# intellerce/controlanimate

Hardware: AMD Instinct MI355X
Metric: frames_per_sec (higher is better)
Workload: dtype fp16

## Files before the change

### controlanimate_amd/_capi.py

```python
from __future__ import annotations

import ctypes as C
import os

_HERE = os.path.dirname(os.path.abspath(__file__))
LIB_PATH = os.environ.get("CA_HIP_LIB") or os.path.join(_HERE, "csrc", "libcontrolanimate_hip.so")

CA_BF16, CA_F16 = 0, 1
CA_F32 = 2
CA_ACT_NONE, CA_ACT_SILU = 0, 1
CA_ACT_RELU = 4
CA_ACT_RELU6 = 5
CA_ACT_LEAKY02 = 6
CA_MLSD_TOPK = 200
CA_POSE_MAX_PEAKS, CA_POSE_MAX_PEOPLE, CA_POSE_AREA_TAPS = 64, 64, 8
CA_POSE_OVERFLOW_PEAKS, CA_POSE_OVERFLOW_PEOPLE = 1, 2
CA_POSE_OVERFLOW_FACES, CA_POSE_OVERFLOW_FACE_RESIZE = 4, 8
CA_FACE_SIZE, CA_FACE_HEAT, CA_FACE_PARTS, CA_FACE_MIN_SIDE, CA_FACE_SLOT_INTS = 384, 48, 71, 11, 8
CA_FACE_MODE_NONE, CA_FACE_MODE_LANCZOS4, CA_FACE_MODE_AREA = 0, 1, 2
CA_POSE_OVERFLOW_HANDS, CA_POSE_OVERFLOW_HAND_RESIZE = 16, 32
CA_HAND_PARTS, CA_HAND_HEAT_COLS, CA_HAND_MAP, CA_HAND_SCALES, CA_HAND_SLOT_INTS = 21, 24, 128, 4, 8
CA_HAND_MODE_NONE, CA_HAND_MODE_RESIZE, CA_HAND_MIN_BOX, CA_HAND_AREA_TAPS = 0, 1, 20, 16
ABI_VERSION = 16


class CAHipUnavailable(RuntimeError):
    pass


class CAHipError(RuntimeError):
    pass


class GemmArgs(C.Structure):
    _fields_ = [
        ("a", C.c_void_p), ("a2", C.c_void_p), ("w", C.c_void_p), ("c", C.c_void_p),
        ("bias", C.c_void_p), ("rowbias", C.c_void_p), ("residual", C.c_void_p),
        ("lda", C.c_int64), ("lda2", C.c_int64), ("ldc", C.c_int64), ("ld_res", C.c_int64),
        ("ld_rowbias", C.c_int64),
        ("m", C.c_int32), ("n", C.c_int32), ("k1", C.c_int32), ("k2", C.c_int32),
        ("rows_per_group", C.c_int32),
        ("alpha", C.c_float), ("post_scale", C.c_float),
        ("act", C.c_int32), ("geglu", C.c_int32), ("out_f32", C.c_int32), ("dtype", C.c_int32),
        ("ln_stats", C.c_void_p), ("ln_colsum", C.c_void_p), ("ln_eps", C.c_float),
        ("workspace", C.c_void_p), ("workspace_bytes", C.c_int64),
        ("row_sums_out", C.c_void_p), ("ln_parts", C.c_int32),
        ("w_frag", C.c_void_p),
    ]


class FfArgs(C.Structure):
    _fields_ = [
        ("x", C.c_void_p), ("w1_frag", C.c_void_p), ("bias1", C.c_void_p), ("colsum1", C.c_void_p), ("ln_stats", C.c_void_p),
        ("w2_frag", C.c_void_p), ("bias2", C.c_void_p), ("residual", C.c_void_p), ("y", C.c_void_p),
        ("lda", C.c_int64), ("ldc", C.c_int64), ("ld_res", C.c_int64),
        ("m", C.c_int32), ("c", C.c_int32), ("inner", C.c_int32), ("ln_eps", C.c_float), ("dtype", C.c_int32),
        ("w_out_frag", C.c_void_p), ("bias_out", C.c_void_p), ("residual_out", C.c_void_p), ("ld_res_out", C.c_int64),
    ]


class TattnArgs(C.Structure):
    _fields_ = [
        ("x", C.c_void_p), ("w_frag", C.c_void_p), ("gamma", C.c_void_p), ("bias_pe", C.c_void_p), ("o", C.c_void_p),
        ("lda", C.c_int64), ("ldo", C.c_int64), ("ld_bias_pe", C.c_int64),
        ("batch", C.c_int32), ("frames", C.c_int32), ("tokens", C.c_int32), ("heads", C.c_int32), ("c", C.c_int32),
        ("ln_eps", C.c_float), ("scale", C.c_float), ("dtype", C.c_int32),
        ("w_out_frag", C.c_void_p), ("bias_out", C.c_void_p), ("residual", C.c_void_p), ("ld_res", C.c_int64),
    ]


ATTN_WOUT_FRAG_ELEMS = 102400
TATTN_W_FRAG_ELEMS = 368640


class XattnArgs(C.Structure):
    _fields_ = [
        ("x", C.c_void_p), ("wq_frag", C.c_void_p), ("bias", C.c_void_p), ("kv_frag", C.c_void_p), ("o", C.c_void_p),
        ("lda", C.c_int64), ("ldo", C.c_int64),
        ("m", C.c_int32), ("tokens", C.c_int32), ("frames_per_kv", C.c_int32), ("kv_mod", C.c_int32), ("kv_batches", C.c_int32),
        ("nk", C.c_int32), ("heads", C.c_int32), ("c", C.c_int32),
        ("ln_eps", C.c_float), ("dtype", C.c_int32),
        ("w_out_frag", C.c_void_p), ("bias_out", C.c_void_p), ("residual", C.c_void_p), ("ld_res", C.c_int64),
        ("kv_frag_ip", C.c_void_p), ("nk_ip", C.c_int32), ("ip_scale", C.c_float),
    ]


XATTN_W_FRAG_ELEMS = 122880
XATTN_KV_FRAG_ELEMS = 7680


class ConvArgs(C.Structure):
    _fields_ = [
        ("x", C.c_void_p), ("x2", C.c_void_p), ("w", C.c_void_p), ("y", C.c_void_p),
        ("bias", C.c_void_p), ("rowbias", C.c_void_p), ("residual", C.c_void_p),
        ("ld_res", C.c_int64), ("ld_rowbias", C.c_int64),
        ("images", C.c_int32), ("hin", C.c_int32), ("win", C.c_int32),
        ("cin1", C.c_int32), ("cin2", C.c_int32), ("cout", C.c_int32),
        ("stride", C.c_int32), ("upsample", C.c_int32), ("rows_per_group", C.c_int32),
        ("alpha", C.c_float), ("post_scale", C.c_float),
        ("act", C.c_int32), ("out_f32", C.c_int32), ("dtype", C.c_int32),
        ("workspace", C.c_void_p), ("workspace_bytes", C.c_int64), ("pad_asym", C.c_int32),
        ("w_wino", C.c_void_p), ("x_is_wino_v", C.c_int32),
    ]


class GroupNormArgs(C.Structure):
    _fields_ = [
        ("x", C.c_void_p), ("x2", C.c_void_p), ("y", C.c_void_p),
        ("gamma", C.c_void_p), ("beta", C.c_void_p), ("partials", C.c_void_p),
        ("images", C.c_int32), ("hw", C.c_int32), ("c1", C.c_int32), ("c2", C.c_int32),
        ("groups", C.c_int32), ("frames_per_stat", C.c_int32),
        ("eps", C.c_float), ("act", C.c_int32), ("dtype", C.c_int32),
        ("wino_v", C.c_void_p), ("wino_h", C.c_int32), ("wino_w", C.c_int32),
    ]


class LayerNormArgs(C.Structure):
    _fields_ = [
        ("x", C.c_void_p), ("y", C.c_void_p), ("gamma", C.c_void_p), ("beta", C.c_void_p),
        ("pos", C.c_void_p),
        ("rows", C.c_int64),
        ("c", C.c_int32), ("rows_per_frame", C.c_int32), ("frames", C.c_int32),
        ("eps", C.c_float), ("dtype", C.c_int32), ("stats", C.c_void_p),
    ]


class AttnArgs(C.Structure):
    _fields_ = [
        ("q", C.c_void_p), ("k", C.c_void_p), ("v", C.c_void_p), ("o", C.c_void_p),
        ("q_outer", C.c_int64), ("q_inner", C.c_int64), ("q_row", C.c_int64),
        ("o_outer", C.c_int64), ("o_inner", C.c_int64), ("o_row", C.c_int64),
        ("k_outer", C.c_int64), ("k_inner", C.c_int64), ("k_row", C.c_int64),
        ("inner_count", C.c_int32), ("kv_inner_count", C.c_int32), ("kv_div", C.c_int32), ("kv_mod", C.c_int32),
        ("batches", C.c_int32), ("heads", C.c_int32), ("head_dim", C.c_int32),
        ("nq", C.c_int32), ("nk", C.c_int32),
        ("scale", C.c_float), ("out_scale", C.c_float),
        ("accumulate", C.c_int32), ("dtype", C.c_int32), ("causal", C.c_int32),
        ("key_mask", C.c_void_p), ("key_mask_stride", C.c_int64),
    ]


class ConvNarrowArgs(C.Structure):
    _fields_ = [
        ("x", C.c_void_p), ("w", C.c_void_p), ("y", C.c_void_p), ("bias", C.c_void_p), ("r1", C.c_void_p), ("r2", C.c_void_p),
        ("ldx", C.c_int64), ("ldy", C.c_int64), ("ld_r1", C.c_int64), ("ld_r2", C.c_int64),
        ("images", C.c_int32), ("hin", C.c_int32), ("win", C.c_int32), ("cin", C.c_int32), ("cout", C.c_int32),
        ("channel_offset", C.c_int32), ("upsample", C.c_int32), ("leaky_relu", C.c_int32),
        ("s0", C.c_float), ("s1", C.c_float), ("s2", C.c_float),
        ("out_u8", C.c_int32), ("dtype", C.c_int32),
    ]


class PerceiverAttnArgs(C.Structure):
    _fields_ = [
        ("q", C.c_void_p), ("x", C.c_void_p), ("l", C.c_void_p), ("o", C.c_void_p),
        ("q_row", C.c_int64), ("q_batch", C.c_int64),
        ("x_row", C.c_int64), ("x_batch", C.c_int64), ("x_v_off", C.c_int64),
        ("l_row", C.c_int64), ("l_batch", C.c_int64), ("l_v_off", C.c_int64),
        ("o_row", C.c_int64), ("o_batch", C.c_int64),
        ("batches", C.c_int32), ("heads", C.c_int32), ("head_dim", C.c_int32),
        ("nq", C.c_int32), ("n_x", C.c_int32), ("n_l", C.c_int32),
        ("scale", C.c_float), ("dtype", C.c_int32),
    ]


class ModconvArgs(C.Structure):
    _fields_ = [
        ("x", C.c_void_p), ("wt", C.c_void_p), ("s", C.c_void_p), ("demod", C.c_void_p), ("noise", C.c_void_p), ("bias", C.c_void_p),
        ("sft_scale", C.c_void_p), ("sft_shift", C.c_void_p), ("y", C.c_void_p),
        ("s_stride", C.c_int64), ("demod_stride", C.c_int64),
        ("images", C.c_int32), ("h", C.c_int32), ("w", C.c_int32), ("cin", C.c_int32), ("cout", C.c_int32),
        ("upsample", C.c_int32), ("x_shared", C.c_int32),
        ("noise_weight", C.c_float), ("dtype", C.c_int32),
    ]


class Conv7x7Args(C.Structure):
    _fields_ = [
        ("x", C.c_void_p * 2), ("w", C.c_void_p * 2), ("bias", C.c_void_p * 2), ("y", C.c_void_p * 2),
        ("ldx", C.c_int64), ("ldy", C.c_int64),
        ("groups", C.c_int32), ("images", C.c_int32), ("h", C.c_int32), ("w_px", C.c_int32), ("cin", C.c_int32), ("cout", C.c_int32),
        ("relu", C.c_int32), ("dtype", C.c_int32),
    ]


SYMBOLS = {
    "ca_abi_version": (C.c_int, []),
    "ca_last_error": (C.c_char_p, []),
    "ca_gemm": (C.c_int, [C.POINTER(GemmArgs), C.c_void_p]),
    "ca_pack_w_frag": (C.c_int, [C.c_void_p, C.c_int32, C.c_int32, C.c_int32, C.c_void_p, C.c_void_p]),
    "ca_pack_w2_frag": (C.c_int, [C.c_void_p, C.c_int32, C.c_int32, C.c_void_p, C.c_void_p]),
    "ca_ff_fused": (C.c_int, [C.POINTER(FfArgs), C.c_void_p]),
    "ca_ff_fused_supported": (C.c_int, [C.POINTER(FfArgs)]),
    "ca_tattn_fused": (C.c_int, [C.POINTER(TattnArgs), C.c_void_p]),
    "ca_tattn_fused_supported": (C.c_int, [C.POINTER(TattnArgs)]),
    "ca_pack_w_tattn": (C.c_int, [C.c_void_p, C.c_int32, C.c_int32, C.c_void_p, C.c_void_p]),
    "ca_pack_w_out": (C.c_int, [C.c_void_p, C.c_int32, C.c_int32, C.c_void_p, C.c_void_p]),
    "ca_xattn_fused": (C.c_int, [C.POINTER(XattnArgs), C.c_void_p]),
    "ca_xattn_fused_supported": (C.c_int, [C.POINTER(XattnArgs)]),
    "ca_xattn_pack_w": (C.c_int, [C.c_void_p, C.c_int32, C.c_int32, C.c_void_p, C.c_void_p]),
    "ca_xattn_pack_kv": (C.c_int, [C.c_void_p, C.c_int64, C.c_int32, C.c_int32, C.c_int32, C.c_int32, C.c_float, C.c_int32, C.c_void_p, C.c_void_p]),
    "ca_gemm_ln_inline_supported": (C.c_int, [C.POINTER(GemmArgs)]),
    "ca_gemm_wants_finished_stats": (C.c_int, [C.POINTER(GemmArgs)]),
    "ca_ln_finish_sums": (C.c_int, [C.c_void_p, C.c_int, C.c_int64, C.c_int, C.c_float, C.c_void_p, C.c_void_p]),
    "ca_gemm_workspace_bytes": (C.c_int64, [C.POINTER(GemmArgs)]),
    "ca_gemm_row_sums_parts": (C.c_int, [C.POINTER(GemmArgs)]),
    "ca_gemm_plan_name": (C.c_int, [C.POINTER(GemmArgs), C.c_char_p, C.c_int32]),
    "ca_conv3x3_plan_name": (C.c_int, [C.POINTER(ConvArgs), C.c_char_p, C.c_int32]),
    "ca_conv3x3": (C.c_int, [C.POINTER(ConvArgs), C.c_void_p]),
    "ca_pack_w_wino": (C.c_int, [C.c_void_p, C.c_int32, C.c_int32, C.c_int32, C.c_void_p, C.c_void_p]),
    "ca_conv3x3_workspace_bytes": (C.c_int64, [C.POINTER(ConvArgs)]),
    "ca_softmax_rows": (C.c_int, [C.c_void_p, C.c_void_p, C.c_int64, C.c_int32, C.c_int64, C.c_int64, C.c_float, C.c_int32, C.c_void_p]),
    "ca_groupnorm_partials_floats": (C.c_int64, [C.c_int32, C.c_int32, C.c_int32, C.c_int32]),
    "ca_groupnorm_stats": (C.c_int, [C.POINTER(GroupNormArgs), C.c_void_p]),
    "ca_groupnorm_apply": (C.c_int, [C.POINTER(GroupNormArgs), C.c_void_p]),
    "ca_groupnorm": (C.c_int, [C.POINTER(GroupNormArgs), C.c_void_p]),
    "ca_groupnorm_wino_supported": (C.c_int, [C.POINTER(GroupNormArgs)]),
    "ca_layernorm": (C.c_int, [C.POINTER(LayerNormArgs), C.c_void_p]),
    "ca_attention": (C.c_int, [C.POINTER(AttnArgs), C.c_void_p]),
    "ca_attention_plan_name": (C.c_int, [C.POINTER(AttnArgs), C.c_char_p, C.c_int32]),
    "ca_add_bcast": (C.c_int, [C.c_void_p, C.c_void_p, C.c_void_p, C.c_int64, C.c_int64, C.c_int32, C.c_void_p]),
    "ca_repeat": (C.c_int, [C.c_void_p, C.c_void_p, C.c_int64, C.c_int32, C.c_void_p]),
    "ca_silu_f32": (C.c_int, [C.c_void_p, C.c_void_p, C.c_int64, C.c_void_p]),
    "ca_timestep_embedding": (C.c_int, [C.c_void_p, C.c_float, C.c_void_p, C.c_int32, C.c_int32, C.c_int32, C.c_void_p]),
    "ca_latents_to_nhwc": (C.c_int, [C.c_void_p, C.c_void_p, C.c_int32, C.c_int32, C.c_int32, C.c_int32, C.c_int32,
                                      C.c_int32, C.c_int32, C.c_float, C.c_int32, C.c_void_p]),
    "ca_nhwc_to_ncfhw_f32": (C.c_int, [C.c_void_p, C.c_void_p, C.c_int32, C.c_int32, C.c_int32, C.c_int32, C.c_int32,
                                        C.c_int32, C.c_int32, C.c_int32, C.c_void_p]),
    "ca_ncfhw_to_nhwc": (C.c_int, [C.c_void_p, C.c_int32, C.POINTER(C.c_int64), C.c_void_p, C.c_int32, C.c_int32,
                                    C.c_int32, C.c_int32, C.c_int32, C.c_int32, C.c_int32, C.c_void_p]),
    "ca_cfg_scheduler_step": (C.c_int, [C.c_void_p, C.c_int32, C.c_int32, C.c_float, C.c_void_p, C.c_void_p,
                                         C.c_void_p, C.c_void_p, C.c_int32, C.c_int32, C.c_int32, C.c_int32,
                                         C.POINTER(C.c_float), C.c_float, C.c_void_p]),
    "ca_lincomb": (C.c_int, [C.c_void_p, C.POINTER(C.c_void_p), C.POINTER(C.c_float), C.c_int32, C.c_int64, C.c_void_p]),
    "ca_conv3x3_narrow": (C.c_int, [C.POINTER(ConvNarrowArgs), C.c_void_p]),
    "ca_conv3x3_narrow_plan_name": (C.c_int, [C.POINTER(ConvNarrowArgs), C.c_char_p, C.c_int32]),
    "ca_rgb8_to_nhwc": (C.c_int, [C.c_void_p, C.c_void_p, C.c_int32, C.c_int32, C.c_int32, C.c_int32, C.c_void_p]),
    "ca_resize_lanczos4_u8": (C.c_int, [C.c_void_p, C.c_void_p, C.c_int32, C.c_int32, C.c_int32, C.c_int32, C.c_int32,
                                         C.c_void_p, C.c_void_p, C.c_void_p, C.c_void_p, C.c_void_p]),
    "ca_color_match_workspace_bytes": (C.c_int64, [C.c_int32, C.c_int64]),
    "ca_hist_u8x3": (C.c_int, [C.c_void_p, C.c_void_p, C.c_int32, C.c_int64, C.c_void_p]),
    "ca_color_moments_f64": (C.c_int, [C.c_void_p, C.c_void_p, C.c_void_p, C.c_void_p, C.c_int32, C.c_int64, C.c_void_p, C.c_int64, C.c_void_p]),
    "ca_color_transform_f64": (C.c_int, [C.c_void_p, C.c_void_p, C.c_void_p, C.c_void_p, C.c_void_p, C.c_void_p, C.c_int32, C.c_int64, C.c_void_p]),
    "ca_sort_f64_segments": (C.c_int, [C.c_void_p, C.c_void_p, C.c_int32, C.c_int64, C.c_void_p, C.c_int64, C.c_void_p]),
    "ca_color_rank_map_f64": (C.c_int, [C.c_void_p, C.c_void_p, C.c_void_p, C.c_void_p, C.c_void_p, C.c_void_p, C.c_int32, C.c_int64,
                                         C.c_void_p, C.c_int64, C.c_void_p]),
    "ca_color_finish_u8": (C.c_int, [C.c_void_p, C.c_void_p, C.c_int32, C.c_int64, C.c_int32, C.c_void_p, C.c_int64, C.c_void_p]),
    "ca_canny_workspace_bytes": (C.c_int64, [C.c_int32, C.c_int32, C.c_int32]),
    "ca_canny_tile_w": (C.c_int32, []),
    "ca_canny_tile_h": (C.c_int32, []),
    "ca_canny_classify": (C.c_int, [C.c_void_p, C.c_int32, C.c_int32, C.c_int32, C.c_int32, C.c_int32, C.c_int32, C.c_void_p, C.c_int64, C.c_void_p]),
    "ca_canny_link": (C.c_int, [C.c_int32, C.c_int32, C.c_int32, C.c_void_p, C.c_int64, C.c_void_p]),
    "ca_canny_link_stage": (C.c_int, [C.c_int32, C.c_int32, C.c_int32, C.c_void_p, C.c_int64, C.c_int32, C.c_void_p]),
    "ca_canny_emit": (C.c_int, [C.c_int32, C.c_int32, C.c_int32, C.c_void_p, C.c_int64, C.c_void_p, C.c_void_p, C.c_int32, C.c_int32, C.c_void_p]),
    "ca_conv_up2_phase_supported": (C.c_int, [C.POINTER(ConvArgs)]),
    "ca_conv_up2_phase": (C.c_int, [C.POINTER(ConvArgs), C.c_void_p]),
    "ca_conv_up2_phase_plan_name": (C.c_int, [C.POINTER(ConvArgs), C.c_char_p, C.c_int32]),
    "ca_perceiver_attn": (C.c_int, [C.POINTER(PerceiverAttnArgs), C.c_void_p]),
    "ca_hed_prep": (C.c_int, [C.c_void_p, C.c_void_p, C.c_void_p, C.c_int32, C.c_int32, C.c_int32, C.c_int32, C.c_void_p]),
    "ca_hed_pool_side": (C.c_int, [C.c_void_p, C.c_void_p, C.c_void_p, C.c_void_p, C.c_void_p, C.c_int32, C.c_int32, C.c_int32, C.c_int32, C.c_int32, C.c_void_p]),
    "ca_hed_fuse": (C.c_int, [C.c_void_p, C.c_void_p, C.c_void_p, C.c_void_p, C.c_void_p, C.c_int32, C.c_int32, C.c_int32, C.c_void_p, C.c_void_p, C.c_int32, C.c_int32, C.c_void_p]),
    "ca_lineart_conv_in": (C.c_int, [C.c_void_p, C.c_void_p, C.c_void_p, C.c_int32, C.c_int32, C.c_int32, C.c_int32, C.c_void_p]),
    "ca_instnorm_partials_floats": (C.c_int64, [C.c_int32, C.c_int32, C.c_int32, C.c_int32]),
    "ca_instnorm_stats": (C.c_int, [C.c_void_p, C.c_void_p, C.c_int32, C.c_int32, C.c_int32, C.c_int32, C.c_int32, C.c_int32, C.c_void_p]),
    "ca_instnorm_apply": (C.c_int, [C.c_void_p, C.c_void_p, C.c_void_p, C.c_void_p, C.c_int32, C.c_int32, C.c_int32, C.c_int32, C.c_int32, C.c_int32, C.c_int32,
                                    C.c_int32, C.c_float, C.c_int32, C.c_void_p]),
    "ca_convt3x3s2_gather": (C.c_int, [C.c_void_p, C.c_void_p, C.c_int32, C.c_int32, C.c_int32, C.c_int32, C.c_int32, C.c_void_p]),
    "ca_lineart_conv_out": (C.c_int, [C.c_void_p, C.c_void_p, C.c_void_p, C.c_void_p, C.c_int32, C.c_int32, C.c_int32, C.c_int32, C.c_void_p]),
    "ca_lineart_finish": (C.c_int, [C.c_void_p, C.c_int32, C.c_int32, C.c_int32, C.c_void_p, C.c_void_p, C.c_int32, C.c_int32, C.c_void_p]),
    "ca_mlsd_prep": (C.c_int, [C.c_void_p, C.c_void_p, C.c_int32, C.c_int32, C.c_int32, C.c_int32, C.c_void_p]),
    "ca_dwconv3x3": (C.c_int, [C.c_void_p, C.c_void_p, C.c_void_p, C.c_void_p, C.c_int32, C.c_int32, C.c_int32, C.c_int32, C.c_int32, C.c_int32, C.c_int32, C.c_void_p]),
    "ca_upsample2x_bilinear_ac": (C.c_int, [C.c_void_p, C.c_void_p, C.c_int32, C.c_int32, C.c_int32, C.c_int32, C.c_int64, C.c_int32, C.c_int32, C.c_void_p]),
    "ca_conv3x3_dil": (C.c_int, [C.c_void_p, C.c_void_p, C.c_void_p, C.c_void_p, C.c_int32, C.c_int32, C.c_int32, C.c_int32, C.c_int32, C.c_int32, C.c_int32, C.c_void_p]),
    "ca_mlsd_decode_workspace_bytes": (C.c_int64, [C.c_int32, C.c_int32, C.c_int32]),
    "ca_mlsd_decode": (C.c_int, [C.c_void_p, C.c_int32, C.c_int32, C.c_int32, C.c_float, C.c_float, C.c_void_p, C.c_int64, C.c_void_p, C.c_void_p, C.c_void_p]),
    "ca_mlsd_draw": (C.c_int, [C.c_void_p, C.c_void_p, C.c_int32, C.c_int32, C.c_int32, C.c_void_p, C.c_void_p, C.c_int32, C.c_int32, C.c_void_p]),
    "ca_softedge_prep": (C.c_int, [C.c_void_p, C.c_void_p, C.c_int32, C.c_int32, C.c_int32, C.c_int32, C.c_void_p]),
    "ca_relu": (C.c_int, [C.c_void_p, C.c_void_p, C.c_int64, C.c_int32, C.c_void_p]),
    "ca_dwconv_k": (C.c_int, [C.c_void_p, C.c_void_p, C.c_void_p, C.c_int32, C.c_int32, C.c_int32, C.c_int32, C.c_int32, C.c_int32, C.c_int32, C.c_void_p]),
    "ca_maxpool2x2": (C.c_int, [C.c_void_p, C.c_void_p, C.c_int32, C.c_int32, C.c_int32, C.c_int32, C.c_int32, C.c_void_p]),
    "ca_pdc_block_supported": (C.c_int, [C.c_int32, C.c_int32]),
    "ca_pdc_block": (C.c_int, [C.c_void_p, C.c_void_p, C.c_void_p, C.c_void_p, C.c_int32, C.c_int32, C.c_int32, C.c_int32, C.c_int32, C.c_int32, C.c_void_p]),
    "ca_cdcm_dil4": (C.c_int, [C.c_void_p, C.c_void_p, C.c_void_p, C.c_int32, C.c_int32, C.c_int32, C.c_int32, C.c_int32, C.c_void_p]),
    "ca_csam_reduce": (C.c_int, [C.c_void_p] * 9 + [C.c_int32] * 5 + [C.c_void_p]),
    "ca_softedge_fuse": (C.c_int, [C.c_void_p] * 5 + [C.c_int32] * 4 + [C.c_void_p] * 3 + [C.c_int32, C.c_int32, C.c_void_p]),
    "ca_lanime_conv_in": (C.c_int, [C.c_void_p] * 5 + [C.c_int32] * 4 + [C.c_void_p]),
    "ca_conv4x4s2": (C.c_int, [C.c_void_p] * 4 + [C.c_int32] * 7 + [C.c_void_p]),
    "ca_im2col4x4s2": (C.c_int, [C.c_void_p] * 2 + [C.c_int32] * 5 + [C.c_void_p]),
    "ca_convt4x4s2": (C.c_int, [C.c_void_p] * 3 + [C.c_int32] * 6 + [C.c_void_p]),
    "ca_instnorm_act_partials_floats": (C.c_int64, [C.c_int32, C.c_int32, C.c_int32, C.c_int32]),
    "ca_instnorm_act": (C.c_int, [C.c_void_p, C.c_void_p] + [C.c_void_p, C.c_int32, C.c_int32, C.c_int32] * 2 + [C.c_int32] * 4 + [C.c_float, C.c_int32, C.c_void_p]),
    "ca_lanime_conv_out": (C.c_int, [C.c_void_p] * 4 + [C.c_int32] * 4 + [C.c_void_p]),
    "ca_lanime_finish": (C.c_int, [C.c_void_p, C.c_int32, C.c_int32, C.c_int32, C.c_void_p, C.c_void_p, C.c_int32, C.c_int32, C.c_void_p]),
    "ca_gfp_prep": (C.c_int, [C.c_void_p] * 4 + [C.c_int32] * 6 + [C.c_void_p]),
    "ca_resample2x": (C.c_int, [C.c_void_p] * 2 + [C.c_int32] * 6 + [C.c_void_p]),
    "ca_gfp_styles": (C.c_int, [C.c_void_p, C.c_void_p, C.c_int64, C.POINTER(C.c_int32), C.c_int32, C.c_void_p, C.c_int64, C.c_int32, C.c_int32, C.c_void_p]),
    "ca_modconv3x3": (C.c_int, [C.POINTER(ModconvArgs), C.c_void_p]),
    "ca_gfp_modulate": (C.c_int, [C.c_void_p, C.c_void_p, C.c_int64, C.c_void_p] + [C.c_int32] * 7 + [C.c_void_p]),
    "ca_gfp_style_epilogue": (C.c_int, [C.c_void_p, C.c_void_p, C.c_int64, C.c_void_p, C.c_float] + [C.c_void_p] * 4 + [C.c_int32] * 5 + [C.c_void_p]),
    "ca_gfp_to_rgb": (C.c_int, [C.c_void_p, C.c_void_p, C.c_void_p, C.c_int64, C.c_void_p, C.c_void_p, C.c_void_p] + [C.c_int32] * 5 + [C.c_void_p]),
    "ca_gfp_finish": (C.c_int, [C.c_void_p, C.c_void_p, C.c_int64, C.c_int32, C.c_void_p]),
    "ca_resize_pil_u8": (C.c_int, [C.c_void_p] * 3 + [C.c_int32] * 5 + [C.c_void_p, C.c_void_p, C.c_int32, C.c_void_p, C.c_void_p, C.c_int32, C.c_void_p]),
    "ca_dpt_patches": (C.c_int, [C.c_void_p, C.c_void_p] + [C.c_int32] * 4 + [C.c_void_p]),
    "ca_depth_to_space": (C.c_int, [C.c_void_p, C.c_void_p] + [C.c_int32] * 5 + [C.c_int64, C.c_int32, C.c_int32, C.c_int32, C.c_void_p]),
    "ca_dpt_head_supported": (C.c_int, [C.c_int32]),
    "ca_dpt_head": (C.c_int, [C.c_void_p] * 6 + [C.c_int32] * 5 + [C.c_void_p]),
    "ca_dpt_logit": (C.c_int, [C.c_void_p] * 4 + [C.c_int64, C.c_void_p]),
    "ca_resize_bicubic_f32": (C.c_int, [C.c_void_p] * 4 + [C.c_int32] * 5 + [C.c_void_p]),
    "ca_depth_finish": (C.c_int, [C.c_void_p, C.c_void_p] + [C.c_int32] * 4 + [C.c_void_p, C.c_void_p, C.c_int32, C.c_int32, C.c_void_p]),
    "ca_pose_prep": (C.c_int, [C.c_void_p] * 8 + [C.c_int32] * 8 + [C.c_void_p]),
    "ca_conv7x7": (C.c_int, [C.POINTER(Conv7x7Args), C.c_void_p]),
    "ca_im2col7x7": (C.c_int, [C.c_void_p] * 2 + [C.c_int32] * 4 + [C.c_int64, C.c_int32, C.c_void_p]),
    "ca_copy_cols": (C.c_int, [C.c_void_p, C.c_void_p, C.c_int64, C.c_int32, C.c_int64, C.c_int32, C.c_int32, C.c_void_p]),
    "ca_pose_maps_workspace_bytes": (C.c_int64, [C.c_int32] * 3),
    "ca_pose_maps": (C.c_int, [C.c_void_p] * 4 + [C.c_int64] + [C.c_void_p] * 3 + [C.c_int32] * 5 + [C.c_void_p]),
    "ca_pose_peaks": (C.c_int, [C.c_void_p] * 6 + [C.c_int32] * 3 + [C.c_void_p]),
    "ca_pose_connect": (C.c_int, [C.c_void_p] * 6 + [C.c_int32] * 3 + [C.c_void_p]),
    "ca_pose_assemble": (C.c_int, [C.c_void_p] * 9 + [C.c_int32] * 3 + [C.c_void_p]),
    "ca_pose_draw": (C.c_int, [C.c_void_p] * 6 + [C.c_int32] * 5 + [C.c_void_p]),
    "ca_face_boxes": (C.c_int, [C.c_void_p] * 6 + [C.c_int32] * 4 + [C.c_void_p]),
    "ca_face_crop": (C.c_int, [C.c_void_p] * 8 + [C.c_int32] * 8 + [C.c_void_p]),
    "ca_face_peaks": (C.c_int, [C.c_void_p] * 3 + [C.c_int32] * 4 + [C.c_void_p]),
    "ca_pose_draw_faces": (C.c_int, [C.c_void_p] * 9 + [C.c_int32] * 5 + [C.c_void_p]),
    "ca_hand_boxes": (C.c_int, [C.c_void_p] * 6 + [C.c_int32] * 4 + [C.c_void_p]),
    "ca_hand_crop": (C.c_int, [C.c_void_p] * 10 + [C.c_int32] * 10 + [C.c_void_p]),
    "ca_hand_maps": (C.c_int, [C.c_void_p] * 7 + [C.c_int32] + [C.c_void_p]),
    "ca_hand_peaks": (C.c_int, [C.c_void_p] * 6 + [C.c_int32] * 4 + [C.c_void_p]),
    "ca_pose_draw_hands": (C.c_int, [C.c_void_p] * 10 + [C.c_int32] * 5 + [C.c_void_p]),
}

_lib = None


def lib() -> C.CDLL:
    global _lib
    if _lib is not None:
        return _lib
    import torch
    if not os.path.exists(LIB_PATH):
        raise CAHipUnavailable(
            f"{LIB_PATH} is missing: the HIP extension is not built. Run "
            "`python -m controlanimate_amd._build` (needs hipcc); there is no CPU fallback.")
    try:
        handle = C.CDLL(LIB_PATH)
    except OSError as e:
        raise CAHipUnavailable(f"cannot load {LIB_PATH}: {e}") from e
    for name, (res, args) in SYMBOLS.items():
        fn = getattr(handle, name)
        fn.restype = res
        fn.argtypes = args
    if handle.ca_abi_version() != ABI_VERSION:
        raise CAHipUnavailable(f"ABI mismatch: library {handle.ca_abi_version()} vs binding {ABI_VERSION}; rebuild")
    _lib = handle
    return handle
# ... 7 lines not shown
```

### controlanimate_amd/attention_processor.py

```python
from __future__ import annotations

from typing import Optional

import torch
from torch import nn

from . import kernels as K
from .context import dispatch
from .layers import HipLinear, LnFold, WeightArena, ln_fold_enabled, pack_concat_rows


class AttnProcessor2_0(nn.Module):

    num_tokens = 0
    drop_ip_tokens = False

    def __init__(self, hidden_size=None, cross_attention_dim=None):
        super().__init__()

    def ip_branch(self, attn, q, ctx, out, images, tokens, kv_rows, frames_per_kv, kv_mod, cache):
        return out

    def ip_fragments(self, attn, ctx, cache):
        return None

    def __call__(self, attn: "Attention", hidden_states: torch.Tensor, encoder_hidden_states: Optional[torch.Tensor] = None,
                 attention_mask=None, temb=None, *, residual: Optional[torch.Tensor] = None, frames_per_kv: int = 1,
                 kv_mod: int = 0, temporal=None, cache: Optional[dict] = None, ln=None, row_sums: bool = False) -> torch.Tensor:
        if attention_mask is not None:
            raise NotImplementedError("attention_mask is not used anywhere on the reference's path")
        B, N, C = hidden_states.shape
        x = hidden_states.reshape(B * N, C)
        res = None if residual is None else residual.reshape(B * N, C)
        if ln is not None and encoder_hidden_states is None and temporal is not None and getattr(attn, "tfrag", None) is not None:
            b, f, n = temporal
            ofrag = getattr(attn, "ofrag", None)
            if ofrag is not None and dispatch.attn_out_fused:
                to_out = attn.to_out[0]
                out = K.tattn_fused(x, attn.tfrag.t, attn.tgamma.t, attn.tbias_pe.t, b, f, n, attn.heads, attn.tln_eps, attn.scale,
                                    w_out_frag=ofrag.t, bias_out=None if to_out.b is None else to_out.b.t, residual=res)
                if out is not None:
                    return out.reshape(B, N, C)
            o = K.tattn_fused(x, attn.tfrag.t, attn.tgamma.t, attn.tbias_pe.t, b, f, n, attn.heads, attn.tln_eps, attn.scale)
            if o is not None:
                out = attn.to_out[0].run(o, residual=res, row_sums=row_sums)
                return K.carry_row_sums(out.reshape(B, N, C), out)
        builtin = type(self).ip_branch is AttnProcessor2_0.ip_branch
        with_ip = (not builtin and type(self).ip_fragments is not AttnProcessor2_0.ip_fragments and dispatch.attn_out_fused and dispatch.xattn_ip_fused
                   and getattr(attn, "ofrag", None) is not None)
        if (ln is not None and encoder_hidden_states is not None and cache is not None and getattr(attn, "xfrag", None) is not None
                and (builtin or with_ip)):
            ctx = encoder_hidden_states
            nb, L, cd = ctx.shape
            nk = L - self.num_tokens
            kv = cache.get(("kv", id(attn)))
            if kv is None:
                kv = cache[("kv", id(attn))] = K.gemm(ctx.reshape(nb * L, cd), attn.kv.t)
            ent = cache.get(("kvf", id(attn)))
            if ent is None:
                ent = cache[("kvf", id(attn))] = (K.xattn_pack_kv(kv, nb, L, nk, attn.scale), nk, L)
            if ent[0] is not None and ent[1] == nk:
                ofrag = getattr(attn, "ofrag", None)
                if ofrag is not None and dispatch.attn_out_fused:
                    to_out = attn.to_out[0]
                    ipf = self.ip_fragments(attn, ctx, cache) if with_ip else None
                    if not with_ip or ipf is not None:
                        out = K.xattn_fused(x, attn.xfrag.t, ln[1].b.t, ent[0], B, N, frames_per_kv, kv_mod, nk, ln[1].eps, w_out_frag=ofrag.t,
                                            bias_out=None if to_out.b is None else to_out.b.t, residual=res,
                                            kv_frag_ip=None if ipf is None else ipf[0], nk_ip=0 if ipf is None else ipf[1],
                                            ip_scale=1.0 if ipf is None else ipf[2])
                        if out is not None:
                            return out.reshape(B, N, C)
                o = K.xattn_fused(x, attn.xfrag.t, ln[1].b.t, ent[0], B, N, frames_per_kv, kv_mod, nk, ln[1].eps) if builtin else None
                if o is not None:
                    out = attn.to_out[0].run(o, residual=res, row_sums=row_sums)
                    return K.carry_row_sums(out.reshape(B, N, C), out)
        if ln is not None:
            st, fold = ln
            if encoder_hidden_states is None and temporal is not None and fold.pe is not None:
                b, f, n = temporal
                qkv = K.gemm(x, fold.w.t, bias=fold.b.t, ln=(st, fold.cs.t), rowbias=fold.rowbias(b, f), rows_per_group=n)
            else:
                qkv = K.gemm(x, fold.w.t, bias=fold.b.t, ln=(st, fold.cs.t))
        if encoder_hidden_states is None:
            if ln is None:
                qkv = K.gemm(x, attn.qkv.t)
            if temporal is not None:
                b, f, n = temporal
                o = K.attention_temporal(qkv, b, f, n, attn.heads)
            else:
                o = K.attention_spatial(qkv, B, N, attn.heads)
        else:
            ctx = encoder_hidden_states
            nb, L, cd = ctx.shape
            q = qkv if ln is not None else K.gemm(x, attn.to_q.w.t)
            kv = None if cache is None else cache.get(("kv", id(attn)))
            if kv is None:
                kv = K.gemm(ctx.reshape(nb * L, cd), attn.kv.t)
                if cache is not None:
                    cache[("kv", id(attn))] = kv
            nk = L - self.num_tokens
            o = K.attention_cross(q, kv, B, N, attn.heads, nk, L, frames_per_kv, kv_mod=kv_mod)
            o = self.ip_branch(attn, q, ctx, o, B, N, L, frames_per_kv, kv_mod, cache)
        out = attn.to_out[0].run(o, residual=res, row_sums=row_sums)
        return K.carry_row_sums(out.reshape(B, N, C), out)


class IPAttnProcessor2_0(AttnProcessor2_0):

    def __init__(self, hidden_size, cross_attention_dim=None, scale=1.0, num_tokens=4):
        super().__init__()
        self.hidden_size = hidden_size
        self.cross_attention_dim = cross_attention_dim
        self.scale = scale
        self.num_tokens = num_tokens
        self.to_k_ip = HipLinear(cross_attention_dim or hidden_size, hidden_size, bias=False)
        self.to_v_ip = HipLinear(cross_attention_dim or hidden_size, hidden_size, bias=False)
        self.kv_ip = None

    def pack(self, arena: WeightArena, dtype):
        self.kv_ip = pack_concat_rows(arena, dtype, [self.to_k_ip, self.to_v_ip])

    def _kv_ip(self, ctx, cache):
        if self.kv_ip is None:
            raise RuntimeError("IPAttnProcessor2_0 installed after prepare(); call model.prepare() again")
        nb, L, cd = ctx.shape
        kvip = None if cache is None else cache.get(("kv_ip", id(self)))
        if kvip is None:
            kvip = K.gemm(ctx.reshape(nb * L, cd), self.kv_ip.t)
            if cache is not None:
                cache[("kv_ip", id(self))] = kvip
        return kvip

    def ip_fragments(self, attn, ctx, cache):
        nb, L, cd = ctx.shape
        if cache is None or not (1 <= self.num_tokens <= 16):
            return None
        ent = cache.get(("kvf_ip", id(self)))
        if ent is None:
            kvip = self._kv_ip(ctx, cache)
            ent = cache[("kvf_ip", id(self))] = (K.xattn_pack_kv(kvip, nb, L, self.num_tokens, attn.scale, row_offset=L - self.num_tokens),
                                                 self.num_tokens, L, attn.scale)
        if ent[0] is None or ent[1] != self.num_tokens or ent[2] != L:
            return None
        return ent[0], self.num_tokens, float(self.scale)

    def ip_branch(self, attn, q, ctx, out, images, tokens, kv_rows, frames_per_kv, kv_mod, cache):
        nb, L, cd = ctx.shape
        kvip = self._kv_ip(ctx, cache)
        return K.attention_cross(q, kvip, images, tokens, attn.heads, self.num_tokens, L, frames_per_kv, out=out,
                                 out_scale=float(self.scale), accumulate=True, kv_row_offset=L - self.num_tokens,
                                 kv_mod=kv_mod)


class CNAttnProcessor2_0(AttnProcessor2_0):

    def __init__(self, num_tokens=4):
        super().__init__()
        self.num_tokens = num_tokens


AttnProcessor = AttnProcessor2_0
IPAttnProcessor = IPAttnProcessor2_0
CNAttnProcessor = CNAttnProcessor2_0


class Attention(nn.Module):

    def __init__(self, query_dim: int, cross_attention_dim: Optional[int] = None, heads: int = 8, dim_head: int = 64,
                 dropout: float = 0.0, bias: bool = False, upcast_attention: bool = False, processor=None, **_):
        super().__init__()
        inner = heads * dim_head
        self.is_cross = cross_attention_dim is not None
        ctx_dim = cross_attention_dim if self.is_cross else query_dim
        self.query_dim, self.cross_attention_dim, self.inner_dim = query_dim, ctx_dim, inner
        self.heads = heads
        self.scale = dim_head ** -0.5
        self.spatial_norm = None
        self.group_norm = None
        self.norm_cross = None
        self.residual_connection = False
        self.rescale_output_factor = 1.0
        self.to_q = HipLinear(query_dim, inner, bias=bias)
        self.to_k = HipLinear(ctx_dim, inner, bias=bias)
        self.to_v = HipLinear(ctx_dim, inner, bias=bias)
        self.to_out = nn.ModuleList([HipLinear(inner, query_dim, bias=True), nn.Identity()])
        self.processor = processor if processor is not None else AttnProcessor2_0()
        self.qkv = self.kv = self.fold = None

    def set_processor(self, processor, _remove_lora: bool = False):
        if isinstance(getattr(self, "processor", None), nn.Module) and not isinstance(processor, nn.Module):
            self._modules.pop("processor", None)
        self.processor = processor

    def get_processor(self, return_deprecated_lora: bool = False):
        return self.processor

    def builtin_processor(self) -> bool:
        return type(self.processor) in (AttnProcessor2_0, IPAttnProcessor2_0, CNAttnProcessor2_0)

    def pack(self, arena: WeightArena, dtype, fold_ln=None, pe=None):
        self.fold = None
        if fold_ln is not None and self.builtin_processor() and ln_fold_enabled():
            self.fold = LnFold(arena, dtype, fold_ln, [self.to_q] if self.is_cross else [self.to_q, self.to_k, self.to_v], pe=pe)
            if self.is_cross:
                self.kv = pack_concat_rows(arena, dtype, [self.to_k, self.to_v])
                self.xfrag = None
                if (self.heads, self.inner_dim, self.query_dim) == (8, 320, 320):
                    from .layers import frag_order_xattn
                    fold = self.fold
                    self.xfrag = arena.add((122880,), dtype, lambda: frag_order_xattn(fold.w_fold().to(dtype).float()))
        elif self.is_cross:
            self.to_q.pack(arena, dtype)
            self.kv = pack_concat_rows(arena, dtype, [self.to_k, self.to_v])
        else:
            self.qkv = pack_concat_rows(arena, dtype, [self.to_q, self.to_k, self.to_v])
        self.to_out[0].pack(arena, dtype)
        self.ofrag = None
        if (self.heads, self.inner_dim, self.query_dim) == (8, 320, 320) and self.fold is not None:
            from .layers import _f32, frag_order_wout
            to_out = self.to_out[0]
            self.ofrag = arena.add((102400,), dtype, lambda: frag_order_wout(_f32(to_out.weight)))
        if hasattr(self.processor, "pack"):
            self.processor.pack(arena, dtype)

    def forward(self, hidden_states, encoder_hidden_states=None, attention_mask=None, **kw):
        return self.processor(self, hidden_states, encoder_hidden_states=encoder_hidden_states,
                              attention_mask=attention_mask, **kw)
```

### controlanimate_amd/context.py

```python
from __future__ import annotations

from dataclasses import dataclass, field
from typing import Optional

import torch


@dataclass
class ExecCtx:
    b: int
    f: int
    dtype: torch.dtype
    temb: torch.Tensor
    emb_groups: int
    ehs: Optional[torch.Tensor] = None
    frames_per_kv: int = 1
    kv_mod: int = 0
    gn_frames_per_stat: int = 1
    cache: dict = field(default_factory=dict)

    @property
    def images(self) -> int:
        return self.b * self.f

    def rows_per_emb_group(self, h: int, w: int) -> int:
        return self.images // self.emb_groups * h * w


class Dispatch:
    gemm_ar = True
    ff_fused = True
    tattn_fused = True
    xattn_fused = True
    attn_out_fused = True
    xattn_ip_fused = True
    conv_winograd = True
    gn_winograd = True
    conv_up2_phase = True
    ln_row_sums = True
    repeat_kernel = True
    ln_fold = True
    cfg_shared = True
    cn_cfg_dedup = True
    pdc_block_fused = True
    dpt_head_fused = False
    pose_conv7_direct = True
    controlnet_streams = 2


dispatch = Dispatch()
```

### controlanimate_amd/csrc/ca_gemm.hip

```cpp

#include "ca_gemm_plan.h"

namespace {
using namespace ca_gemm_detail;
#include "ca_conv_wino.h"

template <int DT, int BM, int BN, int WAVES_M, int WAVES_N, int MODE>
__global__ __launch_bounds__(256) void k_gemm(GemmKParams p) {
  constexpr int TM = BM / WAVES_M / 16;
  constexpr int TN = BN / WAVES_N / 16;
  constexpr int AI = BM / 32;
  constexpr int BI = BN / 32;
  static_assert(2 * (BM + BN) * BK >= BM * (BN + 8), "epilogue staging must fit");
  __shared__ __attribute__((aligned(16))) u16 smem[2 * (BM + BN) * BK];

  const int tid = threadIdx.x;
  const int lane = tid & 63;
  const int wid = tid >> 6;
  const int wm = wid / WAVES_N, wn = wid % WAVES_N;
  const int g = lane >> 4, l15 = lane & 15;

  const int tiles_n = (p.n + BN - 1) / BN;
  const unsigned bid = xcd_remap(blockIdx.x, gridDim.x);
  int tile_m, tile_n;
// ... 389 lines not shown
      return CA_OK;
    case PK_REG:
      if (g.bn == 128) hipLaunchKernelGGL((k_gemm<DT, 128, 128, 2, 2, MODE>), grid, dim3(256), 0, st, p);
      else if (g.bn == 64) hipLaunchKernelGGL((k_gemm<DT, 128, 64, 4, 1, MODE>), grid, dim3(256), 0, st, p);
      else break;
      return CA_OK;
  }
  CA_FAIL(CA_ERR_LAUNCH, "ca_gemm: no kernel for plan kind %d, tile %dx%d, %d stages", (int)g.kind, g.bm, g.bn, g.nbuf);
}

}

extern "C" int ca_gemm(const ca_gemm_args* a, void* stream) {
  DenseLaunch d;
  int rc = gemm_prepare(a, d);
  if (rc) return rc;
  hipStream_t st = (hipStream_t)stream;
  rc = a->dtype == CA_BF16 ? launch_gemm<CA_BF16, 0>(d.p, d.plan, st) : launch_gemm<CA_F16, 0>(d.p, d.plan, st);
  if (rc) return rc;
  CA_CHECK_LAUNCH("ca_gemm");
  return CA_OK;
}

extern "C" int64_t ca_gemm_workspace_bytes(const ca_gemm_args* a) {
  DenseLaunch d;
  return gemm_resolve(a, d) == CA_OK ? d.workspace : 0;
}

extern "C" int ca_gemm_row_sums_parts(const ca_gemm_args* a) {
  DenseLaunch d;
  DenseAsk ask{};
  ask.without_row_sums = true;
  return gemm_resolve(a, d, ask) == CA_OK ? row_sums_parts_of(d.p) : 0;
}

extern "C" int ca_gemm_ln_inline_supported(const ca_gemm_args* a) {
  DenseLaunch d;
  return a && a->ln_colsum && gemm_resolve(a, d) == CA_OK && wres_eligible(d.p) ? 1 : 0;
}

extern "C" int ca_gemm_wants_finished_stats(const ca_gemm_args* a) {
  if (!a || !a->ln_colsum || !a->ln_stats || a->ln_parts <= 0 || a->row_sums_out) return 0;
  DenseLaunch d;
  DenseAsk ask{};
  ask.stats_finished = true;
  return gemm_resolve(a, d, ask) == CA_OK && d.plan.kind == PK_PQ ? 1 : 0;
}

extern "C" int64_t ca_conv3x3_workspace_bytes(const ca_conv_args* a) { return conv_workspace_bytes(a); }

static int launch_conv_wino(const ca_conv_args* a, const GemmKParams& cp, hipStream_t st) {
  const int kc = a->cin1 + a->cin2;
  const ConvGeom g = conv_geom(a);
  const int64_t tiles = wino_tiles(a, g);
  WinoParams w{};
  w.x = (const u16*)a->x;
  w.x2 = (const u16*)a->x2;
  w.v = (u16*)a->workspace;
  u16* mm = (u16*)a->workspace + (a->x_is_wino_v ? 0 : 16 * tiles * kc);
  w.mm = mm;
  w.y = (u16*)a->y;
  w.bias = a->bias;
  w.rowbias = a->rowbias;
  w.res = (const u16*)a->residual;
  w.ld_res = a->ld_res;
  w.ld_rowbias = a->ld_rowbias;
  w.images = a->images, w.h = g.hl, w.w = g.wl, w.c1 = a->cin1, w.c2 = a->cin2, w.cout = a->cout;
  w.ups = a->upsample;
  w.rows_per_group = cp.rows_per_group;
  w.alpha = a->alpha, w.post = a->post_scale, w.act = a->act;
  const int64_t in_threads = tiles * (kc / 8), out_threads = tiles * (a->cout / 8);
  if (a->x_is_wino_v) w.v = (u16*)a->x;
  else if (a->dtype == CA_BF16) hipLaunchKernelGGL((k_wino_in<CA_BF16>), dim3((unsigned)((in_threads + 255) / 256)), dim3(256), 0, st, w);
  else hipLaunchKernelGGL((k_wino_in<CA_F16>), dim3((unsigned)((in_threads + 255) / 256)), dim3(256), 0, st, w);
  GemmKParams q{};
  q.a = w.v;
  q.w = (const u16*)a->w_wino;
  q.c = mm;
  q.lda = kc;
  q.ldc = a->cout;
  q.a_bytes = desc_bytes(16 * tiles * kc);
  q.w_bytes = desc_bytes((int64_t)16 * a->cout * kc);
  q.m = (int)(16 * tiles);
  q.n = a->cout;
  q.c1 = kc;
  q.taps = 1;
  q.kc_tiles = kc / BK;
  q.rows_per_group = 1;
  q.alpha = 1.f, q.post = 1.f;
  q.splits = 1;
  q.w_group_rows = (int)tiles;
  q.w_group_stride = (unsigned)((int64_t)a->cout * kc * 2);
  const unsigned gemm_tiles = (unsigned)((q.m / 256) * (q.n / 320));
  int rc = ca_launch_gemm_pp(q, a->dtype, 0, PK_PQ, gemm_tiles, st);
  if (rc) return rc;
  if (a->dtype == CA_BF16) hipLaunchKernelGGL((k_wino_out<CA_BF16>), dim3((unsigned)((out_threads + 255) / 256)), dim3(256), 0, st, w);
  else hipLaunchKernelGGL((k_wino_out<CA_F16>), dim3((unsigned)((out_threads + 255) / 256)), dim3(256), 0, st, w);
  return CA_OK;
}

extern "C" int ca_pack_w_wino(const void* w, int32_t cout, int32_t cin, int32_t dtype, void* dst, void* stream) {
  CA_REQUIRE(w && dst, "ca_pack_w_wino: null operand");
  CA_REQUIRE(cout > 0 && cin > 0 && (dtype == CA_BF16 || dtype == CA_F16), "ca_pack_w_wino: cout=%d cin=%d dtype=%d", cout, cin, dtype);
  const int64_t n = (int64_t)cout * cin;
  if (dtype == CA_BF16) hipLaunchKernelGGL((k_pack_w_wino<CA_BF16>), dim3((unsigned)((n + 255) / 256)), dim3(256), 0, (hipStream_t)stream, (const u16*)w, (u16*)dst, cout, cin);
  else hipLaunchKernelGGL((k_pack_w_wino<CA_F16>), dim3((unsigned)((n + 255) / 256)), dim3(256), 0, (hipStream_t)stream, (const u16*)w, (u16*)dst, cout, cin);
  CA_CHECK_LAUNCH("ca_pack_w_wino");
  return CA_OK;
}

extern "C" int ca_conv3x3(const ca_conv_args* a, void* stream) {
  GemmKParams p{};
  int rc = conv_prepare(a, p);
  if (rc) return rc;
  hipStream_t st = (hipStream_t)stream;
  if (wino_taken(a)) {
    rc = launch_conv_wino(a, p, st);
    if (rc) return rc;
    CA_CHECK_LAUNCH("ca_conv3x3(winograd)");
    return CA_OK;
  }
  CA_REQUIRE(!a->x_is_wino_v, "ca_conv3x3: x_is_wino_v, but the Winograd route does not take these arguments (images=%d %dx%d cin=%d+%d cout=%d dtype=%d w_wino=%p "
             "workspace=%p of %lld bytes, needs %lld)", a->images, a->hin, a->win, a->cin1, a->cin2, a->cout, a->dtype, a->w_wino, a->workspace,
             (long long)a->workspace_bytes, (long long)wino_workspace_bytes(a));
  rc = a->dtype == CA_BF16 ? launch_gemm<CA_BF16, 1>(p, plan_gemm(p, 1), st) : launch_gemm<CA_F16, 1>(p, plan_gemm(p, 1), st);
  if (rc) return rc;
  CA_CHECK_LAUNCH("ca_conv3x3");
  return CA_OK;
}

extern "C" int ca_conv_up2_phase_supported(const ca_conv_args* a) {
  GemmKParams p{};
  return up2_capable(a, p) && up2_pays(p) ? 1 : 0;
}

extern "C" int ca_conv_up2_phase(const ca_conv_args* a, void* stream) {
  GemmKParams p{};
  CA_REQUIRE(up2_capable(a, p), "ca_conv_up2_phase: arguments the phase form does not take (one fp16 / bf16 source with cin %% 64 == 0, cout %% 320 == 0, upsample = 1, "
             "stride 1, symmetric padding, no row bias / activation / post scale / fp32 output, 16-byte aligned operands, < 2^23 source pixels)");
  int rc = ca_launch_gemm_pp(p, a->dtype, 2, PK_PQ, up2_tiles_total(p), (hipStream_t)stream);
  if (rc) return rc;
  CA_CHECK_LAUNCH("ca_conv_up2_phase");
  return CA_OK;
}

extern "C" int ca_conv_up2_phase_plan_name(const ca_conv_args* a, char* buf, int32_t len) {
  CA_REQUIRE(buf && len > 0, "ca_conv_up2_phase_plan_name: buffer");
  GemmKParams p{};
  CA_REQUIRE(up2_capable(a, p), "ca_conv_up2_phase_plan_name: arguments the phase form does not take");
  snprintf(buf, (size_t)len, "up2_pq256x320");
  return CA_OK;
}

extern "C" int ca_gemm_plan_name(const ca_gemm_args* a, char* buf, int32_t len) {
  CA_REQUIRE(buf && len > 0, "ca_gemm_plan_name: buffer");
  DenseLaunch d;
  int rc = gemm_prepare(a, d);
  if (rc) return rc;
  plan_label(d.plan, buf, len);
  return CA_OK;
}

extern "C" int ca_conv3x3_plan_name(const ca_conv_args* a, char* buf, int32_t len) {
  CA_REQUIRE(buf && len > 0, "ca_conv3x3_plan_name: buffer");
  GemmKParams p{};
  int rc = conv_prepare(a, p);
  if (rc) return rc;
  if (wino_taken(a)) {
    snprintf(buf, (size_t)len, "wino_pq256x320");
    return CA_OK;
  }
  plan_label(plan_gemm(p, 1), buf, len);
  return CA_OK;
}
```

### controlanimate_amd/csrc/ca_gemm_core.h

```cpp
#pragma once
#include "ca_common.h"
#include <stdlib.h>

namespace ca_gemm_detail {


struct GemmKParams {
  const u16* a;
  const u16* a2;
  const u16* w;
  void* c;
  const float* bias;
  const float* rowbias;
  const float* ln_stats;
  const float* ln_colsum;
  const u16* res;
  int64_t lda, lda2, ldc, ld_res, ld_rowbias;
  unsigned a_bytes, a2_bytes, w_bytes;
  int m, n;
  int c1, c2;
  int taps;
  int kc_tiles;
  int hin, win, hout, wout, stride, ups, pad_lo;
  int rows_per_group;
  float alpha, post;
  int act, geglu, out_f32;
  int splits;
  float* partial;
  int dbg;
  int tap_inner;
  float* row_sums;
  int ln_parts;
  int ln_inline;
  float ln_eps;
  const u16* wf;
  int w_group_rows;
  unsigned w_group_stride;
  int up2_rows, up2_tiles;
  unsigned up2_mag_w, up2_mag_h;
};

constexpr int BK = 64;

constexpr int GROUP_M = 8;
__device__ __forceinline__ void tile_coords(unsigned bid, int tiles_m, int tiles_n, int& tile_m, int& tile_n) {
  const unsigned gsz = GROUP_M * tiles_n;
  const unsigned group = bid / gsz, in = bid - group * gsz;
  const int first_m = group * GROUP_M;
  const int gm = tiles_m - first_m < GROUP_M ? tiles_m - first_m : GROUP_M;
  tile_m = first_m + in % gm;
  tile_n = in / gm;
}

__device__ __forceinline__ void k_tile_split(const GemmKParams& p, int t, int kct, int& tap, int& cc) {
  if (p.taps == 1) {
    tap = 0;
    cc = t;
  } else if (p.tap_inner) {
    cc = t / p.taps;
    tap = t - cc * p.taps;
  } else {
    tap = t / kct;
    cc = t - tap * kct;
  }
}

__device__ __forceinline__ int lds_off(int row, int chunk) {
  return row * BK + ((chunk ^ ((row >> 1) & 7)) << 3);
}

template <int DT, int TM, int TN>
__device__ __forceinline__ void gemm_epilogue_direct(const GemmKParams& p, f32x4 (&acc)[TM][TN], int m0, int n0, int wm, int wn,
                                                     int l15, int g) {
#pragma unroll
  for (int i = 0; i < TM; ++i) {
    const int m = m0 + wm * TM * 16 + i * 16 + l15;
    if (m >= p.m) continue;
    const float* rbp = p.rowbias ? p.rowbias + (int64_t)(m / p.rows_per_group) * p.ld_rowbias : nullptr;
#pragma unroll
    for (int j = 0; j < TN; ++j) {
      const int n = n0 + wn * TN * 16 + j * 16 + g * 4;
      if (n >= p.n) continue;
      float v[4];
#pragma unroll
      for (int r = 0; r < 4; ++r) v[r] = acc[i][j][r];
      if (p.bias) {
        f32x4 b = *reinterpret_cast<const f32x4*>(p.bias + n);
#pragma unroll
        for (int r = 0; r < 4; ++r) v[r] += b[r];
      }
      if (rbp) {
        f32x4 b = *reinterpret_cast<const f32x4*>(rbp + n);
#pragma unroll
        for (int r = 0; r < 4; ++r) v[r] += b[r];
      }
#pragma unroll
      for (int r = 0; r < 4; ++r) v[r] *= p.alpha;
      if (p.res) {
        u32x2 rr = *reinterpret_cast<const u32x2*>(p.res + (int64_t)m * p.ld_res + n);
        v[0] += Elem<DT>::to_f((u16)(rr[0] & 0xffffu));
        v[1] += Elem<DT>::to_f((u16)(rr[0] >> 16));
        v[2] += Elem<DT>::to_f((u16)(rr[1] & 0xffffu));
        v[3] += Elem<DT>::to_f((u16)(rr[1] >> 16));
      }
#pragma unroll
      for (int r = 0; r < 4; ++r) v[r] *= p.post;
      if (p.act != CA_ACT_NONE) {
#pragma unroll
        for (int r = 0; r < 4; ++r) v[r] = act_f(v[r], p.act);
      }
      if (p.geglu) {
        const f32x2 gg = gelu_erf_f2((f32x2){v[1], v[3]});
        float o0 = v[0] * gg[0];
        float o1 = v[2] * gg[1];
        const int64_t off = (int64_t)m * p.ldc + (n >> 1);
        if (p.out_f32) {
          float* cp = reinterpret_cast<float*>(p.c) + off;
          cp[0] = o0;
          cp[1] = o1;
        } else {
          *reinterpret_cast<unsigned*>(reinterpret_cast<u16*>(p.c) + off) = pack2<DT>(o0, o1);
        }
      } else {
        const int64_t off = (int64_t)m * p.ldc + n;
        if (p.out_f32) {
          *reinterpret_cast<f32x4*>(reinterpret_cast<float*>(p.c) + off) = (f32x4){v[0], v[1], v[2], v[3]};
        } else {
          u32x2 o;
          o[0] = pack2<DT>(v[0], v[1]);
          o[1] = pack2<DT>(v[2], v[3]);
          *reinterpret_cast<u32x2*>(reinterpret_cast<u16*>(p.c) + off) = o;
        }
      }
    }
  }
}

template <int DT, int BM, int BN, int TM, int TN, int NT = 256, bool ROWSUM = false>
__device__ __forceinline__ void gemm_epilogue(const GemmKParams& p, f32x4 (&acc)[TM][TN], u16* cs, int m0, int n0, int wm, int wn,
                                              int l15, int g, int tid, float2* rs = nullptr) {
  if (p.n < 8) {
    gemm_epilogue_direct<DT, TM, TN>(p, acc, m0, n0, wm, wn, l15, g);
    return;
  }
  constexpr int CLD = BN + 8;
  float2 ln_st[TM];
  f32x4 ln_cs[TN];
  if (p.ln_stats) {
#pragma unroll
    for (int i = 0; i < TM; ++i) {
      const int m = m0 + wm * TM * 16 + i * 16 + l15;
      if (p.ln_parts > 0) {
        float a = 0.f, b = 0.f;
        if (m < p.m) {
          for (int q = 0; q < p.ln_parts; ++q) {
            const float2 v = *reinterpret_cast<const float2*>(p.ln_stats + ((int64_t)m * p.ln_parts + q) * 2);
            a += v.x;
            b += v.y;
          }
        }
        const float inv = 1.f / (float)(p.c1 + p.c2);
        const float mean = a * inv;
        ln_st[i] = make_float2(mean, rsqrtf(fmaxf(b * inv - mean * mean, 0.f) + p.ln_eps));
      } else {
        ln_st[i] = m < p.m ? *reinterpret_cast<const float2*>(p.ln_stats + (int64_t)m * 2) : make_float2(0.f, 0.f);
      }
    }
#pragma unroll
    for (int j = 0; j < TN; ++j) {
      const int n = n0 + wn * TN * 16 + j * 16 + g * 4;
      ln_cs[j] = n < p.n ? *reinterpret_cast<const f32x4*>(p.ln_colsum + n) : (f32x4){0.f, 0.f, 0.f, 0.f};
    }
  }
  f32x4 rb_q[TN];
  bool rb_uniform = false;
  if (p.rowbias) {
    const int r_first = m0 + wm * TM * 16, r_last = r_first + TM * 16 - 1;
    rb_uniform = r_last < p.m && r_first / p.rows_per_group == r_last / p.rows_per_group;
    if (rb_uniform) {
      const float* base = p.rowbias + (int64_t)(r_first / p.rows_per_group) * p.ld_rowbias;
#pragma unroll
      for (int j = 0; j < TN; ++j) {
        const int n = n0 + wn * TN * 16 + j * 16 + g * 4;
        rb_q[j] = n < p.n ? *reinterpret_cast<const f32x4*>(base + n) : (f32x4){0.f, 0.f, 0.f, 0.f};
      }
    }
  }
#pragma unroll
  for (int i = 0; i < TM; ++i) {
    const int row = wm * TM * 16 + i * 16 + l15;
    const int m = m0 + row;
    const float* rbp = (p.rowbias && !rb_uniform && m < p.m) ? p.rowbias + (int64_t)(m / p.rows_per_group) * p.ld_rowbias : nullptr;
// ... 186 lines not shown
```

### controlanimate_amd/csrc/ca_gemm_plan.h

```cpp
#pragma once
#include "ca_gemm_core.h"

namespace ca_gemm_detail {

inline unsigned desc_bytes(int64_t elems) {
  const int64_t b = elems * 2;
  return (b > 0 && b < (int64_t)0xFFFFFF00ll) ? (unsigned)b : 0u;
}

inline bool dma_shape_ok(const GemmKParams& p) { return (p.c1 + p.c2) % BK == 0 && (p.c2 == 0 || p.c1 % BK == 0); }
inline bool dma_sizes_ok(const GemmKParams& p) { return p.a_bytes != 0 && p.w_bytes != 0 && (p.c2 == 0 || p.a2_bytes != 0); }
inline bool dma_capable(const GemmKParams& p) { return dma_shape_ok(p) && dma_sizes_ok(p); }

inline bool wres_eligible(const GemmKParams& p) {
  static const int wres_env = CA_KNOB("CA_GEMM_WRES", -1);
  const int kc = p.c1 + p.c2;
  return wres_env != 0 && kc == 320 && p.taps == 1 && (p.c2 == 0 || p.c1 % 32 == 0) && p.n % 160 == 0 && p.n / 160 <= 32 && !p.out_f32 &&
         p.splits <= 1 && !p.ln_parts && dma_sizes_ok(p) &&
         (!p.rowbias || p.rows_per_group % 32 == 0) &&
         act_out_fit31(p) &&
         (wres_env == 1 || p.m >= 16384);
}

inline bool ar_eligible(const GemmKParams& p, bool scratch) {
// ... 188 lines not shown
  d = DenseLaunch{};
  GemmKParams& p = d.p;
  int rc = gemm_fill(a, p, ask);
  if (rc) return rc;
  const SplitK k = splitk_decide(p, 0);
  splitk_apply(k, a->workspace, a->workspace_bytes, p);
  d.workspace = k.bytes;
  if (p.ln_inline && p.wf) {
    if (ar_eligible(p, true)) d.workspace = (int64_t)p.m * 8;
    if (a->workspace && a->workspace_bytes >= (int64_t)p.m * 8) p.partial = reinterpret_cast<float*>(a->workspace);
  }
  d.plan = plan_gemm(p, 0);
  return CA_OK;
}

inline int gemm_prepare(const ca_gemm_args* a, DenseLaunch& d) {
  int rc = gemm_resolve(a, d);
  if (rc) return rc;
  CA_REQUIRE(!d.p.row_sums || row_sums_capable(d.p), "ca_gemm: row_sums_out is not available for this launch: ask ca_gemm_row_sums_parts() first");
  CA_REQUIRE(!d.p.ln_inline || wres_eligible(d.p), "ca_gemm: in-kernel LayerNorm statistics (ln_stats NULL) are not available for this launch: "
             "ask ca_gemm_ln_inline_supported() first and pass ln_stats otherwise");
  return CA_OK;
}

struct ConvGeom { int hl, wl, hout, wout; int64_t m; };
inline ConvGeom conv_geom(const ca_conv_args* a) {
  ConvGeom g;
  g.hl = a->hin << a->upsample, g.wl = a->win << a->upsample;
  const int pad = a->pad_asym ? 1 : 2;
  g.hout = (g.hl + pad - 3) / a->stride + 1;
  g.wout = (g.wl + pad - 3) / a->stride + 1;
  g.m = (int64_t)a->images * g.hout * g.wout;
  return g;
}
inline int64_t wino_tiles(const ca_conv_args* a, const ConvGeom& g) { return (int64_t)a->images * (g.hl / 2) * (g.wl / 2); }

inline int64_t wino_workspace_bytes(const ca_conv_args* a) {
  if (!a || !a->w_wino || (a->dtype != CA_F16 && a->dtype != CA_BF16) || a->stride != 1 || a->pad_asym || a->out_f32) return 0;
  if (a->upsample != 0 && a->upsample != 1) return 0;
  if (a->x_is_wino_v && (a->cin2 != 0 || a->upsample)) return 0;
  const ConvGeom g = conv_geom(a);
  if (a->images <= 0 || g.hl < 2 || g.wl < 2 || (g.hl & 1) || (g.wl & 1)) return 0;
  const int kc = a->cin1 + a->cin2;
  static const int min_cin = CA_KNOB("CA_WINO_MIN_CIN", 1280);
  if (kc < 640 || kc % BK != 0 || a->cin1 % 8 != 0 || a->cin2 % 8 != 0 || a->cout % 320 != 0) return 0;
  const int64_t tiles = wino_tiles(a, g);
  if (kc < min_cin && !(min_cin == 1280 && tiles <= 4096)) return 0;
  static const int max_tiles = CA_KNOB("CA_WINO_MAX_TILES", 16384);
  if (tiles % 256 != 0 || tiles > max_tiles) return 0;
  if (16 * tiles * (int64_t)(kc > a->cout ? kc : a->cout) * 2 >= 0x7FFFFF00ll) return 0;
  return 16 * tiles * (int64_t)((a->x_is_wino_v ? 0 : kc) + a->cout) * 2;
}

inline bool wino_taken(const ca_conv_args* a) {
  const int64_t wb = wino_workspace_bytes(a);
  return wb > 0 && a->workspace && a->workspace_bytes >= wb && (((uintptr_t)a->workspace | (uintptr_t)a->w_wino) & 15) == 0;
}

inline void conv_fill_sizes(const ca_conv_args* a, const ConvGeom& g, GemmKParams& p) {
  p.a_bytes = desc_bytes((int64_t)a->images * a->hin * a->win * a->cin1);
  p.a2_bytes = a->cin2 ? desc_bytes((int64_t)a->images * a->hin * a->win * a->cin2) : 0u;
  p.w_bytes = desc_bytes((int64_t)a->cout * 9 * (a->cin1 + a->cin2));
  p.m = (int)g.m, p.n = a->cout, p.c1 = a->cin1, p.c2 = a->cin2;
  p.taps = 9;
  static const int tap_inner_env = CA_KNOB("CA_CONV_TAP_INNER", 1);
  p.tap_inner = tap_inner_env;
  p.kc_tiles = ceil_div_i(a->cin1 + a->cin2, BK);
  p.hin = a->hin, p.win = a->win, p.hout = g.hout, p.wout = g.wout;
  p.stride = a->stride, p.ups = a->upsample, p.pad_lo = a->pad_asym ? 0 : 1;
  p.geglu = 0, p.out_f32 = a->out_f32;
  p.splits = 1;
}

inline int conv_prepare(const ca_conv_args* a, GemmKParams& p) {
  CA_REQUIRE(a != nullptr, "ca_conv3x3: null args");
  CA_REQUIRE(a->x && a->w && a->y, "ca_conv3x3: null operand");
  CA_REQUIRE(a->images > 0 && a->hin > 0 && a->win > 0, "ca_conv3x3: bad geometry");
  CA_REQUIRE(a->cin1 > 0 && a->cin1 % 8 == 0 && a->cin2 >= 0 && a->cin2 % 8 == 0,
             "ca_conv3x3: cin1=%d cin2=%d must be multiples of 8", a->cin1, a->cin2);
  CA_REQUIRE(a->cin2 == 0 || a->x2, "ca_conv3x3: x2 missing");
  CA_REQUIRE(a->stride == 1 || a->stride == 2, "ca_conv3x3: stride %d", a->stride);
  CA_REQUIRE(a->upsample == 0 || a->upsample == 1, "ca_conv3x3: upsample %d", a->upsample);
  CA_REQUIRE(a->dtype == CA_BF16 || a->dtype == CA_F16, "ca_conv3x3: dtype %d", a->dtype);
  CA_REQUIRE(!a->rowbias || a->rows_per_group > 0, "ca_conv3x3: rows_per_group");
  int rc = check_epilogue("ca_conv3x3", a->cout, 0, a->cout, a->ld_res, a->residual);
  if (rc) return rc;
  CA_REQUIRE(a->pad_asym == 0 || a->pad_asym == 1, "ca_conv3x3: pad_asym %d", a->pad_asym);
  const ConvGeom g = conv_geom(a);
  CA_REQUIRE(g.m < (1ll << 31), "ca_conv3x3: too many output pixels");
  conv_fill_sizes(a, g, p);
  p.a = (const u16*)a->x, p.a2 = (const u16*)a->x2, p.w = (const u16*)a->w, p.c = a->y;
  p.bias = a->bias, p.rowbias = a->rowbias, p.res = (const u16*)a->residual;
  p.ldc = a->cout, p.ld_res = a->ld_res, p.ld_rowbias = a->ld_rowbias;
  p.rows_per_group = a->rows_per_group > 0 ? a->rows_per_group : 1;
  p.alpha = a->alpha, p.post = a->post_scale, p.act = a->act;
  splitk_apply(splitk_decide(p, 1), a->workspace, a->workspace_bytes, p);
  return CA_OK;
}

inline int64_t conv_workspace_bytes(const ca_conv_args* a) {
  if (!a || a->images <= 0 || a->hin <= 0 || a->win <= 0 || (a->stride != 1 && a->stride != 2)) return 0;
  const int64_t wb = wino_workspace_bytes(a);
  if (wb > 0) return wb;
  const ConvGeom g = conv_geom(a);
  if (g.m >= (1ll << 31)) return 0;
  GemmKParams p{};
  conv_fill_sizes(a, g, p);
  return splitk_decide(p, 1).bytes;
}

inline bool up2_capable(const ca_conv_args* a, GemmKParams& p) {
  if (!a || !a->x || !a->w || !a->y || a->x2 || a->cin2 != 0 || a->images <= 0 || a->hin <= 0 || a->win <= 0) return false;
  if (a->upsample != 1 || a->stride != 1 || a->pad_asym || a->out_f32 || a->x_is_wino_v || a->rowbias) return false;
  if ((a->dtype != CA_F16 && a->dtype != CA_BF16) || a->act != CA_ACT_NONE || a->post_scale != 1.f) return false;
  if (a->cin1 <= 0 || a->cin1 % BK != 0 || a->cout <= 0 || a->cout % 320 != 0) return false;
  if ((((uintptr_t)a->x | (uintptr_t)a->w | (uintptr_t)a->y | (uintptr_t)a->residual) & 15) != 0) return false;
  if (a->residual && (a->ld_res < a->cout || a->ld_res % 8 != 0)) return false;
  const int64_t rows = (int64_t)a->images * a->hin * a->win;
  if (rows + a->win + 2 >= (1 << 23)) return false;
  p = GemmKParams{};
  p.a = (const u16*)a->x;
  p.w = (const u16*)a->w;
  p.c = a->y;
  p.bias = a->bias;
  p.res = (const u16*)a->residual;
  p.ldc = a->cout;
  p.ld_res = a->ld_res;
  p.a_bytes = desc_bytes(rows * a->cin1);
  p.w_bytes = desc_bytes((int64_t)4 * a->cout * 4 * a->cin1);
  p.n = a->cout;
  p.c1 = a->cin1;
  p.taps = 4;
  p.tap_inner = 1;
  p.kc_tiles = a->cin1 / BK;
  p.hin = a->hin, p.win = a->win, p.hout = 2 * a->hin, p.wout = 2 * a->win;
  p.stride = 1, p.ups = 1, p.pad_lo = 1;
  p.rows_per_group = 1;
  p.alpha = a->alpha, p.post = 1.f;
  p.splits = 1;
  p.up2_rows = (int)rows;
  p.up2_tiles = ceil_div_i((int)rows, 256);
  p.m = 4 * p.up2_tiles * 256;
  p.up2_mag_w = a->win == 1 ? 0xFFFFFFFFu : (unsigned)((1ull << 32) / (unsigned)a->win);
  p.up2_mag_h = a->hin == 1 ? 0xFFFFFFFFu : (unsigned)((1ull << 32) / (unsigned)a->hin);
  p.w_group_stride = (unsigned)((int64_t)a->cout * 4 * a->cin1 * 2);
  return dma_sizes_ok(p) && act_out_fit31(p) && p.w_bytes < FIT31;
}
inline unsigned up2_tiles_total(const GemmKParams& p) { return (unsigned)(4 * p.up2_tiles * (p.n / 320)); }
inline bool up2_pays(const GemmKParams& p) {
  const unsigned tiles = up2_tiles_total(p);
  return tiles >= 256 && (tiles % 256 == 0 || tiles >= 1024);
}

}
```

### controlanimate_amd/csrc/ca_gemm_pp.hip

```cpp
#include "ca_gemm_core.h"
#include <type_traits>

namespace {
using namespace ca_gemm_detail;
#include "ca_gemm_pp2.h"
#include "ca_gemm_wres.h"
#include "ca_gemm_ps.h"
#include "ca_gemm_pq.h"

int cu_count() {
  static int n = 0;
  if (!n) {
    int dev = 0;
    hipDeviceProp_t prop;
    if (hipGetDevice(&dev) == hipSuccess && hipGetDeviceProperties(&prop, dev) == hipSuccess) n = prop.multiProcessorCount;
    if (n <= 0) n = 256;
  }
  return n;
}

template <class Launch>
int launch_stamped(const GemmKParams& p, hipStream_t st, const char* label, unsigned sep, unsigned eol, Launch launch) {
  static unsigned long long* dbuf = nullptr;
  if (!dbuf && hipMalloc(&dbuf, 4096 * 8) != hipSuccess) return CA_ERR_LAUNCH;
  (void)hipMemsetAsync(dbuf, 0, 4096 * 8, st);
  GemmKParams q = p;
  q.partial = reinterpret_cast<float*>(dbuf);
  launch(q);
  (void)hipStreamSynchronize(st);
  static int printed = 0;
  if (printed++ < 1) {
    static unsigned long long host[4096];
    (void)hipMemcpy(host, dbuf, sizeof(host), hipMemcpyDeviceToHost);
    for (int g = 0; g < 2; ++g) {
      fprintf(stderr, "[%s stamps group %d, %dx%dx%d] tag:delta_cycles ...\n", label, g, p.m, p.n, (p.c1 + p.c2) * p.taps);
      unsigned long long prev = host[g * 2048];
      for (int i = 0; i < 1000 && host[g * 2048 + 2 * i]; ++i) {
        fprintf(stderr, "%llu:%llu ", host[g * 2048 + 2 * i + 1], host[g * 2048 + 2 * i] - prev);
        prev = host[g * 2048 + 2 * i];
        if (host[g * 2048 + 2 * i + 1] == sep) fprintf(stderr, "| ");
        if (host[g * 2048 + 2 * i + 1] == eol) fprintf(stderr, "\n");
      }
      fprintf(stderr, "\n");
    }
  }
  return CA_OK;
}

template <int DT, int MODE>
int launch_pp(const GemmKParams& p, PlanKind kind, unsigned tiles, hipStream_t st) {
  const unsigned c_bytes = (unsigned)c_extent_bytes(p), res_bytes = (unsigned)res_extent_bytes(p);
  const unsigned grid = tiles < (unsigned)cu_count() ? tiles : (unsigned)cu_count();
  switch (kind) {
    case PK_PQ: {
      auto launch = [&](const GemmKParams& q) {
        if (MODE == 0 && (q.geglu || q.ln_colsum || q.ln_stats)) hipLaunchKernelGGL((k_gemm_pq<DT, 0, 1>), dim3(grid), dim3(512), 0, st, q, (int)tiles, c_bytes, 0u);
        else if (MODE == 0 && q.row_sums) hipLaunchKernelGGL((k_gemm_pq<DT, 0, 2>), dim3(grid), dim3(512), 0, st, q, (int)tiles, c_bytes, res_bytes);
        else hipLaunchKernelGGL((k_gemm_pq<DT, MODE>), dim3(grid), dim3(512), 0, st, q, (int)tiles, c_bytes, res_bytes);
      };
#ifdef CA_STAMPS
      if (p.dbg == 9) return launch_stamped(p, st, "pq", 8, 10, launch);
#endif
      launch(p);
      return CA_OK;
    }
    case PK_PS: {
      auto launch = [&](const GemmKParams& q) { hipLaunchKernelGGL((k_gemm_ps<DT, MODE>), dim3(grid), dim3(512), 0, st, q, (int)tiles, c_bytes, res_bytes); };
#ifdef CA_STAMPS
      if (p.dbg == 9) return launch_stamped(p, st, "ps", 8, 10, launch);
#endif
      launch(p);
      return CA_OK;
    }
    case PK_WRES: {
      if (MODE != 0) return CA_ERR_LAUNCH;
      const int panels = p.n / 160;
      const int chunks = (p.m + 255) / 256;
      int per = (cu_count() / 8) / panels;
      if (per * 8 > chunks) per = chunks / 8;
      if (per < 1) per = 1;
      const unsigned rb_bytes = p.rowbias ? (unsigned)(((int64_t)((p.m - 1) / p.rows_per_group) * p.ld_rowbias + p.n) * 4) : 16u;
      hipLaunchKernelGGL((k_gemm_wres<DT>), dim3(8 * per * panels), dim3(512), 0, st, p, panels, 8 * per, chunks, rb_bytes, c_bytes, res_bytes);
      return CA_OK;
    }
    case PK_PP2:
      hipLaunchKernelGGL((k_gemm_pp2<DT, MODE>), dim3(tiles), dim3(512), 0, st, p);
      return CA_OK;
    default: return CA_ERR_LAUNCH;
  }
}

template <int DT>
int launch_up2(const GemmKParams& p, PlanKind kind, unsigned tiles, hipStream_t st) {
  if (kind != PK_PQ) return CA_ERR_LAUNCH;
  const unsigned grid = tiles < (unsigned)cu_count() ? tiles : (unsigned)cu_count();
  hipLaunchKernelGGL((k_gemm_pq<DT, 2>), dim3(grid), dim3(512), 0, st, p, (int)tiles, (unsigned)c_extent_bytes(p), (unsigned)res_extent_bytes(p));
  return CA_OK;
}
}

int ca_launch_gemm_pp(const ca_gemm_detail::GemmKParams& p0, int dtype, int mode, ca_gemm_detail::PlanKind kind, unsigned tiles, hipStream_t st) {
  static const int dbg = CA_KNOB("CA_PP_DBG", 0);
  ca_gemm_detail::GemmKParams p = p0;
  p.dbg = dbg;
  if (mode == 2) return dtype == CA_BF16 ? launch_up2<CA_BF16>(p, kind, tiles, st) : launch_up2<CA_F16>(p, kind, tiles, st);
  if (dtype == CA_BF16) return mode ? launch_pp<CA_BF16, 1>(p, kind, tiles, st) : launch_pp<CA_BF16, 0>(p, kind, tiles, st);
  return mode ? launch_pp<CA_F16, 1>(p, kind, tiles, st) : launch_pp<CA_F16, 0>(p, kind, tiles, st);
}
```

### controlanimate_amd/csrc/ca_gemm_pq.h

```cpp

#ifdef CA_PQ_ABLATE
#define CA_PQ_ABL(bit) (((CA_PQ_ABLATE) & (bit)) != 0)
#else
#define CA_PQ_ABL(bit) false
#endif

__device__ __forceinline__ unsigned pq_udiv(unsigned r, unsigned d, unsigned mag) {
  const unsigned q = __umulhi(r, mag);
  return r - q * d >= d ? q + 1 : q;
}

template <int DT, int MODE, int EPI = 0>
__global__ __launch_bounds__(512, 2) void k_gemm_pq(GemmKParams p, int tiles_total, unsigned c_bytes, unsigned res_bytes) {
  constexpr int BM = 256, BN = 320, KT = 64;
  constexpr int TM = 8, TN = 5;
  constexpr int A_ROWS = 256, B0_ROWS = 128, B1_ROWS = 192;
  constexpr int OFF_A = 0, OFF_B0 = A_ROWS * KT, OFF_B1 = (A_ROWS + B0_ROWS) * KT;
  constexpr int BUF = (A_ROWS + B0_ROWS + B1_ROWS) * KT;
  constexpr int PAR_BASE = 2 * BUF * 2;
  constexpr int P_BI = 0, P_RB0 = 1280, P_RB1 = 2560, P_CS = 3840, PSET = EPI == 1 ? 5120 : 4096;
  constexpr int FLAG_BASE = PAR_BASE + 2 * PSET;
  constexpr int SMEM_BYTES = FLAG_BASE + 8 * 2 * 256;
  static_assert(SMEM_BYTES <= 160 * 1024, "LDS");
  __shared__ __attribute__((aligned(16))) unsigned char smem_b[SMEM_BYTES];
  u16* const smem = reinterpret_cast<u16*>(smem_b);

  const int tid = threadIdx.x;
  const int lane = tid & 63;
  const int wid = __builtin_amdgcn_readfirstlane(tid >> 6);
  const int wr = wid >> 2, wc = wid & 3;
  const int g = lane >> 4, l15 = lane & 15;

  const int tiles_n = p.n / BN;
  const int tiles_m = MODE == 2 ? 4 * p.up2_tiles : (p.m + BM - 1) / BM;
  const int G = gridDim.x;
  const int bslot = (G % 8 == 0) ? (int)(blockIdx.x % 8) * (G / 8) + (int)(blockIdx.x / 8) : (int)blockIdx.x;
  const int my_tiles = bslot < tiles_total ? (tiles_total - bslot + G - 1) / G : 0;
  if (my_tiles == 0) return;

  for (int i = tid; i < 8 * 2 * 64; i += 512) reinterpret_cast<unsigned*>(smem_b + FLAG_BASE)[i] = 0xFFFFFFFFu;
  __syncthreads();

  const __amdgpu_buffer_rsrc_t rs_a = __builtin_amdgcn_make_buffer_rsrc((void*)p.a, 0, p.a_bytes, 0x00020000);
  const __amdgpu_buffer_rsrc_t rs_a2 = __builtin_amdgcn_make_buffer_rsrc((void*)(p.a2 ? p.a2 : p.a), 0, p.a2 ? p.a2_bytes : p.a_bytes, 0x00020000);
  const __amdgpu_buffer_rsrc_t rs_w = __builtin_amdgcn_make_buffer_rsrc((void*)p.w, 0, p.w_bytes, 0x00020000);
  const __amdgpu_buffer_rsrc_t rs_c = __builtin_amdgcn_make_buffer_rsrc(p.c, 0, c_bytes, 0x00020000);
  const __amdgpu_buffer_rsrc_t rs_bi = __builtin_amdgcn_make_buffer_rsrc((void*)(p.bias ? (const void*)p.bias : (const void*)p.w), 0, p.bias ? (unsigned)p.n * 4u : 0u, 0x00020000);
  const bool geglu = EPI == 1 && p.geglu != 0;
  const unsigned long long res_addr = (unsigned long long)(p.res ? (const void*)p.res : (const void*)p.c);
  const u32x4 rs_res = {(unsigned)__builtin_amdgcn_readfirstlane((int)(unsigned)res_addr), (unsigned)__builtin_amdgcn_readfirstlane((int)(unsigned)((res_addr >> 32) & 0xffffu)),
                        (unsigned)__builtin_amdgcn_readfirstlane((int)(p.res ? res_bytes : 0u)), 0x00020000u};
  const unsigned rb_groups = p.rowbias ? (unsigned)((p.m + p.rows_per_group - 1) / p.rows_per_group) : 0u;
  const __amdgpu_buffer_rsrc_t rs_rb = __builtin_amdgcn_make_buffer_rsrc((void*)(p.rowbias ? (const void*)p.rowbias : (const void*)p.w), 0,
                                                                         p.rowbias ? (unsigned)(((int64_t)(rb_groups - 1) * p.ld_rowbias + p.n) * 4) : 0u, 0x00020000);
  const __amdgpu_buffer_rsrc_t rs_seq = __builtin_amdgcn_make_buffer_rsrc((void*)ca_seq_table.v, 0, 4096u, 0x00020000);

#ifdef CA_STAMPS
  unsigned long long* const stamps = reinterpret_cast<unsigned long long*>(p.partial);
  int stamp_i = 0;
  auto stamp = [&](int tag) __attribute__((always_inline)) {
    if (p.dbg == 9 && blockIdx.x == 0 && (wid == 0 || wid == 4) && lane == 0 && stamp_i < 1000) {
      stamps[(wid >> 2) * 2048 + 2 * stamp_i] = __builtin_readcyclecounter();
      stamps[(wid >> 2) * 2048 + 2 * stamp_i + 1] = (unsigned long long)tag;
      ++stamp_i;
    }
  };
#else
  auto stamp = [&](int) __attribute__((always_inline)) {};
#endif
  auto swz = [](int row) { return (row >> 1) & 7; };
  const int kc = p.c1 + p.c2;
  const int kct = kc / KT;
  const unsigned wld = (unsigned)(p.taps * kc);
  const int nt = p.taps * kct;
  const int total_kt = my_tiles * nt;

  constexpr unsigned OOB_V = 0x80000000u;
  unsigned b0_v[2] = {0, 0}, b1_v[3] = {0, 0, 0};
  unsigned a_v[4] = {0, 0, 0, 0};
  int d_seq = 0, d_t = 0, d_tap = 0, d_c0 = 0, d_n = 0;
  bool d_live = true;
  unsigned char* const my_flags = smem_b + FLAG_BASE + wid * 2 * 256;

  auto tile_of = [&](int seq, int& tm, int& tn) __attribute__((always_inline)) -> bool {
    const int id = seq * G + bslot;
    if (id >= tiles_total) return false;
    tile_coords((unsigned)id, tiles_m, tiles_n, tm, tn);
    return true;
  };

  auto dma_set_tile = [&](int seq, int m0, int n0) __attribute__((always_inline)) {
    if (CA_PQ_ABL(16)) m0 = 0, n0 = 0;
    int lane_o = lane;
    asm volatile("" : "+v"(lane_o));
    const int r8 = lane_o >> 3, cp = lane_o & 7;
    const int a_chunk0 = cp ^ swz(r8), b1_chunk0 = cp ^ swz(wid * 24 + r8);
#pragma unroll
    for (int i = 0; i < 4; ++i) {
      const int m = m0 + wid * 32 + i * 8 + r8;
      const bool ok = m < p.m;
      if (MODE == 2) {
        const int ph = m0 / (p.up2_tiles * BM);
        const int py = ph >> 1, px = ph & 1;
        const int r = m - ph * (p.up2_tiles * BM);
        const bool okr = r < p.up2_rows;
        const int rr = okr ? r : p.up2_rows - 1;
        const unsigned q = pq_udiv((unsigned)rr, (unsigned)p.win, p.up2_mag_w);
        const int xs = rr - (int)q * p.win;
        const int ys = (int)q - (int)pq_udiv(q, (unsigned)p.hin, p.up2_mag_h) * p.hin;
        const int hi0 = ys + py - 1, wi0 = xs + px - 1;
        const int p0 = rr + (py - 1) * p.win + (px - 1);
        a_v[i] = ((unsigned)p0 & 0xFFFFFFu) | (hi0 >= 0 ? 1u << 24 : 0u) | (hi0 + 1 < p.hin ? 1u << 25 : 0u) | (wi0 >= 0 ? 1u << 26 : 0u) | (wi0 + 1 < p.win ? 1u << 27 : 0u) |
                 (okr ? 1u << 28 : 0u);
      } else if (MODE == 1) {
        const int mm = ok ? m : p.m - 1;
        const int hw = p.hout * p.wout;
        const int img = mm / hw;
        const int rem = mm - img * hw;
        const int ho = rem / p.wout, wo = rem - ho * p.wout;
        const int hi0 = ho * p.stride - p.pad_lo, wi0 = wo * p.stride - p.pad_lo;
        const int p0 = (img * p.hin + hi0) * p.win + wi0;
        a_v[i] = ((unsigned)p0 & 0xFFFFFFu) | (hi0 >= 0 ? 1u << 24 : 0u) | (hi0 + 2 < p.hin ? 1u << 25 : 0u) | (wi0 >= 0 ? 1u << 26 : 0u) | (wi0 + 2 < p.win ? 1u << 27 : 0u) |
                 (ok ? 1u << 28 : 0u);
      } else {
        a_v[i] = ok ? (unsigned)m * (unsigned)p.lda * 2u + (unsigned)((a_chunk0 ^ (4 * (i & 1))) * 16) : OOB_V;
      }
    }
    unsigned wgrp = 0u;
    if (MODE == 0 && EPI == 0 && p.w_group_rows > 0) wgrp = (unsigned)(m0 / p.w_group_rows) * p.w_group_stride;
    if (MODE == 2) wgrp = (unsigned)(m0 / (p.up2_tiles * BM)) * p.w_group_stride;
#pragma unroll
    for (int i = 0; i < 2; ++i) {
      const int r = wid * 16 + i * 8 + r8;
      b0_v[i] = wgrp + (unsigned)(n0 + (r >> 5) * 80 + ca_ps_col((r >> 4) & 1, r & 15, geglu)) * wld * 2u + (unsigned)((a_chunk0 ^ (4 * i)) * 16);
    }
#pragma unroll
    for (int i = 0; i < 3; ++i) {
      const int r1 = wid * 24 + i * 8 + r8;
      b1_v[i] = wgrp + (unsigned)(n0 + (r1 / 48) * 80 + ca_ps_col(2 + (r1 % 48) / 16, r1 & 15, geglu)) * wld * 2u + (unsigned)((b1_chunk0 ^ (4 * (i & 1))) * 16);
    }
    d_tap = 0;
    d_c0 = 0;
    unsigned char* pset = smem_b + PAR_BASE + (seq & 1) * PSET;
    if (EPI == 1 && wid == 4) {
      const __amdgpu_buffer_rsrc_t rs_cs = __builtin_amdgcn_make_buffer_rsrc((void*)(p.ln_colsum ? (const void*)p.ln_colsum : (const void*)p.w), 0, p.ln_colsum ? (unsigned)p.n * 4u : 0u, 0x00020000);
      __builtin_amdgcn_raw_ptr_buffer_load_lds(rs_cs, (__attribute__((address_space(3))) void*)(pset + P_CS), 16, (unsigned)n0 * 4u + lane_o * 16u, 0, 0, 0);
      __builtin_amdgcn_raw_ptr_buffer_load_lds(rs_cs, (__attribute__((address_space(3))) void*)(pset + P_CS + 1024), 4, (unsigned)n0 * 4u + 1024u + lane_o * 4u, 0, 0, 0);
    }
    if (wid >= 1 && wid <= 3) {
      const bool has1 = p.rowbias && m0 / p.rows_per_group + 1 < (int)rb_groups;
      const unsigned base = wid == 1 ? (unsigned)n0 * 4u
                                     : wid == 2 ? (unsigned)n0 * 4u + (unsigned)(p.rowbias ? m0 / p.rows_per_group : 0) * (unsigned)p.ld_rowbias * 4u
                                                : (has1 ? (unsigned)n0 * 4u + (unsigned)(m0 / p.rows_per_group + 1) * (unsigned)p.ld_rowbias * 4u : OOB_V);
      unsigned char* dst = pset + (wid == 1 ? P_BI : wid == 2 ? P_RB0 : P_RB1);
      if (wid == 1) {
        __builtin_amdgcn_raw_ptr_buffer_load_lds(rs_bi, (__attribute__((address_space(3))) void*)dst, 16, base + lane_o * 16u, 0, 0, 0);
        __builtin_amdgcn_raw_ptr_buffer_load_lds(rs_bi, (__attribute__((address_space(3))) void*)(dst + 1024), 4, base + 1024u + lane_o * 4u, 0, 0, 0);
      } else {
        __builtin_amdgcn_raw_ptr_buffer_load_lds(rs_rb, (__attribute__((address_space(3))) void*)dst, 16, base + lane_o * 16u, 0, 0, 0);
        __builtin_amdgcn_raw_ptr_buffer_load_lds(rs_rb, (__attribute__((address_space(3))) void*)(dst + 1024), 4, base + 1024u + lane_o * 4u, 0, 0, 0);
      }
    }
  };

  auto issue_tile = [&]() __attribute__((always_inline)) {
    if (!d_live) return;
    if (CA_PQ_ABL(1) && d_n >= 2) {
      ++d_n;
      ++d_t;
      return;
    }
    const int par = d_n & 1;
    u16* buf = smem + par * BUF;
    const unsigned wk = (unsigned)(d_tap * kc + d_c0) * 2u;
    const bool src2 = d_c0 >= p.c1;
    __builtin_amdgcn_raw_ptr_buffer_load_lds(rs_w, (__attribute__((address_space(3))) void*)(buf + OFF_B0 + (wid * 2 + 0) * 8 * KT), 16, b0_v[0], wk, 0, 0);
    __builtin_amdgcn_raw_ptr_buffer_load_lds(rs_w, (__attribute__((address_space(3))) void*)(buf + OFF_B0 + (wid * 2 + 1) * 8 * KT), 16, b0_v[1], wk, 0, 0);
    if (MODE != 0) {
      int lane_o = lane;
      asm volatile("" : "+v"(lane_o));
      const unsigned cs2 = (unsigned)(src2 ? p.c2 : p.c1) * 2u;
      const int kh = MODE == 2 ? d_tap >> 1 : (d_tap >= 6 ? 2 : (d_tap >= 3 ? 1 : 0)), kw = MODE == 2 ? d_tap & 1 : d_tap - kh * 3;
      const unsigned need = MODE == 2 ? (1u << 28) | (kh == 0 ? 1u << 24 : 1u << 25) | (kw == 0 ? 1u << 26 : 1u << 27)
                                      : (1u << 28) | (kh == 0 ? 1u << 24 : kh == 2 ? 1u << 25 : 0u) | (kw == 0 ? 1u << 26 : kw == 2 ? 1u << 27 : 0u);
      const int delta = kh * p.win + kw;
      const unsigned cadd = (unsigned)(src2 ? d_c0 - p.c1 : d_c0) * 2u + (unsigned)(((lane_o & 7) ^ swz(lane_o >> 3)) * 16);
#pragma unroll
      for (int i = 0; i < 4; ++i) {
        const unsigned av = a_v[i];
        const int pix = (((int)(av << 8)) >> 8) + delta;
        const unsigned off = __umul24((unsigned)pix, cs2) + (cadd ^ ((i & 1) ? 64u : 0u));
        const unsigned voff = (av & need) == need ? off : OOB_V;
        void* d = buf + OFF_A + (wid * 4 + i) * 8 * KT;
        if (src2) __builtin_amdgcn_raw_ptr_buffer_load_lds(rs_a2, (__attribute__((address_space(3))) void*)d, 16, voff, 0, 0, 0);
        else __builtin_amdgcn_raw_ptr_buffer_load_lds(rs_a, (__attribute__((address_space(3))) void*)d, 16, voff, 0, 0, 0);
      }
    } else {
#pragma unroll
      for (int i = 0; i < 4; ++i)
        __builtin_amdgcn_raw_ptr_buffer_load_lds(rs_a, (__attribute__((address_space(3))) void*)(buf + OFF_A + (wid * 4 + i) * 8 * KT), 16, a_v[i], (unsigned)d_c0 * 2u, 0, 0);
    }
#pragma unroll
    for (int i = 0; i < 3; ++i)
      __builtin_amdgcn_raw_ptr_buffer_load_lds(rs_w, (__attribute__((address_space(3))) void*)(buf + OFF_B1 + (wid * 3 + i) * 8 * KT), 16, b1_v[i], wk, 0, 0);
    __builtin_amdgcn_raw_ptr_buffer_load_lds(rs_seq, (__attribute__((address_space(3))) void*)(my_flags + par * 256), 4, 0u, (unsigned)(d_n & 1023) * 4u, 0, 0);
    ++d_n;
    ++d_t;
    if (p.taps == 1) {
      d_c0 += KT;
    } else if (++d_tap == p.taps) {
      d_tap = 0;
      d_c0 += KT;
    }
  };
#define CA_PQ_SET_TILE(SEQ)                                  \
  {                                                          \
    int tm_, tn_;                                            \
    d_live = tile_of((SEQ), tm_, tn_);                       \
    if (d_live) dma_set_tile((SEQ), tm_ * BM, tn_ * BN);     \
  }
  auto advance_and_issue = [&]() __attribute__((always_inline)) {
    if (d_t == nt) {
      d_t = 0;
      ++d_seq;
      CA_PQ_SET_TILE(d_seq)
    }
    issue_tile();
  };

  auto flag_begin = [&](int slot) __attribute__((always_inline)) -> unsigned {
    unsigned fv;
    const unsigned addr = (unsigned)(size_t)(__attribute__((address_space(3))) unsigned char*)(my_flags + slot * 256);
    asm volatile("ds_read_b32 %0, %1" : "=v"(fv) : "v"(addr) : "memory");
    return fv;
  };
  auto flag_finish = [&](int slot, int seqno, unsigned fv) __attribute__((always_inline)) {
    asm volatile("s_waitcnt lgkmcnt(0)" : "+v"(fv)::"memory");
    if (CA_PQ_ABL(1)) return;
    const unsigned want = (unsigned)(seqno & 1023);
    if ((unsigned)__builtin_amdgcn_readfirstlane(fv) == want) return;
    const unsigned addr = (unsigned)(size_t)(__attribute__((address_space(3))) unsigned char*)(my_flags + slot * 256);
    for (unsigned spins = 0; spins < (1u << 20); ++spins) {
      __builtin_amdgcn_s_sleep(1);
      unsigned v;
      asm volatile("ds_read_b32 %0, %1\n\ts_waitcnt lgkmcnt(0)" : "=v"(v) : "v"(addr) : "memory");
      if ((unsigned)__builtin_amdgcn_readfirstlane(v) == want) return;
    }
    asm volatile("s_waitcnt vmcnt(0)" ::: "memory");
  };

  f32x4 acc[TM][TN];
#pragma unroll
  for (int i = 0; i < TM; ++i)
#pragma unroll
    for (int j = 0; j < TN; ++j) acc[i][j] = (f32x4){0.f, 0.f, 0.f, 0.f};

  int fa_base, fb0_base, fb1_base;
  {
    const int ra = wr * 128 + l15, rb0 = wc * 32 + l15, rb1 = wc * 48 + l15;
    fa_base = OFF_A + ra * KT + ((g ^ swz(ra)) << 3);
    fb0_base = OFF_B0 + rb0 * KT + ((g ^ swz(rb0)) << 3);
    fb1_base = OFF_B1 + rb1 * KT + ((g ^ swz(rb1)) << 3);
  }
  u32x4 fa[TM], fb[TN];
  if (CA_PQ_ABL(2)) {
#pragma unroll
    for (int i = 0; i < TM; ++i) fa[i] = (u32x4){(unsigned)lane * 0x9E3779B9u + i, (unsigned)lane * 0x85EBCA6Bu, (unsigned)lane * 0xC2B2AE35u, (unsigned)lane * 0x27D4EB2Fu} & 0x3BFF3BFFu;
#pragma unroll
    for (int j = 0; j < TN; ++j) fb[j] = (u32x4){(unsigned)lane * 0x165667B1u + j, (unsigned)lane * 0xD3A2646Cu, (unsigned)lane * 0xFD7046C5u, (unsigned)lane * 0xB55A4F09u} & 0x3BFF3BFFu;
  }
  auto read_frags = [&](const u16* buf, int s) __attribute__((always_inline)) {
    if (CA_PQ_ABL(2)) {
#pragma unroll
      for (int i = 0; i < TM; ++i) asm volatile("" : "+v"(fa[i]));
#pragma unroll
      for (int j = 0; j < TN; ++j) asm volatile("" : "+v"(fb[j]));
      return;
    }
    const int x = s ? 32 : 0;
#pragma unroll
    for (int i = 0; i < TM; ++i) fa[i] = ld16(buf + (fa_base ^ x) + i * 16 * KT);
#pragma unroll
    for (int j = 0; j < 2; ++j) fb[j] = ld16(buf + (fb0_base ^ x) + j * 16 * KT);
#pragma unroll
    for (int j = 0; j < 3; ++j) fb[2 + j] = ld16(buf + (fb1_base ^ x) + j * 16 * KT);
  };
  auto mfma_all = [&]() __attribute__((always_inline)) {
    if (CA_PQ_ABL(4)) return;
    __builtin_amdgcn_sched_barrier(0);
    __builtin_amdgcn_s_setprio(1);
#pragma unroll
    for (int i = 0; i < TM; ++i)
#pragma unroll
      for (int j = 0; j < TN; ++j) acc[i][j] = Elem<DT>::mfma(fb[j], fa[i], acc[i][j]);
    __builtin_amdgcn_s_setprio(0);
    __builtin_amdgcn_sched_barrier(0);
  };

  auto epilogue = [&](int seq, int m0, int n0) __attribute__((always_inline)) {
    const unsigned char* pset = smem_b + PAR_BASE + (seq & 1) * PSET;
    int lane_o = lane;
    asm volatile("" : "+v"(lane_o));
    const int l15 = lane_o & 15, g = lane_o >> 4;
    int rb_sel = 0;
    if (p.rowbias) rb_sel = (m0 + wr * 128) / p.rows_per_group - m0 / p.rows_per_group;
    const unsigned char* rbp = pset + (rb_sel ? P_RB1 : P_RB0);
    f32x4 bi[TN], rb[TN];
#pragma unroll
    for (int j = 0; j < TN; ++j) {
      const int c0 = wc * 80 + (j < 4 ? 32 * (j >> 1) + 8 * g + 4 * (j & 1) : 64 + 4 * g);
      bi[j] = *reinterpret_cast<const f32x4*>(pset + P_BI + c0 * 4);
      rb[j] = *reinterpret_cast<const f32x4*>(rbp + c0 * 4);
    }
    const int up_ph = MODE == 2 ? m0 / (p.up2_tiles * BM) : 0;
    auto rowoff_of = [&](int i, int64_t ld) __attribute__((always_inline)) -> unsigned {
      int m = m0 + wr * 128 + i * 16 + l15;
      if (MODE == 2) {
        const int r = m - up_ph * (p.up2_tiles * BM);
        const int xs = r - (int)pq_udiv((unsigned)r, (unsigned)p.win, p.up2_mag_w) * p.win;
        m = r < p.up2_rows ? 4 * r - 2 * xs + (up_ph >> 1) * 2 * p.win + (up_ph & 1) : 0x7FFFFFFF;
      }
      return m < (MODE == 2 ? 4 * p.up2_rows : p.m) ? (unsigned)m * (unsigned)ld * 2u + (unsigned)(n0 + wc * 80) * 2u : OOB_V;
    };
    u32x4 r16[2][2];
    u32x2 r8[2];
    r16[0][0] = r16[0][1] = r16[1][0] = r16[1][1] = (u32x4){0u, 0u, 0u, 0u};
    r8[0] = r8[1] = (u32x2){0u, 0u};
    auto res_load = [&](int i, int slot) __attribute__((always_inline)) {
      const unsigned ro = rowoff_of(i, p.ld_res);
      const unsigned o0 = ro + (unsigned)(8 * g) * 2u, o1 = ro + (unsigned)(32 + 8 * g) * 2u, o2 = ro + (unsigned)(64 + 4 * g) * 2u;
      asm volatile("s_nop 4\n\tbuffer_load_dwordx4 %0, %3, %6, 0 offen\n\tbuffer_load_dwordx4 %1, %4, %6, 0 offen\n\tbuffer_load_dwordx2 %2, %5, %6, 0 offen"
                   : "=&v"(r16[slot][0]), "=&v"(r16[slot][1]), "=&v"(r8[slot])
                   : "v"(o0), "v"(o1), "v"(o2), "s"(rs_res)
                   : "memory");
    };
    float rsum[TM], rsq[TM];
#pragma unroll
    for (int i = 0; i < TM; ++i) rsum[i] = rsq[i] = 0.f;
    if (p.res) res_load(0, 0);
#pragma unroll
    for (int i = 0; i < TM; ++i) {
      const int slot = i & 1;
      if (p.res) {
        if (i + 1 < TM) res_load(i + 1, slot ^ 1);
        if (i == 0 || i + 1 == TM) asm volatile("s_waitcnt vmcnt(3)" ::: "memory");
        else asm volatile("s_waitcnt vmcnt(6)" ::: "memory");
        asm volatile("" : "+v"(r16[slot][0]), "+v"(r16[slot][1]), "+v"(r8[slot])::"memory");
      }
      const unsigned ro = (p.dbg != 1) ? rowoff_of(i, p.ldc) : OOB_V;
#pragma unroll
      for (int pr = 0; pr < 3; ++pr) {
        const int nq = pr < 2 ? 2 : 1;
        unsigned w[4] = {0u, 0u, 0u, 0u};
#pragma unroll
        for (int u = 0; u < 2; ++u) {
          if (u >= nq) break;
          const int j = pr * 2 + u;
          float v[4];
#pragma unroll
          for (int r = 0; r < 4; ++r) v[r] = ((acc[i][j][r] + bi[j][r]) + rb[j][r]) * p.alpha;
          acc[i][j] = (f32x4){0.f, 0.f, 0.f, 0.f};
          w[2 * u] = pack2<DT>(v[0], v[1]);
          w[2 * u + 1] = pack2<DT>(v[2], v[3]);
        }
#pragma unroll
        for (int k = 0; k < 4; ++k) {
          if (k >= 2 * nq) break;
          const unsigned rr = pr < 2 ? r16[slot][pr & 1][k] : r8[slot][k & 1];
          if (DT == CA_F16) {
            unsigned s_;
            asm("v_pk_add_f16 %0, %1, %2" : "=v"(s_) : "v"(w[k]), "v"(rr));
            w[k] = s_;
          } else {
            w[k] = pack2<DT>(Elem<DT>::to_f((u16)(w[k] & 0xffffu)) + Elem<DT>::to_f((u16)(rr & 0xffffu)),
                             Elem<DT>::to_f((u16)(w[k] >> 16)) + Elem<DT>::to_f((u16)(rr >> 16)));
          }
        }
        if (EPI == 2) {
#pragma unroll
          for (int k = 0; k < 4; ++k) {
            if (k >= 2 * nq) break;
            const float lo = Elem<DT>::to_f((u16)(w[k] & 0xffffu)), hi = Elem<DT>::to_f((u16)(w[k] >> 16));
            rsum[i] += lo + hi;
            rsq[i] = fmaf(lo, lo, fmaf(hi, hi, rsq[i]));
          }
        }
        if (pr < 2) __builtin_amdgcn_raw_buffer_store_b128((u32x4){w[0], w[1], w[2], w[3]}, rs_c, ro + (unsigned)(32 * pr + 8 * g) * 2u, 0, 0);
        else __builtin_amdgcn_raw_buffer_store_b64((u32x2){w[0], w[1]}, rs_c, ro + (unsigned)(64 + 4 * g) * 2u, 0, 0);
      }
    }
    if (EPI == 2) {
      const int tn4 = (n0 / BN) * 4 + wc, parts = (p.n / BN) * 4;
#pragma unroll
      for (int i = 0; i < TM; ++i) {
        float a = rsum[i], b = rsq[i];
        a += __shfl_xor(a, 16);
        b += __shfl_xor(b, 16);
        a += __shfl_xor(a, 32);
        b += __shfl_xor(b, 32);
        const int m = m0 + wr * 128 + i * 16 + l15;
        if (g == 0 && m < p.m) *reinterpret_cast<float2*>(p.row_sums + ((int64_t)m * parts + tn4) * 2) = make_float2(a, b);
      }
    }
    asm volatile("s_waitcnt lgkmcnt(0)" ::: "memory");
  };

  auto epilogue_ln = [&](int seq, int m0, int n0) __attribute__((always_inline)) {
    const unsigned char* pset = smem_b + PAR_BASE + (seq & 1) * PSET;
    int lane_o = lane;
    asm volatile("" : "+v"(lane_o));
    const int l15 = lane_o & 15, g = lane_o >> 4;
    float2 st[TM];
    if (p.ln_stats) {
      const __amdgpu_buffer_rsrc_t rs_st = __builtin_amdgcn_make_buffer_rsrc((void*)p.ln_stats, 0, (unsigned)p.m * 8u, 0x00020000);
#pragma unroll
      for (int i = 0; i < TM; ++i) {
        const int m = m0 + wr * 128 + i * 16 + l15;
        const u32x2 v = __builtin_bit_cast(u32x2, __builtin_amdgcn_raw_buffer_load_b64(rs_st, m < p.m ? (unsigned)m * 8u : OOB_V, 0, 0));
        st[i] = make_float2(__uint_as_float(v[0]), __uint_as_float(v[1]));
      }
    } else {
#pragma unroll
      for (int i = 0; i < TM; ++i) st[i] = make_float2(0.f, 1.f);
    }
    f32x4 cs[TN], bi[TN];
#pragma unroll
    for (int j = 0; j < TN; ++j) {
      const int c0 = wc * 80 + (geglu ? (j < 4 ? 16 * g + 4 * j : 64 + 4 * g) : (j < 4 ? 32 * (j >> 1) + 8 * g + 4 * (j & 1) : 64 + 4 * g));
      cs[j] = *reinterpret_cast<const f32x4*>(pset + P_CS + c0 * 4);
      bi[j] = *reinterpret_cast<const f32x4*>(pset + P_BI + c0 * 4);
    }
#pragma unroll
    for (int i = 0; i < TM; ++i) {
      const int m = m0 + wr * 128 + i * 16 + l15;
      const unsigned ro = (m < p.m && p.dbg != 1) ? (unsigned)m * (unsigned)p.ldc * 2u + (unsigned)(geglu ? (n0 >> 1) + wc * 40 : n0 + wc * 80) * 2u : OOB_V;
      unsigned w[TN];
#pragma unroll
      for (int j = 0; j < TN; ++j) {
        float v[4];
#pragma unroll
        for (int r = 0; r < 4; ++r) {
          float x = st[i].y * (acc[i][j][r] - st[i].x * cs[j][r]);
          x = (x + bi[j][r]) + 0.f;
          v[r] = x * p.alpha;
        }
        if (geglu) {
#pragma unroll
          for (int r = 0; r < 4; ++r) v[r] = Elem<DT>::to_f(Elem<DT>::from_f(v[r]));
          const f32x2 gg = gelu_erf_f2((f32x2){v[1], v[3]});
          w[j] = pack2<DT>(v[0] * gg[0], v[2] * gg[1]);
        } else if (j < 4) {
          const unsigned lo = pack2<DT>(v[0], v[1]), hi = pack2<DT>(v[2], v[3]);
          if ((j & 1) == 0) {
            w[0] = lo;
            w[1] = hi;
          } else {
            __builtin_amdgcn_raw_buffer_store_b128((u32x4){w[0], w[1], lo, hi}, rs_c, ro + (unsigned)(32 * (j >> 1) + 8 * g) * 2u, 0, 0);
          }
        } else {
          __builtin_amdgcn_raw_buffer_store_b64((u32x2){pack2<DT>(v[0], v[1]), pack2<DT>(v[2], v[3])}, rs_c, ro + (unsigned)(64 + 4 * g) * 2u, 0, 0);
        }
      }
      if (geglu) {
        __builtin_amdgcn_raw_buffer_store_b128((u32x4){w[0], w[1], w[2], w[3]}, rs_c, ro + (unsigned)(8 * g) * 2u, 0, 0);
        __builtin_amdgcn_raw_buffer_store_b32(w[4], rs_c, ro + (unsigned)(32 + 2 * g) * 2u, 0, 0);
      }
    }
#pragma unroll
    for (int i = 0; i < TM; ++i)
#pragma unroll
      for (int j = 0; j < TN; ++j) acc[i][j] = (f32x4){0.f, 0.f, 0.f, 0.f};
    asm volatile("s_waitcnt lgkmcnt(0)" ::: "memory");
  };

  const bool g1_late = MODE != 0 && wr == 1;
  CA_PQ_SET_TILE(0)
  issue_tile();
  if (g1_late) advance_and_issue();
  {
    const unsigned f0 = flag_begin(0);
    flag_finish(0, 0, f0);
  }
  __builtin_amdgcn_s_barrier();
  if (wr == 1) __builtin_amdgcn_s_barrier();

  int cv = 0;
  for (int seq = 0; seq < my_tiles; ++seq) {
    int tm, tn;
    tile_of(seq, tm, tn);
    const int m0 = tm * BM, n0 = tn * BN;
    for (int t = 0; t < (p.dbg == 2 ? 0 : nt); ++t) {
      const int par = cv & 1;
      const u16* buf = smem + par * BUF;
      stamp(1);
      __builtin_amdgcn_sched_barrier(0);
      read_frags(buf, 0);
      if (!g1_late) advance_and_issue();
      asm volatile("s_waitcnt lgkmcnt(0)" ::: "memory");
      stamp(2);
      if (!CA_PQ_ABL(8)) __builtin_amdgcn_s_barrier();
      stamp(3);
      mfma_all();
      stamp(4);
      if (!CA_PQ_ABL(8)) __builtin_amdgcn_s_barrier();
      stamp(5);
      __builtin_amdgcn_sched_barrier(0);
      unsigned fl = 0;
      if (wr == 1) fl = flag_begin(par ^ 1);
      read_frags(buf, 1);
      if (wr == 1 && cv + 1 < total_kt) flag_finish(par ^ 1, cv + 1, fl);
      else asm volatile("s_waitcnt lgkmcnt(0)" ::: "memory");
      stamp(6);
      if (!CA_PQ_ABL(8)) __builtin_amdgcn_s_barrier();
      stamp(7);
      if (g1_late) advance_and_issue();
      if (wr == 0) fl = flag_begin(par ^ 1);
      mfma_all();
      if (wr == 0 && cv + 1 < total_kt) flag_finish(par ^ 1, cv + 1, fl);
      stamp(8);
      if (!CA_PQ_ABL(8)) __builtin_amdgcn_s_barrier();
      ++cv;
    }
    if (wr == 0) __builtin_amdgcn_s_barrier();
    stamp(9);
    if (EPI == 1) epilogue_ln(seq, m0, n0);
    else epilogue(seq, m0, n0);
    stamp(10);
    if (wr == 1) __builtin_amdgcn_s_barrier();
  }
#undef CA_PQ_SET_TILE
  if (wr == 0) __builtin_amdgcn_s_barrier();
}
```

### controlanimate_amd/kernels.py

```python
from __future__ import annotations

import ctypes as C
from typing import Optional

import torch

from . import _capi
from .context import dispatch
from ._capi import (AttnArgs, ConvArgs, ConvNarrowArgs, FfArgs, PerceiverAttnArgs, TattnArgs, XattnArgs, GemmArgs, GroupNormArgs, LayerNormArgs, CA_ACT_NONE,
                    CA_ACT_SILU, CA_BF16, CA_F16, check, lib)

ACT_NONE, ACT_SILU = CA_ACT_NONE, CA_ACT_SILU
ACT_QUICK_GELU, ACT_GELU = 2, 3
ACT_RELU = _capi.CA_ACT_RELU
ACT_RELU6 = _capi.CA_ACT_RELU6


def dt_code(dtype: torch.dtype) -> int:
    if dtype == torch.bfloat16:
        return CA_BF16
    if dtype == torch.float16:
        return CA_F16
    raise TypeError(f"activations must be bf16 or fp16, got {dtype}")

# ... 25 lines not shown
         bias: Optional[torch.Tensor] = None, rowbias: Optional[torch.Tensor] = None,
         rows_per_group: int = 0, residual: Optional[torch.Tensor] = None, alpha: float = 1.0,
         post_scale: float = 1.0, act: int = ACT_NONE, geglu: bool = False, out_f32: bool = False,
         out: Optional[torch.Tensor] = None, ln=None, row_sums: bool = False) -> torch.Tensor:
    _req_cuda(a, w, a2, bias, rowbias, residual, out)
    assert a.dim() == 2 and a.stride(1) == 1 and w.dim() == 2 and w.is_contiguous()
    m, k1 = a.shape
    k2 = 0
    if a2 is not None:
        assert a2.dim() == 2 and a2.stride(1) == 1 and a2.shape[0] == m and a2.dtype == a.dtype
        k2 = a2.shape[1]
    n = w.shape[0]
    assert w.shape[1] == k1 + k2 and w.dtype == a.dtype
    ncols = n // 2 if geglu else n
    if out is None:
        out = torch.empty((m, ncols), device=a.device, dtype=torch.float32 if out_f32 else a.dtype)
    assert out.shape == (m, ncols) and out.stride(1) == 1
    if residual is not None:
        assert residual.shape == (m, n) and residual.stride(1) == 1 and residual.dtype == a.dtype
    if bias is not None:
        assert bias.dtype == torch.float32 and bias.numel() == n
    if rowbias is not None:
        assert rowbias.dtype == torch.float32 and rowbias.dim() == 2 and rowbias.shape[1] == n and rows_per_group > 0
    args = GemmArgs(a=_p(a), a2=_p(a2), w=_p(w), c=_p(out), bias=_p(bias), rowbias=_p(rowbias),
                    residual=_p(residual), lda=a.stride(0), lda2=a2.stride(0) if a2 is not None else 0,
                    ldc=out.stride(0), ld_res=residual.stride(0) if residual is not None else 0,
                    ld_rowbias=rowbias.stride(0) if rowbias is not None else 0,
                    m=m, n=n, k1=k1, k2=k2, rows_per_group=rows_per_group, alpha=alpha,
                    post_scale=post_scale, act=act, geglu=int(geglu), out_f32=int(out_f32),
                    dtype=dt_code(a.dtype))
    frag = getattr(w, "_frag", None)
    if frag is not None and frag[1] == bool(geglu) and dispatch.gemm_ar:
        args.w_frag = _p(frag[0])
    if ln is not None:
        st, cs = ln
        assert cs.dtype == torch.float32 and cs.numel() == n
        args.ln_colsum = _p(cs)
        if isinstance(st, RowStats):
            assert st.x.data_ptr() == a.data_ptr() and st.x.shape == a.shape, "RowStats belongs to another tensor"
            args.ln_eps = st.eps
            if lib().ca_gemm_ln_inline_supported(C.byref(args)):
                pass
            elif st.sums is not None:
                rs, parts = st.sums
                assert rs.shape == (m, parts, 2) and rs.dtype == torch.float32 and rs.is_contiguous()
                args.ln_stats, args.ln_parts = _p(rs), min(parts, 4)
                if parts > 4 or lib().ca_gemm_wants_finished_stats(C.byref(args)):
                    fin = getattr(st, "_finished", None)
                    if fin is None:
                        fin = torch.empty((m, 2), device=a.device, dtype=torch.float32)
                        check(lib().ca_ln_finish_sums(_p(rs), parts, m, k1 + k2, st.eps, _p(fin), _stream()), "ca_ln_finish_sums")
                        st._finished = fin
                    args.ln_stats, args.ln_parts = _p(fin), 0
            else:
                st = st.tensor()
        if not isinstance(st, RowStats):
            assert st.dtype == torch.float32 and st.shape == (m, 2) and st.is_contiguous()
            args.ln_stats = _p(st)
    if hasattr(out, "_row_sums"):
        del out._row_sums
    if row_sums and dispatch.ln_row_sums and not geglu and not out_f32:
        parts = int(lib().ca_gemm_row_sums_parts(C.byref(args)))
        if parts > 0:
            rs = torch.empty((m, parts, 2), device=a.device, dtype=torch.float32)
            args.row_sums_out = _p(rs)
            out._row_sums = (rs, parts)
    wbytes = 0 if args.row_sums_out else int(lib().ca_gemm_workspace_bytes(C.byref(args)))
    if wbytes > 0:
        ws = torch.empty((wbytes,), device=a.device, dtype=torch.uint8)
        args.workspace, args.workspace_bytes = _p(ws), wbytes
    _record_plan(lib().ca_gemm_plan_name, args)
    check(lib().ca_gemm(C.byref(args), _stream()), "ca_gemm")
    return out


def attach_w_frag(w: torch.Tensor, geglu: bool = False) -> torch.Tensor:
    _req_cuda(w)
    if w.dim() != 2 or w.shape[1] != 320 or w.shape[0] % 320 != 0 or not w.is_contiguous() or w.dtype not in (torch.float16, torch.bfloat16):
        return w
    dst = torch.empty_like(w)
    check(lib().ca_pack_w_frag(w.data_ptr(), w.shape[0], w.shape[1], int(bool(geglu)), dst.data_ptr(), _stream()), "ca_pack_w_frag")
    w._frag = (dst, bool(geglu))
    return w


def ff_fused(x: torch.Tensor, w1_frag: torch.Tensor, bias1: torch.Tensor, colsum1: torch.Tensor, w2_frag: torch.Tensor,
             bias2: Optional[torch.Tensor], ln_eps: float, residual: Optional[torch.Tensor] = None,
             ln_stats: Optional[torch.Tensor] = None, *, w_out_frag: Optional[torch.Tensor] = None, bias_out: Optional[torch.Tensor] = None,
             residual_out: Optional[torch.Tensor] = None) -> Optional[torch.Tensor]:
    if not dispatch.ff_fused:
        return None
    _req_cuda(x, w1_frag, bias1, colsum1, w2_frag, bias2, residual, ln_stats, w_out_frag, bias_out, residual_out)
    if x.dim() != 2 or x.stride(1) != 1 or (residual is not None and (residual.shape != x.shape or residual.stride(1) != 1 or residual.dtype != x.dtype)):
        return None
    if w_out_frag is None and (bias_out is not None or residual_out is not None):
        return None
    if residual_out is not None and (residual_out.shape != x.shape or residual_out.stride(1) != 1 or residual_out.dtype != x.dtype):
        return None
    m, c = x.shape
    inner = w2_frag.shape[1]
    y = torch.empty((m, c), device=x.device, dtype=x.dtype)
    args = FfArgs(x=_p(x), w1_frag=_p(w1_frag), bias1=_p(bias1), colsum1=_p(colsum1), ln_stats=_p(ln_stats), w2_frag=_p(w2_frag),
                  bias2=_p(bias2), residual=_p(residual), y=_p(y), lda=x.stride(0), ldc=y.stride(0),
                  ld_res=residual.stride(0) if residual is not None else 0, m=m, c=c, inner=inner, ln_eps=float(ln_eps), dtype=dt_code(x.dtype),
                  w_out_frag=_p(w_out_frag), bias_out=_p(bias_out), residual_out=_p(residual_out),
                  ld_res_out=residual_out.stride(0) if residual_out is not None else 0)
    if not lib().ca_ff_fused_supported(C.byref(args)):
        return None
    if _plan_sink is not None:
        _plan_sink.append("ff_out128" if w_out_frag is not None else "ff_fused128")
    check(lib().ca_ff_fused(C.byref(args), _stream()), "ca_ff_fused")
    return y


def tattn_fused(x: torch.Tensor, w_frag: torch.Tensor, gamma: torch.Tensor, bias_pe: torch.Tensor, b: int, frames: int, tokens: int,
                heads: int, ln_eps: float, scale: float, *, w_out_frag: Optional[torch.Tensor] = None, bias_out: Optional[torch.Tensor] = None,
                residual: Optional[torch.Tensor] = None) -> Optional[torch.Tensor]:
    if not dispatch.tattn_fused:
        return None
    _req_cuda(x, w_frag, gamma, bias_pe, w_out_frag, bias_out, residual)
    if x.dim() != 2 or x.stride(1) != 1 or x.shape[0] != b * frames * tokens or bias_pe.shape[0] < frames or bias_pe.stride(1) != 1:
        return None
    if w_out_frag is None and (bias_out is not None or residual is not None):
        return None
    if residual is not None and (residual.shape != x.shape or residual.stride(1) != 1 or residual.dtype != x.dtype):
        return None
    c = x.shape[1]
    o = torch.empty((x.shape[0], c), device=x.device, dtype=x.dtype)
    args = TattnArgs(x=_p(x), w_frag=_p(w_frag), gamma=_p(gamma), bias_pe=_p(bias_pe), o=_p(o), lda=x.stride(0), ldo=o.stride(0),
                     ld_bias_pe=bias_pe.stride(0), batch=b, frames=frames, tokens=tokens, heads=heads, c=c, ln_eps=float(ln_eps),
                     scale=float(scale), dtype=dt_code(x.dtype), w_out_frag=_p(w_out_frag), bias_out=_p(bias_out), residual=_p(residual),
                     ld_res=residual.stride(0) if residual is not None else 0)
    if not lib().ca_tattn_fused_supported(C.byref(args)):
        return None
    if _plan_sink is not None:
        _plan_sink.append("tattn_out128" if w_out_frag is not None else "tattn_fused128")
    check(lib().ca_tattn_fused(C.byref(args), _stream()), "ca_tattn_fused")
    return o


def xattn_pack_kv(kv: torch.Tensor, kv_batches: int, rows_per_batch: int, nk: int, scale: float, row_offset: int = 0,
                  out: Optional[torch.Tensor] = None) -> Optional[torch.Tensor]:
    if (not dispatch.xattn_fused or kv.dim() != 2 or kv.shape[1] != 640 or kv.stride(1) != 1 or not (64 < nk <= 80 or 1 <= nk <= 16)
            or kv.dtype not in (torch.float16, torch.bfloat16)):
        return None
    _req_cuda(kv)
    dst = out if out is not None else torch.empty((kv_batches, 8, _capi.XATTN_KV_FRAG_ELEMS), device=kv.device, dtype=kv.dtype)
    assert dst.shape == (kv_batches, 8, _capi.XATTN_KV_FRAG_ELEMS) and dst.dtype == kv.dtype and dst.is_contiguous()
    check(lib().ca_xattn_pack_kv(kv.data_ptr(), kv.stride(0), kv_batches, rows_per_batch, row_offset, nk, float(scale), dt_code(kv.dtype),
                                 dst.data_ptr(), _stream()), "ca_xattn_pack_kv")
    return dst


def xattn_fused(x: torch.Tensor, wq_frag: torch.Tensor, bias: Optional[torch.Tensor], kv_frag: torch.Tensor, images: int, tokens: int,
                frames_per_kv: int, kv_mod: int, nk: int, ln_eps: float, *, w_out_frag: Optional[torch.Tensor] = None,
                bias_out: Optional[torch.Tensor] = None, residual: Optional[torch.Tensor] = None, kv_frag_ip: Optional[torch.Tensor] = None,
                nk_ip: int = 0, ip_scale: float = 1.0) -> Optional[torch.Tensor]:
    if not dispatch.xattn_fused or kv_frag is None:
        return None
    _req_cuda(x, wq_frag, bias, kv_frag, w_out_frag, bias_out, residual, kv_frag_ip)
    if kv_frag_ip is not None and (w_out_frag is None or kv_frag_ip.shape != kv_frag.shape or kv_frag_ip.dtype != x.dtype or not kv_frag_ip.is_contiguous()):
        return None
    if x.dim() != 2 or x.stride(1) != 1 or x.shape[0] != images * tokens:
        return None
    if w_out_frag is None and (bias_out is not None or residual is not None):
        return None
    if residual is not None and (residual.shape != x.shape or residual.stride(1) != 1 or residual.dtype != x.dtype):
        return None
    assert kv_frag.dtype == x.dtype and wq_frag.dtype == x.dtype, "ca_xattn_fused: x, the packed Wq and the packed K/V must share one dtype"
    c = x.shape[1]
    o = torch.empty((x.shape[0], c), device=x.device, dtype=x.dtype)
    args = XattnArgs(x=_p(x), wq_frag=_p(wq_frag), bias=_p(bias), kv_frag=_p(kv_frag), o=_p(o), lda=x.stride(0), ldo=o.stride(0), m=x.shape[0],
                     tokens=tokens, frames_per_kv=frames_per_kv, kv_mod=kv_mod if kv_mod > 0 else images, kv_batches=kv_frag.shape[0],
                     nk=nk, heads=8, c=c, ln_eps=float(ln_eps), dtype=dt_code(x.dtype), w_out_frag=_p(w_out_frag), bias_out=_p(bias_out),
                     residual=_p(residual), ld_res=residual.stride(0) if residual is not None else 0, kv_frag_ip=_p(kv_frag_ip),
                     nk_ip=nk_ip if kv_frag_ip is not None else 0, ip_scale=float(ip_scale) if kv_frag_ip is not None else 0.0)
    if not lib().ca_xattn_fused_supported(C.byref(args)):
        return None
    if _plan_sink is not None:
        _plan_sink.append(("xattn_ip_out128" if kv_frag_ip is not None else "xattn_out128") if w_out_frag is not None else "xattn_fused128")
    check(lib().ca_xattn_fused(C.byref(args), _stream()), "ca_xattn_fused")
    return o


def row_sums_of(t: torch.Tensor):
    return getattr(t, "_row_sums", None)


def carry_row_sums(dst: torch.Tensor, src: torch.Tensor) -> torch.Tensor:
    s = getattr(src, "_row_sums", None)
    if s is not None:
        dst._row_sums = s
    return dst


class RowStats:

    def __init__(self, x: torch.Tensor, eps: float = 1e-5, sums=None):
        self.x, self.eps, self._t, self.sums = x, float(eps), None, sums

    def tensor(self) -> torch.Tensor:
        if self._t is None:
            self._t = row_stats(self.x, self.eps)
        return self._t


def conv3x3(x: torch.Tensor, w: torch.Tensor, *, x2: Optional[torch.Tensor] = None,
            bias: Optional[torch.Tensor] = None, rowbias: Optional[torch.Tensor] = None,
            rows_per_group: int = 0, residual: Optional[torch.Tensor] = None, stride: int = 1,
            upsample: bool = False, alpha: float = 1.0, post_scale: float = 1.0, act: int = ACT_NONE,
            out_f32: bool = False, pad_asym: bool = False, w_wino: Optional[torch.Tensor] = None,
            out: Optional[torch.Tensor] = None, split_k: bool = True) -> torch.Tensor:
    _req_cuda(x, w, x2, bias, rowbias, residual, w_wino)
    assert x.dim() == 4 and x.is_contiguous() and w.dim() == 4 and w.is_contiguous()
    images, hin, win, cin1 = x.shape
    cin2 = 0
    if x2 is not None:
        assert x2.is_contiguous() and x2.shape[:3] == x.shape[:3] and x2.dtype == x.dtype
        cin2 = x2.shape[3]
    cout = w.shape[0]
    assert tuple(w.shape[1:]) == (3, 3, cin1 + cin2) and w.dtype == x.dtype
    hl, wl = (hin * 2, win * 2) if upsample else (hin, win)
    pad = 1 if pad_asym else 2
    hout, wout = (hl + pad - 3) // stride + 1, (wl + pad - 3) // stride + 1
    if out is None:
        y = torch.empty((images, hout, wout, cout), device=x.device, dtype=torch.float32 if out_f32 else x.dtype)
    else:
        _req_cuda(out)
        assert tuple(out.shape) == (images, hout, wout, cout) and out.is_contiguous() and out.dtype == (torch.float32 if out_f32 else x.dtype)
        y = out
    ld_res = 0
    if residual is not None:
        assert residual.dtype == x.dtype and residual.is_contiguous() and residual.numel() == images * hout * wout * cout, \
            f"residual {tuple(residual.shape)} {residual.dtype} contiguous={residual.is_contiguous()} vs output {(images, hout, wout, cout)} {x.dtype}"
        ld_res = cout
    if rowbias is not None:
        assert rowbias.dtype == torch.float32 and rowbias.dim() == 2 and rowbias.shape[1] == cout and rows_per_group > 0
    if bias is not None:
        assert bias.dtype == torch.float32 and bias.numel() == cout
    args = ConvArgs(x=_p(x), x2=_p(x2), w=_p(w), y=_p(y), bias=_p(bias), rowbias=_p(rowbias),
                    residual=_p(residual), ld_res=ld_res,
                    ld_rowbias=rowbias.stride(0) if rowbias is not None else 0, images=images, hin=hin,
                    win=win, cin1=cin1, cin2=cin2, cout=cout, stride=stride, upsample=int(upsample),
                    rows_per_group=rows_per_group, alpha=alpha, post_scale=post_scale, act=act,
                    out_f32=int(out_f32), dtype=dt_code(x.dtype), pad_asym=int(pad_asym))
    if w_wino is not None and dispatch.conv_winograd:
        assert w_wino.dtype == x.dtype and w_wino.is_contiguous() and tuple(w_wino.shape) == (16, cout, cin1 + cin2)
        args.w_wino = _p(w_wino)
    wbytes = int(lib().ca_conv3x3_workspace_bytes(C.byref(args))) if split_k else 0
    if wbytes > 0:
        ws = torch.empty((wbytes,), device=x.device, dtype=torch.uint8)
        args.workspace, args.workspace_bytes = _p(ws), wbytes
    _record_plan(lib().ca_conv3x3_plan_name, args)
    check(lib().ca_conv3x3(C.byref(args), _stream()), "ca_conv3x3")
    return y


def _up2_args(x, w_phase, bias, residual, alpha, y=None) -> ConvArgs:
    images, hin, win, cin = x.shape
    cout = w_phase.shape[1]
    return ConvArgs(x=_p(x), w=_p(w_phase), y=_p(y) if y is not None else _p(x), bias=_p(bias), residual=_p(residual),
                    ld_res=cout if residual is not None else 0, images=images, hin=hin, win=win, cin1=cin, cin2=0, cout=cout, stride=1,
                    upsample=1, rows_per_group=0, alpha=alpha, post_scale=1.0, act=ACT_NONE, out_f32=0, dtype=dt_code(x.dtype), pad_asym=0)


def conv_up2_phase_supported(x: torch.Tensor, w_phase: torch.Tensor, *, bias: Optional[torch.Tensor] = None,
                             residual: Optional[torch.Tensor] = None, alpha: float = 1.0) -> bool:
    if x.dim() != 4 or w_phase.dim() != 5 or not x.is_contiguous() or x.dtype not in (torch.float16, torch.bfloat16):
        return False
    return bool(lib().ca_conv_up2_phase_supported(C.byref(_up2_args(x, w_phase, bias, residual, alpha))))


def conv_up2_phase(x: torch.Tensor, w_phase: torch.Tensor, *, bias: Optional[torch.Tensor] = None,
                   residual: Optional[torch.Tensor] = None, alpha: float = 1.0) -> torch.Tensor:
    _req_cuda(x, w_phase, bias, residual)
    assert x.dim() == 4 and x.is_contiguous() and w_phase.dim() == 5 and w_phase.is_contiguous() and w_phase.dtype == x.dtype
    images, hin, win, cin = x.shape
    cout = w_phase.shape[1]
    assert tuple(w_phase.shape) == (4, cout, 2, 2, cin)
    y = torch.empty((images, 2 * hin, 2 * win, cout), device=x.device, dtype=x.dtype)
    if residual is not None:
        assert residual.dtype == x.dtype and residual.is_contiguous() and residual.numel() == y.numel()
    if bias is not None:
        assert bias.dtype == torch.float32 and bias.numel() == cout
    args = _up2_args(x, w_phase, bias, residual, alpha, y)
    _record_plan(lib().ca_conv_up2_phase_plan_name, args)
    check(lib().ca_conv_up2_phase(C.byref(args), _stream()), "ca_conv_up2_phase")
    return y


_gn_wino_declined: dict = {}


def group_norm_conv3x3_wino(x: torch.Tensor, gamma: torch.Tensor, beta: torch.Tensor, w: torch.Tensor, w_wino: torch.Tensor, *,
                            x2: Optional[torch.Tensor] = None, groups: int = 32, eps: float = 1e-5, act: int = ACT_NONE,
                            bias: Optional[torch.Tensor] = None, rowbias: Optional[torch.Tensor] = None, rows_per_group: int = 0,
                            residual: Optional[torch.Tensor] = None, post_scale: float = 1.0) -> Optional[torch.Tensor]:
    if not (dispatch.conv_winograd and dispatch.gn_winograd):
        return None
    _req_cuda(x, gamma, beta, w, w_wino, x2, bias, rowbias, residual)
    if x.dim() != 4 or not x.is_contiguous() or x.dtype != torch.float16 or (x2 is not None and (not x2.is_contiguous() or x2.shape[:3] != x.shape[:3])):
        return None
    images, h, w_, c1 = x.shape
    c2 = 0 if x2 is None else x2.shape[3]
    c, cout = c1 + c2, w.shape[0]
    tiles = images * (h // 2) * (w_ // 2)
# ... 1480 lines not shown
```

### controlanimate_amd/unet.py

```python
from __future__ import annotations

from collections import OrderedDict

import dataclasses
import json
import os
from dataclasses import dataclass
from typing import Any, Dict, Optional, Tuple, Union

import torch
from torch import nn

from . import kernels as K
from .context import ExecCtx, dispatch
from .layers import HipGroupNorm, HipLinear, WeightArena, pack_concat_bias, pack_concat_rows
from .resnet import InflatedConv3d, InflatedGroupNorm, ResnetBlock3D
from .unet_blocks import UNetMidBlock3DCrossAttn, get_down_block, get_up_block


@dataclass
class UNet3DConditionOutput:
    sample: torch.Tensor


class FrozenConfig(dict):
    def __getattr__(self, k):
        try:
            return self[k]
        except KeyError as e:
            raise AttributeError(k) from e


class Timesteps(nn.Module):
    def __init__(self, num_channels: int, flip_sin_to_cos: bool = True, downscale_freq_shift: float = 0):
        super().__init__()
        if not flip_sin_to_cos or downscale_freq_shift != 0:
            raise NotImplementedError("SD1.5 uses flip_sin_to_cos=True, freq_shift=0")
        self.num_channels = num_channels


class TimestepEmbedding(nn.Module):
    def __init__(self, in_channels: int, time_embed_dim: int, act_fn: str = "silu", post_act_fn=None, cond_proj_dim=None):
        super().__init__()
        self.linear_1 = HipLinear(in_channels, time_embed_dim)
        self.cond_proj = HipLinear(cond_proj_dim, in_channels, bias=False) if cond_proj_dim is not None else None
        self.linear_2 = HipLinear(time_embed_dim, time_embed_dim)

    def pack(self, arena, dtype):
        self.linear_1.pack(arena, dtype)
        self.linear_2.pack(arena, dtype)
        if self.cond_proj is not None:
            self.cond_proj.pack(arena, dtype)


class HipModelMixin:

    def _init_exec(self):
        self.arena: Optional[WeightArena] = None
        self.act_dtype = torch.float16
        self._temb_w = self._temb_b = None
        self._slots: "OrderedDict[int, dict]" = OrderedDict()

    def all_resnets(self):
        return [m for m in self.modules() if isinstance(m, ResnetBlock3D)]

    def prepare(self, device=None, dtype: Optional[torch.dtype] = None) -> "HipModelMixin":
        if dtype is not None:
            self.act_dtype = dtype
        if device is None:
            device = next(self.parameters()).device
        device = torch.device(device)
        if device.type != "cuda":
            raise RuntimeError("prepare() needs a HIP device: the execution path has no CPU fallback")
        K.lib()
        arena = WeightArena()
        for child in self.children():
            self._pack_tree(child, arena)
        resnets = self.all_resnets()
        off = 0
        for r in resnets:
            r.temb_slice = (off, off + r.out_channels)
            off += r.out_channels
        self._temb_w = pack_concat_rows(arena, self.act_dtype, [r.time_emb_proj for r in resnets])
        self._temb_b = pack_concat_bias(arena, [r.time_emb_proj for r in resnets])
        arena.finalize(device)
        self.arena = arena
        self._slots.clear()
        return self

    MAX_CACHE_SLOTS = 4

    def cache_slot(self, src: Optional[torch.Tensor] = None) -> Optional[dict]:
        if src is None:
            return next(reversed(self._slots.values())) if self._slots else None
        ent = self._slots.get(id(src))
        return ent if ent is not None and ent["src"] is src else None

    @property
    def _cache(self) -> dict:
        ent = self.cache_slot()
        return ent["cache"] if ent is not None else {}

    @property
    def _cache_key(self):
        ent = self.cache_slot()
        return (ent["src"], ent["version"]) if ent is not None else None

    def refresh_window_caches(self, src: Optional[torch.Tensor] = None) -> int:
        ent = self.cache_slot(src)
        if ent is None or ent["cache"].get("ehs") is None:
            return 0
        cache, src = ent["cache"], ent["src"]
        ehs = cache["ehs"]
        ehs.copy_(src.to(device=ehs.device, dtype=ehs.dtype))
        ent["version"] = src._version
        nb, L, cd = ehs.shape
        n = 0
        for m in self.modules():
            kv = cache.get(("kv", id(m)))
            if kv is not None and hasattr(m, "kv"):
                K.gemm(ehs.reshape(nb * L, cd), m.kv.t, out=kv)
                n += 1
                ent = cache.get(("kvf", id(m)))
                if ent is not None and ent[0] is not None:
                    K.xattn_pack_kv(kv, nb, ent[2], ent[1], m.scale, out=ent[0])
        for proc in (getattr(self, "attn_processors", None) or {}).values():
            kvip = cache.get(("kv_ip", id(proc)))
            if kvip is not None:
                K.gemm(ehs.reshape(nb * L, cd), proc.kv_ip.t, out=kvip)
                n += 1
                ent = cache.get(("kvf_ip", id(proc)))
                if ent is not None and ent[0] is not None:
                    K.xattn_pack_kv(kvip, nb, ent[2], ent[1], ent[3], row_offset=ent[2] - ent[1], out=ent[0])
        return n

    def _pack_tree(self, m: nn.Module, arena: WeightArena):
        if hasattr(m, "pack"):
            m.pack(arena, self.act_dtype)
            return
        for c in m.children():
            self._pack_tree(c, arena)

    def release_master_weights(self):
        for p in self.parameters():
            p.data = torch.empty(0, dtype=p.dtype, device=p.device)

    def half(self):
        self.act_dtype = torch.float16
        self.arena = None
        return self

    def bfloat16(self):
        self.act_dtype = torch.bfloat16
        self.arena = None
        return self

    @property
    def dtype(self) -> torch.dtype:
        return self.act_dtype

    @property
    def device(self) -> torch.device:
        if self.arena is not None and self.arena.buffer is not None:
            return self.arena.buffer.device
        return next(self.parameters()).device

    def _ensure_ready(self, device):
        device = torch.device(device)
        if device.type == "cuda" and device.index is None:
            device = torch.device("cuda", torch.cuda.current_device())
        if self.arena is None or self.arena.buffer is None or self.arena.buffer.device != device:
            self.prepare(device)

    @property
    def attn_processors(self) -> Dict[str, Any]:
        procs: Dict[str, Any] = {}

        def rec(name, module):
            if hasattr(module, "get_processor"):
                procs[f"{name}.processor"] = module.get_processor(return_deprecated_lora=True)
            for sub, child in module.named_children():
                rec(f"{name}.{sub}", child)

        for name, module in self.named_children():
            rec(name, module)
        return procs

    def set_attn_processor(self, processor, _remove_lora=False):
        count = len(self.attn_processors)
        if isinstance(processor, dict) and len(processor) != count:
            raise ValueError(f"A dict of processors was passed, but the number of processors {len(processor)} does not match the"
                             f" number of attention layers: {count}. Please make sure to pass {count} processor classes.")
        processor = dict(processor) if isinstance(processor, dict) else processor

        def rec(name, module):
            if hasattr(module, "set_processor"):
                module.set_processor(processor if not isinstance(processor, dict) else processor.pop(f"{name}.processor"),
                                     _remove_lora=_remove_lora)
            for sub, child in module.named_children():
                rec(f"{name}.{sub}", child)

        for name, module in self.named_children():
            rec(name, module)
        self.arena = None

    def _time_embedding(self, timestep, groups: int, device, timestep_cond=None) -> torch.Tensor:
        dim = self.time_proj.num_channels
        if torch.is_tensor(timestep) and (timestep.numel() > 1 or timestep.is_cuda):
            if timestep.numel() not in (1, groups):
                raise ValueError("timestep tensor must be a scalar or one value per batch element")
            t = timestep.to(device=device, dtype=torch.float32).reshape(-1).expand(groups).contiguous()
            t_emb = K.timestep_embedding(t, groups, dim, self.act_dtype, device)
        else:
            tv = float(timestep.item()) if torch.is_tensor(timestep) else float(timestep)
            t_emb = K.timestep_embedding(tv, groups, dim, self.act_dtype, device)
        te = self.time_embedding
        if timestep_cond is not None:
            if te.cond_proj is None:
                raise ValueError("timestep_cond given but the model has no time_cond_proj_dim")
            cond = timestep_cond.to(device=device, dtype=self.act_dtype)
            if cond.shape[0] != groups:
                cond = cond.expand(groups, -1)
            t_emb = K.gemm(cond.contiguous(), te.cond_proj.w.t, residual=t_emb)
        h = te.linear_1.run(t_emb, act=K.ACT_SILU)
        emb = te.linear_2.run(h, act=K.ACT_SILU)
        return K.gemm(emb, self._temb_w.t, bias=self._temb_b.t, out_f32=True)

    def _prompt(self, encoder_hidden_states: torch.Tensor, device) -> Tuple[torch.Tensor, dict]:
        src = encoder_hidden_states
        ent = self.cache_slot(src)
        if ent is not None and "ehs" in ent["cache"] and tuple(ent["cache"]["ehs"].shape) == tuple(src.shape):
            self._slots.move_to_end(id(src))
            if ent["version"] != src._version:
                self.refresh_window_caches(src)
            return ent["cache"]["ehs"], ent["cache"]
        ehs = src.to(device=device, dtype=self.act_dtype).contiguous()
        ent = {"src": src, "version": src._version, "cache": {"ehs": ehs}}
        self._slots.pop(id(src), None)
        self._slots[id(src)] = ent
        while len(self._slots) > self.MAX_CACHE_SLOTS:
            self._slots.popitem(last=False)
        return ehs, ent["cache"]


class UNet3DConditionModel(HipModelMixin, nn.Module):
    _supports_gradient_checkpointing = False

    def __init__(
        self,
        sample_size: Optional[int] = None,
        in_channels: int = 4,
        out_channels: int = 4,
        center_input_sample: bool = False,
        flip_sin_to_cos: bool = True,
        freq_shift: int = 0,
        down_block_types: Tuple[str, ...] = ("CrossAttnDownBlock3D", "CrossAttnDownBlock3D", "CrossAttnDownBlock3D", "DownBlock3D"),
        mid_block_type: str = "UNetMidBlock3DCrossAttn",
        up_block_types: Tuple[str, ...] = ("UpBlock3D", "CrossAttnUpBlock3D", "CrossAttnUpBlock3D", "CrossAttnUpBlock3D"),
        only_cross_attention: Union[bool, Tuple[bool, ...]] = False,
        block_out_channels: Tuple[int, ...] = (320, 640, 1280, 1280),
        layers_per_block: int = 2,
        downsample_padding: int = 1,
        mid_block_scale_factor: float = 1,
        act_fn: str = "silu",
        norm_num_groups: int = 32,
        norm_eps: float = 1e-5,
        cross_attention_dim: int = 1280,
        attention_head_dim: Union[int, Tuple[int, ...]] = 8,
        dual_cross_attention: bool = False,
        use_linear_projection: bool = False,
        class_embed_type: Optional[str] = None,
        num_class_embeds: Optional[int] = None,
        upcast_attention: bool = False,
        resnet_time_scale_shift: str = "default",
        use_inflated_groupnorm: bool = False,
        time_cond_proj_dim: Optional[int] = None,
        use_motion_module: bool = False,
        motion_module_resolutions: Tuple[int, ...] = (1, 2, 4, 8),
# ... 197 lines not shown
```

### include/controlanimate_hip.h

```cpp
#ifndef CONTROLANIMATE_HIP_H
#define CONTROLANIMATE_HIP_H

#include <stdint.h>

#ifdef __cplusplus
extern "C" {
#endif

#define CA_ABI_VERSION 16

#define CA_BF16 0
#define CA_F16 1
#define CA_F32 2

#define CA_OK 0
#define CA_ERR_INVALID_ARG (-1)
#define CA_ERR_UNSUPPORTED (-2)
#define CA_ERR_LAUNCH (-3)

#define CA_ACT_NONE 0
#define CA_ACT_SILU 1
#define CA_ACT_QUICK_GELU 2
#define CA_ACT_GELU 3
#define CA_ACT_RELU 4
#define CA_ACT_RELU6 5
#define CA_ACT_LEAKY02 6

int ca_abi_version(void);
const char* ca_last_error(void);

typedef struct ca_gemm_args {
  const void* a;
  const void* a2;
  const void* w;
  void* c;
  const float* bias;
  const float* rowbias;
  const void* residual;
  int64_t lda, lda2, ldc, ld_res, ld_rowbias;
  int32_t m, n, k1, k2;
  int32_t rows_per_group;
  float alpha, post_scale;
  int32_t act;
  int32_t geglu;
  int32_t out_f32;
  int32_t dtype;
  const float* ln_stats;
  const float* ln_colsum;
  float ln_eps;
  void* workspace;
  int64_t workspace_bytes;
  float* row_sums_out;
  int32_t ln_parts;
  const void* w_frag;
} ca_gemm_args;
int ca_gemm(const ca_gemm_args* args, void* stream);
int ca_pack_w_frag(const void* w, int32_t n, int32_t k, int32_t geglu, void* dst, void* stream);
typedef struct ca_ff_args {
  const void* x;
  const void* w1_frag;
  const float* bias1;
  const float* colsum1;
  const float* ln_stats;
  const void* w2_frag;
  const float* bias2;
  const void* residual;
  void* y;
  int64_t lda, ldc, ld_res;
  int32_t m, c, inner;
  float ln_eps;
  int32_t dtype;
  const void* w_out_frag;
  const float* bias_out;
  const void* residual_out;
  int64_t ld_res_out;
} ca_ff_args;
int ca_ff_fused(const ca_ff_args* args, void* stream);
int ca_ff_fused_supported(const ca_ff_args* args);
int ca_pack_w2_frag(const void* w, int32_t n, int32_t k, void* dst, void* stream);
#define CA_TATTN_W_FRAG_ELEMS 368640
typedef struct ca_tattn_args {
  const void* x;
  const void* w_frag;
  const float* gamma;
  const float* bias_pe;
  void* o;
  int64_t lda, ldo, ld_bias_pe;
  int32_t batch, frames, tokens, heads, c;
  float ln_eps, scale;
  int32_t dtype;
  const void* w_out_frag;
  const float* bias_out;
  const void* residual;
  int64_t ld_res;
} ca_tattn_args;
int ca_tattn_fused(const ca_tattn_args* args, void* stream);
int ca_tattn_fused_supported(const ca_tattn_args* args);
#define CA_ATTN_WOUT_FRAG_ELEMS 102400
int ca_pack_w_out(const void* w, int32_t n, int32_t k, void* dst, void* stream);
int ca_pack_w_tattn(const void* w, int32_t n, int32_t k, void* dst, void* stream);
#define CA_XATTN_W_FRAG_ELEMS 122880
#define CA_XATTN_KV_FRAG_ELEMS 7680
typedef struct ca_xattn_args {
  const void* x;
  const void* wq_frag;
  const float* bias;
  const void* kv_frag;
  void* o;
  int64_t lda, ldo;
  int32_t m, tokens, frames_per_kv, kv_mod, kv_batches, nk, heads, c;
  float ln_eps;
  int32_t dtype;
  const void* w_out_frag;
  const float* bias_out;
  const void* residual;
  int64_t ld_res;
  const void* kv_frag_ip;
  int32_t nk_ip;
  float ip_scale;
} ca_xattn_args;
int ca_xattn_fused(const ca_xattn_args* args, void* stream);
int ca_xattn_fused_supported(const ca_xattn_args* args);
int ca_xattn_pack_w(const void* w, int32_t n, int32_t k, void* dst, void* stream);
int ca_xattn_pack_kv(const void* kv, int64_t ld, int32_t kv_batches, int32_t rows_per_batch, int32_t row_offset, int32_t nk, float scale, int32_t dtype,
                     void* dst, void* stream);
int64_t ca_gemm_workspace_bytes(const ca_gemm_args* args);
int ca_gemm_row_sums_parts(const ca_gemm_args* args);
int ca_gemm_ln_inline_supported(const ca_gemm_args* args);
int ca_gemm_wants_finished_stats(const ca_gemm_args* args);
int ca_ln_finish_sums(const float* sums, int parts, int64_t rows, int k, float eps, float* mean_rstd, void* stream);
int ca_gemm_plan_name(const ca_gemm_args* args, char* buf, int32_t len);

typedef struct ca_conv_args {
  const void* x;
  const void* x2;
  const void* w;
  void* y;
  const float* bias;
  const float* rowbias;
  const void* residual;
  int64_t ld_res, ld_rowbias;
  int32_t images, hin, win, cin1, cin2, cout;
  int32_t stride;
  int32_t upsample;
  int32_t rows_per_group;
  float alpha, post_scale;
  int32_t act;
  int32_t out_f32;
  int32_t dtype;
  void* workspace;
  int64_t workspace_bytes;
  int32_t pad_asym;
  const void* w_wino;
  int32_t x_is_wino_v;
} ca_conv_args;
int ca_pack_w_wino(const void* w, int32_t cout, int32_t cin, int32_t dtype, void* dst, void* stream);
int64_t ca_conv3x3_workspace_bytes(const ca_conv_args* args);
int ca_conv3x3(const ca_conv_args* args, void* stream);
int ca_conv3x3_plan_name(const ca_conv_args* args, char* buf, int32_t len);
int ca_conv_up2_phase_supported(const ca_conv_args* args);
int ca_conv_up2_phase(const ca_conv_args* args, void* stream);
int ca_conv_up2_phase_plan_name(const ca_conv_args* args, char* buf, int32_t len);

typedef struct ca_groupnorm_args {
  const void* x;
  const void* x2;
  void* y;
  const float* gamma;
  const float* beta;
  float* partials;
  int32_t images, hw, c1, c2;
  int32_t groups;
  int32_t frames_per_stat;
  float eps;
  int32_t act;
  int32_t dtype;
  void* wino_v;
  int32_t wino_h, wino_w;
} ca_groupnorm_args;
int ca_groupnorm_wino_supported(const ca_groupnorm_args* args);
int64_t ca_groupnorm_partials_floats(int32_t images, int32_t hw, int32_t frames_per_stat, int32_t groups);
int ca_groupnorm_stats(const ca_groupnorm_args* args, void* stream);
int ca_groupnorm_apply(const ca_groupnorm_args* args, void* stream);
int ca_groupnorm(const ca_groupnorm_args* args, void* stream);

typedef struct ca_layernorm_args {
  const void* x; void* y;
  const float* gamma; const float* beta;
  const float* pos;
  int64_t rows;
  int32_t c;
  int32_t rows_per_frame, frames;
  float eps;
  int32_t dtype;
  float* stats;
} ca_layernorm_args;
int ca_layernorm(const ca_layernorm_args* args, void* stream);

typedef struct ca_attn_args {
  const void* q; const void* k; const void* v; void* o;
  int64_t q_outer, q_inner, q_row;
  int64_t o_outer, o_inner, o_row;
  int64_t k_outer, k_inner, k_row;
  int32_t inner_count, kv_inner_count, kv_div, kv_mod;
  int32_t batches, heads, head_dim;
  int32_t nq, nk;
  float scale;
  float out_scale;
  int32_t accumulate;
  int32_t dtype;
  int32_t causal;
  const uint8_t* key_mask;
  int64_t key_mask_stride;
} ca_attn_args;
int ca_attention(const ca_attn_args* args, void* stream);
int ca_attention_plan_name(const ca_attn_args* args, char* buf, int32_t len);


int ca_add_bcast(const void* a, const void* b, void* out, int64_t n, int64_t b_period,
                 int32_t dtype, void* stream);
int ca_repeat(const void* src, void* dst, int64_t bytes, int32_t times, void* stream);

int ca_softmax_rows(const float* x, void* y, int64_t rows, int32_t cols, int64_t ldx, int64_t ldy,
                    float scale, int32_t dtype, void* stream);

int ca_silu_f32(const float* x, float* y, int64_t n, void* stream);

int ca_timestep_embedding(const float* t_dev, float t_host, void* out, int32_t batch,
                          int32_t dim, int32_t dtype, void* stream);

int ca_latents_to_nhwc(const float* latents, void* out, int32_t b0, int32_t c, int32_t f,
                       int32_t h, int32_t w, int32_t cpad, int32_t rep, float in_scale,
                       int32_t dtype, void* stream);

int ca_nhwc_to_ncfhw_f32(const void* x, float* out, int32_t b, int32_t c, int32_t f, int32_t h,
                         int32_t w, int32_t ldx, int32_t x_is_f32, int32_t dtype, void* stream);

int ca_ncfhw_to_nhwc(const void* x, int32_t x_kind , const int64_t strides[5],
                     void* out, int32_t b, int32_t c, int32_t f, int32_t h, int32_t w, int32_t cpad,
                     int32_t dtype, void* stream);

int ca_cfg_scheduler_step(const float* eps, int32_t ld_eps, int32_t rep, float guidance,
                          const float* latents, const float* noise, float* prev, float* denoised,
                          int32_t c, int32_t f, int32_t h, int32_t w, const float coef[7],
                          float clip, void* stream);

int ca_lincomb(float* out, const float* const* x, const float* coef, int32_t n_terms, int64_t n, void* stream);

typedef struct ca_conv3x3_narrow_args {
  const void* x;
  const void* w;
  void* y;
  const float* bias;
  const void* r1;
  const void* r2;
  int64_t ldx, ldy, ld_r1, ld_r2;
  int32_t images, hin, win, cin, cout;
  int32_t channel_offset;
  int32_t upsample;
  int32_t leaky_relu;
  float s0, s1, s2;
  int32_t out_u8;
  int32_t dtype;
} ca_conv3x3_narrow_args;
int ca_conv3x3_narrow(const ca_conv3x3_narrow_args* args, void* stream);
int ca_conv3x3_narrow_plan_name(const ca_conv3x3_narrow_args* args, char* buf, int32_t len);

int ca_rgb8_to_nhwc(const uint8_t* src, void* dst, int32_t images, int32_t h, int32_t w, int32_t dtype, void* stream);

int ca_resize_lanczos4_u8(const uint8_t* src, uint8_t* dst, int32_t images, int32_t sh, int32_t sw, int32_t dh, int32_t dw,
                          const int32_t* xofs, const int16_t* alpha, const int32_t* yofs, const int16_t* beta, void* stream);


int64_t ca_color_match_workspace_bytes(int32_t images, int64_t pixels);

int ca_hist_u8x3(const uint8_t* src, uint32_t* hist, int32_t images, int64_t pixels, void* stream);

int ca_color_moments_f64(const uint8_t* src, const double* lut, const double* mean, double* moments, int32_t images,
// ... 286 lines not shown
```

Baseline: 16.39.

## Fold cross-attention Q/K and V/out projections into two grouped GEMMs

Result: no change. 16.47, median of 6 (+0.5%).

```diff
diff --git a/controlanimate_amd/_capi.py b/controlanimate_amd/_capi.py
--- a/controlanimate_amd/_capi.py
+++ b/controlanimate_amd/_capi.py
@@ -85,6 +85,17 @@
     ]
 
 
+class XattnFoldedArgs(C.Structure):
+    _fields_ = [
+        ("x", C.c_void_p), ("ln_stats", C.c_void_p), ("w1", C.c_void_p), ("colsum1", C.c_void_p), ("bias1", C.c_void_p), ("p", C.c_void_p),
+        ("w2", C.c_void_p), ("bias_out", C.c_void_p), ("residual", C.c_void_p), ("y", C.c_void_p), ("row_sums_out", C.c_void_p),
+        ("lda", C.c_int64), ("ldy", C.c_int64), ("ld_res", C.c_int64),
+        ("m", C.c_int32), ("c", C.c_int32), ("heads", C.c_int32), ("nk", C.c_int32),
+        ("rows_per_group", C.c_int32), ("group_mod", C.c_int32), ("groups", C.c_int32),
+        ("dtype", C.c_int32),
+    ]
+
+
 XATTN_W_FRAG_ELEMS = 122880
 XATTN_KV_FRAG_ELEMS = 7680
 
@@ -200,6 +211,11 @@
     "ca_xattn_fused_supported": (C.c_int, [C.POINTER(XattnArgs)]),
     "ca_xattn_pack_w": (C.c_int, [C.c_void_p, C.c_int32, C.c_int32, C.c_void_p, C.c_void_p]),
     "ca_xattn_pack_kv": (C.c_int, [C.c_void_p, C.c_int64, C.c_int32, C.c_int32, C.c_int32, C.c_int32, C.c_float, C.c_int32, C.c_void_p, C.c_void_p]),
+    "ca_xattn_folded_supported": (C.c_int, [C.POINTER(XattnFoldedArgs)]),
+    "ca_xattn_folded": (C.c_int, [C.POINTER(XattnFoldedArgs), C.c_void_p]),
+    "ca_xattn_folded_plan_name": (C.c_int, [C.POINTER(XattnFoldedArgs), C.c_char_p, C.c_int32]),
+    "ca_xattn_fold_pack": (C.c_int, [C.c_void_p, C.c_int64, C.c_int32, C.c_int32, C.c_int32, C.c_int32, C.c_int32, C.c_float, C.c_int32,
+                                     C.c_void_p, C.c_void_p, C.c_void_p, C.c_void_p, C.c_void_p, C.c_void_p, C.c_void_p, C.c_void_p]),
     "ca_gemm_ln_inline_supported": (C.c_int, [C.POINTER(GemmArgs)]),
     "ca_gemm_wants_finished_stats": (C.c_int, [C.POINTER(GemmArgs)]),
     "ca_ln_finish_sums": (C.c_int, [C.c_void_p, C.c_int, C.c_int64, C.c_int, C.c_float, C.c_void_p, C.c_void_p]),
diff --git a/controlanimate_amd/attention_processor.py b/controlanimate_amd/attention_processor.py
--- a/controlanimate_amd/attention_processor.py
+++ b/controlanimate_amd/attention_processor.py
@@ -75,6 +75,11 @@
                 if o is not None:
                     out = attn.to_out[0].run(o, residual=res, row_sums=row_sums)
                     return K.carry_row_sums(out.reshape(B, N, C), out)
+        if (ln is not None and encoder_hidden_states is not None and cache is not None and builtin and self.num_tokens == 0 and dispatch.xattn_folded
+                and attn.query_dim in (640, 1280) and attn.inner_dim == attn.query_dim):
+            out = xattn_folded_site(attn, x, res, ln, encoder_hidden_states, B, N, frames_per_kv, kv_mod, cache, row_sums)
+            if out is not None:
+                return K.carry_row_sums(out.reshape(B, N, C), out)
         if ln is not None:
             st, fold = ln
             if encoder_hidden_states is None and temporal is not None and fold.pe is not None:
@@ -106,6 +111,40 @@
         return K.carry_row_sums(out.reshape(B, N, C), out)
 
 
+def xattn_folded_site(attn: "Attention", x, res, ln, ctx, images: int, tokens: int, frames_per_kv: int, kv_mod: int, cache: dict,
+                      row_sums: bool = False, force: bool = False, keep_p: bool = False):
+    st, fold = ln
+    nb, L, cd = ctx.shape
+    m = images * tokens
+    rows_per_group, group_mod = tokens * frames_per_kv, (kv_mod if kv_mod > 0 else nb)
+    key = ("xfold", id(attn), m, rows_per_group, group_mod)
+    ent = cache.get(key)
+    if ent is None:
+        packed = None
+        if L <= 80 and K.xattn_folded_supported(m, attn.query_dim, attn.heads, L, rows_per_group, group_mod, nb, x.dtype, force=force):
+            kv = cache.get(("kv", id(attn)))
+            if kv is None:
+                kv = cache[("kv", id(attn))] = K.gemm(ctx.reshape(nb * L, cd), attn.kv.t)
+            packed = K.xattn_fold_pack(kv, nb, L, L, attn.heads, attn.scale, fold.w.t, fold.b.t, attn.to_out[0].w.t)
+        ent = cache[key] = (packed, attn, L)
+    if ent[0] is None or ent[2] != L:
+        return None
+    to_out = attn.to_out[0]
+    return K.xattn_folded(x, st, ent[0], L, rows_per_group, group_mod, bias_out=None if to_out.b is None else to_out.b.t, residual=res,
+                          row_sums=row_sums, force=force, keep_p=keep_p)
+
+
+def refresh_xattn_folded(cache: dict, nb: int) -> int:
+    n = 0
+    for key, ent in cache.items():
+        if isinstance(key, tuple) and key[0] == "xfold" and ent[0] is not None:
+            packed, attn, L = ent
+            fold = attn.fold
+            K.xattn_fold_pack(cache[("kv", id(attn))], nb, L, L, attn.heads, attn.scale, fold.w.t, fold.b.t, attn.to_out[0].w.t, out=packed)
+            n += 1
+    return n
+
+
 class IPAttnProcessor2_0(AttnProcessor2_0):
 
     def __init__(self, hidden_size, cross_attention_dim=None, scale=1.0, num_tokens=4):
diff --git a/controlanimate_amd/context.py b/controlanimate_amd/context.py
--- a/controlanimate_amd/context.py
+++ b/controlanimate_amd/context.py
@@ -41,6 +41,7 @@
     repeat_kernel = True
     ln_fold = True
     cfg_shared = True
+    xattn_folded = True
     cn_cfg_dedup = True
     pdc_block_fused = True
     dpt_head_fused = False
diff --git a/controlanimate_amd/csrc/ca_gemm.hip b/controlanimate_amd/csrc/ca_gemm.hip
--- a/controlanimate_amd/csrc/ca_gemm.hip
+++ b/controlanimate_amd/csrc/ca_gemm.hip
@@ -565,6 +565,114 @@
   return CA_OK;
 }
 
+namespace {
+template <int DT>
+__global__ __launch_bounds__(256) void k_xfold_pack_w1(const u16* __restrict__ kv, int64_t ld, int rows_per_batch, int nk, int c, int heads, float sl2,
+                                                       const u16* __restrict__ wq, const float* __restrict__ bq, u16* __restrict__ w1,
+                                                       float* __restrict__ cs1, float* __restrict__ b1) {
+  __shared__ float kk[256];
+  __shared__ float red[2][256];
+  const int tid = threadIdx.x, n1 = heads * 80, d = c / heads;
+  const int g = (int)blockIdx.x / n1, n = (int)blockIdx.x % n1, h = n / 80, j = n % 80;
+  const bool live = j < nk;
+  float bpart = 0.f, spart = 0.f;
+  if (live && tid < d) {
+    kk[tid] = Elem<DT>::to_f(kv[((int64_t)g * rows_per_batch + j) * ld + h * d + tid]);
+    bpart = kk[tid] * bq[h * d + tid];
+  }
+  __syncthreads();
+  u16* dst = w1 + ((int64_t)g * n1 + n) * c;
+  for (int col = tid; col < c; col += 256) {
+    float acc = 0.f;
+    if (live)
+      for (int dd = 0; dd < d; ++dd) acc = fmaf(kk[dd], Elem<DT>::to_f(wq[(int64_t)(h * d + dd) * c + col]), acc);
+    const u16 r = Elem<DT>::from_f(acc * sl2);
+    dst[col] = r;
+    spart += Elem<DT>::to_f(r);
+  }
+  red[0][tid] = spart;
+  red[1][tid] = bpart;
+  __syncthreads();
+  for (int s = 128; s > 0; s >>= 1) {
+    if (tid < s) red[0][tid] += red[0][tid + s], red[1][tid] += red[1][tid + s];
+    __syncthreads();
+  }
+  if (tid == 0) cs1[g * n1 + n] = red[0][0], b1[g * n1 + n] = red[1][0] * sl2;
+}
+template <int DT>
+__global__ __launch_bounds__(256) void k_xfold_pack_w2(const u16* __restrict__ kv, int64_t ld, int rows_per_batch, int nk, int c, int heads,
+                                                       const u16* __restrict__ wo, u16* __restrict__ w2) {
+  __shared__ float ww[2048];
+  const int tid = threadIdx.x, n1 = heads * 80, d = c / heads;
+  const int g = (int)blockIdx.x / c, n = (int)blockIdx.x % c;
+  for (int t = tid; t < c; t += 256) ww[t] = Elem<DT>::to_f(wo[(int64_t)n * c + t]);
+  __syncthreads();
+  u16* dst = w2 + ((int64_t)g * c + n) * n1;
+  for (int col = tid; col < n1; col += 256) {
+    const int h = col / 80, j = col % 80;
+    float acc = 0.f;
+    if (j < nk) {
+      const u16* vrow = kv + ((int64_t)g * rows_per_batch + j) * ld + c + h * d;
+      for (int dd = 0; dd < d; dd += 8) {
+        float v[8];
+        unpack8<DT>(ld16(vrow + dd), v);
+#pragma unroll
+        for (int k = 0; k < 8; ++k) acc = fmaf(ww[h * d + dd + k], v[k], acc);
+      }
+    }
+    dst[col] = Elem<DT>::from_f(acc);
+  }
+}
+}
+
+extern "C" int ca_xattn_fold_pack(const void* kv, int64_t ld, int32_t groups, int32_t rows_per_batch, int32_t nk, int32_t c, int32_t heads, float scale, int32_t dtype,
+                                  const void* wq, const float* bq, const void* wo, void* w1, float* colsum1, float* bias1, void* w2, void* stream) {
+  CA_REQUIRE(kv && wq && bq && wo && w1 && colsum1 && bias1 && w2, "ca_xattn_fold_pack: null operand");
+  CA_REQUIRE(dtype == CA_BF16 || dtype == CA_F16, "ca_xattn_fold_pack: dtype %d", dtype);
+  CA_REQUIRE(groups > 0 && heads > 0 && c > 0 && c % heads == 0 && (c / heads) % 8 == 0 && c / heads <= 256 && c <= 2048 && (int64_t)groups * c * heads * 80 < (1ll << 30),
+             "ca_xattn_fold_pack: groups=%d c=%d heads=%d (head dim a multiple of 8, <= 256; c <= 2048)", groups, c, heads);
+  CA_REQUIRE(nk >= 1 && nk <= 80 && nk <= rows_per_batch && ld >= 2 * (int64_t)c && ld % 8 == 0 && scale > 0.f,
+             "ca_xattn_fold_pack: nk=%d rows_per_batch=%d ld=%lld (K | V of c columns each, 1..80 keys)", nk, rows_per_batch, (long long)ld);
+  CA_REQUIRE((((uintptr_t)kv | (uintptr_t)wq | (uintptr_t)wo | (uintptr_t)w1 | (uintptr_t)w2) & 15) == 0, "ca_xattn_fold_pack: operands must be 16-byte aligned");
+  const float sl2 = scale * 1.4426950408889634f;
+  hipStream_t st = (hipStream_t)stream;
+  const dim3 g1((unsigned)(groups * heads * 80)), g2((unsigned)(groups * c));
+  if (dtype == CA_BF16) {
+    hipLaunchKernelGGL((k_xfold_pack_w1<CA_BF16>), g1, dim3(256), 0, st, (const u16*)kv, ld, rows_per_batch, nk, c, heads, sl2, (const u16*)wq, bq, (u16*)w1, colsum1, bias1);
+    hipLaunchKernelGGL((k_xfold_pack_w2<CA_BF16>), g2, dim3(256), 0, st, (const u16*)kv, ld, rows_per_batch, nk, c, heads, (const u16*)wo, (u16*)w2);
+  } else {
+    hipLaunchKernelGGL((k_xfold_pack_w1<CA_F16>), g1, dim3(256), 0, st, (const u16*)kv, ld, rows_per_batch, nk, c, heads, sl2, (const u16*)wq, bq, (u16*)w1, colsum1, bias1);
+    hipLaunchKernelGGL((k_xfold_pack_w2<CA_F16>), g2, dim3(256), 0, st, (const u16*)kv, ld, rows_per_batch, nk, c, heads, (const u16*)wo, (u16*)w2);
+  }
+  CA_CHECK_LAUNCH("ca_xattn_fold_pack");
+  return CA_OK;
+}
+
+extern "C" int ca_xattn_folded_supported(const ca_xattn_folded_args* a) {
+  GemmKParams p1{}, p2{};
+  return xfold_capable(a, p1, p2) && xfold_pays(p1, p2) ? 1 : 0;
+}
+
+extern "C" int ca_xattn_folded(const ca_xattn_folded_args* a, void* stream) {
+  GemmKParams p1{}, p2{};
+  CA_REQUIRE(xfold_capable(a, p1, p2), "ca_xattn_folded: arguments the folded form does not take (fp16 / bf16, heads %% 4 == 0, c %% 320 == 0, 1 <= nk <= 80, "
+             "rows_per_group %% 256 == 0, groups >= group_mod >= 1, strides multiples of 8, 16-byte aligned operands, < 2 GB each)");
+  int rc = ca_launch_gemm_pp(p1, a->dtype, 0, PK_PQ, xfold_tiles(p1), (hipStream_t)stream);
+  if (rc) return rc;
+  rc = ca_launch_gemm_pp(p2, a->dtype, 0, PK_PQ, xfold_tiles(p2), (hipStream_t)stream);
+  if (rc) return rc;
+  CA_CHECK_LAUNCH("ca_xattn_folded");
+  return CA_OK;
+}
+
+extern "C" int ca_xattn_folded_plan_name(const ca_xattn_folded_args* a, char* buf, int32_t len) {
+  CA_REQUIRE(buf && len > 0, "ca_xattn_folded_plan_name: buffer");
+  GemmKParams p1{}, p2{};
+  CA_REQUIRE(xfold_capable(a, p1, p2), "ca_xattn_folded_plan_name: arguments the folded form does not take");
+  snprintf(buf, (size_t)len, "pq256x320_xsm");
+  return CA_OK;
+}
+
 extern "C" int ca_gemm_plan_name(const ca_gemm_args* a, char* buf, int32_t len) {
   CA_REQUIRE(buf && len > 0, "ca_gemm_plan_name: buffer");
   DenseLaunch d;
diff --git a/controlanimate_amd/csrc/ca_gemm_core.h b/controlanimate_amd/csrc/ca_gemm_core.h
--- a/controlanimate_amd/csrc/ca_gemm_core.h
+++ b/controlanimate_amd/csrc/ca_gemm_core.h
@@ -38,6 +38,7 @@
   unsigned w_group_stride;
   int up2_rows, up2_tiles;
   unsigned up2_mag_w, up2_mag_h;
+  int w_group_mod, w_group_count, xsm_nk;
 };
 
 constexpr int BK = 64;
diff --git a/controlanimate_amd/csrc/ca_gemm_plan.h b/controlanimate_amd/csrc/ca_gemm_plan.h
--- a/controlanimate_amd/csrc/ca_gemm_plan.h
+++ b/controlanimate_amd/csrc/ca_gemm_plan.h
@@ -364,4 +364,45 @@
   return tiles >= 256 && (tiles % 256 == 0 || tiles >= 1024);
 }
 
-}
+inline bool xfold_capable(const ca_xattn_folded_args* a, GemmKParams& p1, GemmKParams& p2) {
+  if (!a || !a->x || !a->ln_stats || !a->w1 || !a->colsum1 || !a->bias1 || !a->p || !a->w2 || !a->y) return false;
+  if ((a->dtype != CA_F16 && a->dtype != CA_BF16) || a->m <= 0 || a->heads <= 0 || a->heads % 4 != 0) return false;
+  if (a->c < 2 * BK || a->c % 320 != 0 || a->c % BK != 0 || a->nk < 1 || a->nk > 80) return false;
+  if (a->rows_per_group <= 0 || a->rows_per_group % 256 != 0 || a->group_mod < 1 || a->groups < a->group_mod) return false;
+  if (a->lda < a->c || a->lda % 8 != 0 || a->ldy < a->c || a->ldy % 8 != 0 || (a->residual && (a->ld_res < a->c || a->ld_res % 8 != 0))) return false;
+  if ((((uintptr_t)a->x | (uintptr_t)a->w1 | (uintptr_t)a->p | (uintptr_t)a->w2 | (uintptr_t)a->y | (uintptr_t)a->residual) & 15) != 0) return false;
+  if ((((uintptr_t)a->ln_stats | (uintptr_t)a->colsum1 | (uintptr_t)a->bias1 | (uintptr_t)a->bias_out | (uintptr_t)a->row_sums_out) & 7) != 0) return false;
+  const int n1 = a->heads * 80;
+  GemmKParams q{};
+  q.taps = 1;
+  q.rows_per_group = 1;
+  q.alpha = 1.f, q.post = 1.f;
+  q.splits = 1;
+  q.m = a->m;
+  q.w_group_rows = a->rows_per_group, q.w_group_mod = a->group_mod, q.w_group_count = a->groups;
+  p1 = q;
+  p1.a = (const u16*)a->x, p1.w = (const u16*)a->w1, p1.c = a->p;
+  p1.bias = a->bias1, p1.ln_stats = a->ln_stats, p1.ln_colsum = a->colsum1;
+  p1.lda = a->lda, p1.ldc = n1;
+  p1.n = n1, p1.c1 = a->c, p1.kc_tiles = a->c / BK;
+  p1.a_bytes = desc_bytes((int64_t)(a->m - 1) * a->lda + a->c);
+  p1.w_bytes = desc_bytes((int64_t)a->groups * n1 * a->c);
+  p1.w_group_stride = (unsigned)((int64_t)n1 * a->c * 2);
+  p1.xsm_nk = a->nk;
+  p2 = q;
+  p2.a = (const u16*)a->p, p2.w = (const u16*)a->w2, p2.c = a->y;
+  p2.bias = a->bias_out, p2.res = (const u16*)a->residual, p2.row_sums = a->row_sums_out;
+  p2.lda = n1, p2.ldc = a->ldy, p2.ld_res = a->ld_res;
+  p2.n = a->c, p2.c1 = n1, p2.kc_tiles = n1 / BK;
+  p2.a_bytes = desc_bytes((int64_t)a->m * n1);
+  p2.w_bytes = desc_bytes((int64_t)a->groups * a->c * n1);
+  p2.w_group_stride = p1.w_group_stride;
+  return dma_capable(p1) && dma_capable(p2) && act_out_fit31(p1) && act_out_fit31(p2) && p1.w_bytes < FIT31 && p2.w_bytes < FIT31;
+}
+inline unsigned xfold_tiles(const GemmKParams& p) { return (unsigned)(ceil_div_i(p.m, 256) * (p.n / 320)); }
+inline bool xfold_pays(const GemmKParams& p1, const GemmKParams& p2) {
+  (void)p2;
+  return p1.m >= (p1.c1 >= 1280 ? 8192 : 32768);
+}
+
+}
diff --git a/controlanimate_amd/csrc/ca_gemm_pp.hip b/controlanimate_amd/csrc/ca_gemm_pp.hip
--- a/controlanimate_amd/csrc/ca_gemm_pp.hip
+++ b/controlanimate_amd/csrc/ca_gemm_pp.hip
@@ -54,7 +54,9 @@
   switch (kind) {
     case PK_PQ: {
       auto launch = [&](const GemmKParams& q) {
-        if (MODE == 0 && (q.geglu || q.ln_colsum || q.ln_stats)) hipLaunchKernelGGL((k_gemm_pq<DT, 0, 1>), dim3(grid), dim3(512), 0, st, q, (int)tiles, c_bytes, 0u);
+        if (MODE == 0 && q.xsm_nk > 0) hipLaunchKernelGGL((k_gemm_pq<DT, 0, 3>), dim3(grid), dim3(512), 0, st, q, (int)tiles, c_bytes, 0u);
+        else if (MODE == 0 && q.w_group_mod > 0) hipLaunchKernelGGL((k_gemm_pq<DT, 0, 4>), dim3(grid), dim3(512), 0, st, q, (int)tiles, c_bytes, res_bytes);
+        else if (MODE == 0 && (q.geglu || q.ln_colsum || q.ln_stats)) hipLaunchKernelGGL((k_gemm_pq<DT, 0, 1>), dim3(grid), dim3(512), 0, st, q, (int)tiles, c_bytes, 0u);
         else if (MODE == 0 && q.row_sums) hipLaunchKernelGGL((k_gemm_pq<DT, 0, 2>), dim3(grid), dim3(512), 0, st, q, (int)tiles, c_bytes, res_bytes);
         else hipLaunchKernelGGL((k_gemm_pq<DT, MODE>), dim3(grid), dim3(512), 0, st, q, (int)tiles, c_bytes, res_bytes);
       };
diff --git a/controlanimate_amd/csrc/ca_gemm_pq.h b/controlanimate_amd/csrc/ca_gemm_pq.h
--- a/controlanimate_amd/csrc/ca_gemm_pq.h
+++ b/controlanimate_amd/csrc/ca_gemm_pq.h
@@ -18,7 +18,7 @@
   constexpr int OFF_A = 0, OFF_B0 = A_ROWS * KT, OFF_B1 = (A_ROWS + B0_ROWS) * KT;
   constexpr int BUF = (A_ROWS + B0_ROWS + B1_ROWS) * KT;
   constexpr int PAR_BASE = 2 * BUF * 2;
-  constexpr int P_BI = 0, P_RB0 = 1280, P_RB1 = 2560, P_CS = 3840, PSET = EPI == 1 ? 5120 : 4096;
+  constexpr int P_BI = 0, P_RB0 = 1280, P_RB1 = 2560, P_CS = 3840, PSET = (EPI == 1 || EPI == 3) ? 5120 : 4096;
   constexpr int FLAG_BASE = PAR_BASE + 2 * PSET;
   constexpr int SMEM_BYTES = FLAG_BASE + 8 * 2 * 256;
   static_assert(SMEM_BYTES <= 160 * 1024, "LDS");
@@ -45,7 +45,7 @@
   const __amdgpu_buffer_rsrc_t rs_a2 = __builtin_amdgcn_make_buffer_rsrc((void*)(p.a2 ? p.a2 : p.a), 0, p.a2 ? p.a2_bytes : p.a_bytes, 0x00020000);
   const __amdgpu_buffer_rsrc_t rs_w = __builtin_amdgcn_make_buffer_rsrc((void*)p.w, 0, p.w_bytes, 0x00020000);
   const __amdgpu_buffer_rsrc_t rs_c = __builtin_amdgcn_make_buffer_rsrc(p.c, 0, c_bytes, 0x00020000);
-  const __amdgpu_buffer_rsrc_t rs_bi = __builtin_amdgcn_make_buffer_rsrc((void*)(p.bias ? (const void*)p.bias : (const void*)p.w), 0, p.bias ? (unsigned)p.n * 4u : 0u, 0x00020000);
+  const __amdgpu_buffer_rsrc_t rs_bi = __builtin_amdgcn_make_buffer_rsrc((void*)(p.bias ? (const void*)p.bias : (const void*)p.w), 0, p.bias ? (unsigned)p.n * 4u * (EPI == 3 ? (unsigned)p.w_group_count : 1u) : 0u, 0x00020000);
   const bool geglu = EPI == 1 && p.geglu != 0;
   const unsigned long long res_addr = (unsigned long long)(p.res ? (const void*)p.res : (const void*)p.c);
   const u32x4 rs_res = {(unsigned)__builtin_amdgcn_readfirstlane((int)(unsigned)res_addr), (unsigned)__builtin_amdgcn_readfirstlane((int)(unsigned)((res_addr >> 32) & 0xffffu)),
@@ -128,6 +128,8 @@
     }
     unsigned wgrp = 0u;
     if (MODE == 0 && EPI == 0 && p.w_group_rows > 0) wgrp = (unsigned)(m0 / p.w_group_rows) * p.w_group_stride;
+    unsigned grp = 0u;
+    if (MODE == 0 && EPI >= 3) grp = (unsigned)((m0 / p.w_group_rows) % p.w_group_mod), wgrp = grp * p.w_group_stride;
     if (MODE == 2) wgrp = (unsigned)(m0 / (p.up2_tiles * BM)) * p.w_group_stride;
 #pragma unroll
     for (int i = 0; i < 2; ++i) {
@@ -147,9 +149,15 @@
       __builtin_amdgcn_raw_ptr_buffer_load_lds(rs_cs, (__attribute__((address_space(3))) void*)(pset + P_CS), 16, (unsigned)n0 * 4u + lane_o * 16u, 0, 0, 0);
       __builtin_amdgcn_raw_ptr_buffer_load_lds(rs_cs, (__attribute__((address_space(3))) void*)(pset + P_CS + 1024), 4, (unsigned)n0 * 4u + 1024u + lane_o * 4u, 0, 0, 0);
     }
+    if (EPI == 3 && wid == 4) {
+      const __amdgpu_buffer_rsrc_t rs_cs = __builtin_amdgcn_make_buffer_rsrc((void*)p.ln_colsum, 0, (unsigned)p.n * 4u * (unsigned)p.w_group_count, 0x00020000);
+      const unsigned base = (grp * (unsigned)p.n + (unsigned)n0) * 4u;
+      __builtin_amdgcn_raw_ptr_buffer_load_lds(rs_cs, (__attribute__((address_space(3))) void*)(pset + P_CS), 16, base + lane_o * 16u, 0, 0, 0);
+      __builtin_amdgcn_raw_ptr_buffer_load_lds(rs_cs, (__attribute__((address_space(3))) void*)(pset + P_CS + 1024), 4, base + 1024u + lane_o * 4u, 0, 0, 0);
+    }
     if (wid >= 1 && wid <= 3) {
       const bool has1 = p.rowbias && m0 / p.rows_per_group + 1 < (int)rb_groups;
-      const unsigned base = wid == 1 ? (unsigned)n0 * 4u
+      const unsigned base = wid == 1 ? ((EPI == 3 ? grp * (unsigned)p.n : 0u) + (unsigned)n0) * 4u
                                      : wid == 2 ? (unsigned)n0 * 4u + (unsigned)(p.rowbias ? m0 / p.rows_per_group : 0) * (unsigned)p.ld_rowbias * 4u
                                                 : (has1 ? (unsigned)n0 * 4u + (unsigned)(m0 / p.rows_per_group + 1) * (unsigned)p.ld_rowbias * 4u : OOB_V);
       unsigned char* dst = pset + (wid == 1 ? P_BI : wid == 2 ? P_RB0 : P_RB1);
@@ -376,7 +384,7 @@
                              Elem<DT>::to_f((u16)(w[k] >> 16)) + Elem<DT>::to_f((u16)(rr >> 16)));
           }
         }
-        if (EPI == 2) {
+        if (EPI == 2 || EPI == 4) {
 #pragma unroll
           for (int k = 0; k < 4; ++k) {
             if (k >= 2 * nq) break;
@@ -389,7 +397,7 @@
         else __builtin_amdgcn_raw_buffer_store_b64((u32x2){w[0], w[1]}, rs_c, ro + (unsigned)(64 + 4 * g) * 2u, 0, 0);
       }
     }
-    if (EPI == 2) {
+    if (EPI == 2 || (EPI == 4 && p.row_sums)) {
       const int tn4 = (n0 / BN) * 4 + wc, parts = (p.n / BN) * 4;
 #pragma unroll
       for (int i = 0; i < TM; ++i) {
@@ -464,6 +472,78 @@
       if (geglu) {
         __builtin_amdgcn_raw_buffer_store_b128((u32x4){w[0], w[1], w[2], w[3]}, rs_c, ro + (unsigned)(8 * g) * 2u, 0, 0);
         __builtin_amdgcn_raw_buffer_store_b32(w[4], rs_c, ro + (unsigned)(32 + 2 * g) * 2u, 0, 0);
+      }
+    }
+#pragma unroll
+    for (int i = 0; i < TM; ++i)
+#pragma unroll
+      for (int j = 0; j < TN; ++j) acc[i][j] = (f32x4){0.f, 0.f, 0.f, 0.f};
+    asm volatile("s_waitcnt lgkmcnt(0)" ::: "memory");
+  };
+
+  auto epilogue_xsm = [&](int seq, int m0, int n0) __attribute__((always_inline)) {
+    const unsigned char* pset = smem_b + PAR_BASE + (seq & 1) * PSET;
+    int lane_o = lane;
+    asm volatile("" : "+v"(lane_o));
+    const int l15 = lane_o & 15, g = lane_o >> 4;
+    float2 st[TM];
+    {
+      const __amdgpu_buffer_rsrc_t rs_st = __builtin_amdgcn_make_buffer_rsrc((void*)p.ln_stats, 0, (unsigned)p.m * 8u, 0x00020000);
+#pragma unroll
+      for (int i = 0; i < TM; ++i) {
+        const int m = m0 + wr * 128 + i * 16 + l15;
+        const u32x2 v = __builtin_bit_cast(u32x2, __builtin_amdgcn_raw_buffer_load_b64(rs_st, m < p.m ? (unsigned)m * 8u : OOB_V, 0, 0));
+        st[i] = make_float2(__uint_as_float(v[0]), __uint_as_float(v[1]));
+      }
+    }
+    f32x4 cs[TN], bi[TN];
+    int kq[TN];
+#pragma unroll
+    for (int j = 0; j < TN; ++j) {
+      kq[j] = j < 4 ? 32 * (j >> 1) + 8 * g + 4 * (j & 1) : 64 + 4 * g;
+      cs[j] = *reinterpret_cast<const f32x4*>(pset + P_CS + (wc * 80 + kq[j]) * 4);
+      bi[j] = *reinterpret_cast<const f32x4*>(pset + P_BI + (wc * 80 + kq[j]) * 4);
+    }
+#pragma unroll
+    for (int i = 0; i < TM; ++i) {
+      const int m = m0 + wr * 128 + i * 16 + l15;
+      const unsigned ro = (m < p.m && p.dbg != 1) ? (unsigned)m * (unsigned)p.ldc * 2u + (unsigned)(n0 + wc * 80) * 2u : OOB_V;
+      float mx = -INFINITY;
+#pragma unroll
+      for (int j = 0; j < TN; ++j)
+#pragma unroll
+        for (int r = 0; r < 4; ++r) {
+          float x = st[i].y * (acc[i][j][r] - st[i].x * cs[j][r]) + bi[j][r];
+          x = kq[j] + r < p.xsm_nk ? x : -INFINITY;
+          acc[i][j][r] = x;
+          mx = fmaxf(mx, x);
+        }
+      mx = fmaxf(mx, __shfl_xor(mx, 16));
+      mx = fmaxf(mx, __shfl_xor(mx, 32));
+      float sum = 0.f;
+#pragma unroll
+      for (int j = 0; j < TN; ++j)
+#pragma unroll
+        for (int r = 0; r < 4; ++r) {
+          const float e = __builtin_amdgcn_exp2f(acc[i][j][r] - mx);
+          acc[i][j][r] = e;
+          sum += e;
+        }
+      sum += __shfl_xor(sum, 16);
+      sum += __shfl_xor(sum, 32);
+      const float inv = 1.f / sum;
+      unsigned w0 = 0u, w1 = 0u;
+#pragma unroll
+      for (int j = 0; j < TN; ++j) {
+        const unsigned lo = pack2<DT>(acc[i][j][0] * inv, acc[i][j][1] * inv), hi = pack2<DT>(acc[i][j][2] * inv, acc[i][j][3] * inv);
+        if (j == 4) {
+          __builtin_amdgcn_raw_buffer_store_b64((u32x2){lo, hi}, rs_c, ro + (unsigned)(64 + 4 * g) * 2u, 0, 0);
+        } else if ((j & 1) == 0) {
+          w0 = lo;
+          w1 = hi;
+        } else {
+          __builtin_amdgcn_raw_buffer_store_b128((u32x4){w0, w1, lo, hi}, rs_c, ro + (unsigned)(32 * (j >> 1) + 8 * g) * 2u, 0, 0);
+        }
       }
     }
 #pragma unroll
@@ -524,6 +604,7 @@
     if (wr == 0) __builtin_amdgcn_s_barrier();
     stamp(9);
     if (EPI == 1) epilogue_ln(seq, m0, n0);
+    else if (EPI == 3) epilogue_xsm(seq, m0, n0);
     else epilogue(seq, m0, n0);
     stamp(10);
     if (wr == 1) __builtin_amdgcn_s_barrier();
diff --git a/controlanimate_amd/kernels.py b/controlanimate_amd/kernels.py
--- a/controlanimate_amd/kernels.py
+++ b/controlanimate_amd/kernels.py
@@ -201,6 +201,85 @@
     return dst
 
 
+def xattn_fold_pack(kv: torch.Tensor, groups: int, rows_per_batch: int, nk: int, heads: int, scale: float, wq: torch.Tensor, bq: torch.Tensor,
+                    wo: torch.Tensor, out=None):
+    _req_cuda(kv, wq, bq, wo)
+    c = wq.shape[0]
+    assert kv.dim() == 2 and kv.stride(1) == 1 and kv.shape == (groups * rows_per_batch, 2 * c) and kv.dtype == wq.dtype == wo.dtype
+    assert wq.shape == (c, c) and wo.shape == (c, c) and wq.is_contiguous() and wo.is_contiguous() and bq.dtype == torch.float32 and bq.numel() == c
+    n1 = heads * 80
+    if out is None:
+        out = (torch.empty((groups, n1, c), device=kv.device, dtype=kv.dtype), torch.empty((groups, n1), device=kv.device, dtype=torch.float32),
+               torch.empty((groups, n1), device=kv.device, dtype=torch.float32), torch.empty((groups, c, n1), device=kv.device, dtype=kv.dtype))
+    w1, cs1, b1, w2 = out
+    assert w1.shape == (groups, n1, c) and w2.shape == (groups, c, n1) and w1.is_contiguous() and w2.is_contiguous() and w1.dtype == kv.dtype
+    check(lib().ca_xattn_fold_pack(kv.data_ptr(), kv.stride(0), groups, rows_per_batch, nk, c, heads, float(scale), dt_code(kv.dtype), wq.data_ptr(),
+                                   bq.data_ptr(), wo.data_ptr(), w1.data_ptr(), cs1.data_ptr(), b1.data_ptr(), w2.data_ptr(), _stream()), "ca_xattn_fold_pack")
+    return out
+
+
+def _xattn_folded_args(x, w1, cs1, b1, w2, nk, rows_per_group, group_mod, bias_out, residual) -> _capi.XattnFoldedArgs:
+    groups, n1, c = w1.shape
+    return _capi.XattnFoldedArgs(x=_p(x), w1=_p(w1), colsum1=_p(cs1), bias1=_p(b1), w2=_p(w2), bias_out=_p(bias_out), residual=_p(residual),
+                                 lda=x.stride(0), ldy=c, ld_res=residual.stride(0) if residual is not None else 0, m=x.shape[0], c=c, heads=n1 // 80, nk=nk,
+                                 rows_per_group=rows_per_group, group_mod=group_mod, groups=groups, dtype=dt_code(x.dtype))
+
+
+def xattn_folded_supported(m: int, c: int, heads: int, nk: int, rows_per_group: int, group_mod: int, groups: int, dtype: torch.dtype, *,
+                           key_mask=None, force: bool = False) -> bool:
+    if not dispatch.xattn_folded or key_mask is not None or dtype not in (torch.float16, torch.bfloat16) or heads <= 0 or c % 8 != 0:
+        return False
+    fake = 0x1000
+    args = _capi.XattnFoldedArgs(x=fake, ln_stats=fake, w1=fake, colsum1=fake, bias1=fake, p=fake, w2=fake, y=fake, lda=c, ldy=c, m=m, c=c, heads=heads, nk=nk,
+                                 rows_per_group=rows_per_group, group_mod=group_mod, groups=groups, dtype=dt_code(dtype))
+    if lib().ca_xattn_folded_supported(C.byref(args)):
+        return True
+    return bool(force) and lib().ca_xattn_folded_plan_name(C.byref(args), C.create_string_buffer(64), 64) == 0
+
+
+def xattn_folded(x: torch.Tensor, st: "RowStats", packed, nk: int, rows_per_group: int, group_mod: int, *, bias_out: Optional[torch.Tensor] = None,
+                 residual: Optional[torch.Tensor] = None, row_sums: bool = False, force: bool = False, keep_p: bool = False) -> Optional[torch.Tensor]:
+    if not dispatch.xattn_folded:
+        return None
+    w1, cs1, b1, w2 = packed
+    _req_cuda(x, w1, cs1, b1, w2, bias_out, residual)
+    if x.dim() != 2 or x.stride(1) != 1 or x.shape[1] != w1.shape[2] or x.dtype != w1.dtype:
+        return None
+    if residual is not None and (residual.shape != x.shape or residual.stride(1) != 1 or residual.dtype != x.dtype):
+        return None
+    m, c = x.shape
+    args = _xattn_folded_args(x, w1, cs1, b1, w2, nk, rows_per_group, group_mod, bias_out, residual)
+    args.ln_stats = args.p = args.y = _p(x)
+    if not lib().ca_xattn_folded_supported(C.byref(args)):
+        name = C.create_string_buffer(64)
+        if not (force and lib().ca_xattn_folded_plan_name(C.byref(args), name, 64) == 0):
+            return None
+    assert isinstance(st, RowStats) and st.x.data_ptr() == x.data_ptr() and st.x.shape == x.shape, "RowStats belongs to another tensor"
+    if st.sums is not None:
+        fin = getattr(st, "_finished", None)
+        if fin is None:
+            rs, parts = st.sums
+            fin = torch.empty((m, 2), device=x.device, dtype=torch.float32)
+            check(lib().ca_ln_finish_sums(_p(rs), parts, m, c, st.eps, _p(fin), _stream()), "ca_ln_finish_sums")
+            st._finished = fin
+    else:
+        fin = st.tensor()
+    p = torch.empty((m, w1.shape[1]), device=x.device, dtype=x.dtype)
+    y = torch.empty((m, c), device=x.device, dtype=x.dtype)
+    args.ln_stats, args.p, args.y = _p(fin), _p(p), _p(y)
+    if row_sums and dispatch.ln_row_sums:
+        parts = 4 * (c // 320)
+        rs = torch.empty((m, parts, 2), device=x.device, dtype=torch.float32)
+        args.row_sums_out = _p(rs)
+        y._row_sums = (rs, parts)
+    if _plan_sink is not None:
+        _plan_sink.extend(["pq256x320_xsm", "pq256x320_xsm"])
+    check(lib().ca_xattn_folded(C.byref(args), _stream()), "ca_xattn_folded")
+    if keep_p:
+        y._p = p
+    return y
+
+
 def xattn_fused(x: torch.Tensor, wq_frag: torch.Tensor, bias: Optional[torch.Tensor], kv_frag: torch.Tensor, images: int, tokens: int,
                 frames_per_kv: int, kv_mod: int, nk: int, ln_eps: float, *, w_out_frag: Optional[torch.Tensor] = None,
                 bias_out: Optional[torch.Tensor] = None, residual: Optional[torch.Tensor] = None, kv_frag_ip: Optional[torch.Tensor] = None,
diff --git a/controlanimate_amd/unet.py b/controlanimate_amd/unet.py
--- a/controlanimate_amd/unet.py
+++ b/controlanimate_amd/unet.py
@@ -124,6 +124,8 @@
                 ent = cache.get(("kvf", id(m)))
                 if ent is not None and ent[0] is not None:
                     K.xattn_pack_kv(kv, nb, ent[2], ent[1], m.scale, out=ent[0])
+        from .attention_processor import refresh_xattn_folded
+        refresh_xattn_folded(cache, nb)
         for proc in (getattr(self, "attn_processors", None) or {}).values():
             kvip = cache.get(("kv_ip", id(proc)))
             if kvip is not None:
diff --git a/include/controlanimate_hip.h b/include/controlanimate_hip.h
--- a/include/controlanimate_hip.h
+++ b/include/controlanimate_hip.h
@@ -124,6 +124,28 @@
 int ca_xattn_pack_w(const void* w, int32_t n, int32_t k, void* dst, void* stream);
 int ca_xattn_pack_kv(const void* kv, int64_t ld, int32_t kv_batches, int32_t rows_per_batch, int32_t row_offset, int32_t nk, float scale, int32_t dtype,
                      void* dst, void* stream);
+typedef struct ca_xattn_folded_args {
+  const void* x;
+  const float* ln_stats;
+  const void* w1;
+  const float* colsum1;
+  const float* bias1;
+  void* p;
+  const void* w2;
+  const float* bias_out;
+  const void* residual;
+  void* y;
+  float* row_sums_out;
+  int64_t lda, ldy, ld_res;
+  int32_t m, c, heads, nk;
+  int32_t rows_per_group, group_mod, groups;
+  int32_t dtype;
+} ca_xattn_folded_args;
+int ca_xattn_folded_supported(const ca_xattn_folded_args* args);
+int ca_xattn_folded(const ca_xattn_folded_args* args, void* stream);
+int ca_xattn_folded_plan_name(const ca_xattn_folded_args* args, char* buf, int32_t len);
+int ca_xattn_fold_pack(const void* kv, int64_t ld, int32_t groups, int32_t rows_per_batch, int32_t nk, int32_t c, int32_t heads, float scale, int32_t dtype,
+                       const void* wq, const float* bq, const void* wo, void* w1, float* colsum1, float* bias1, void* w2, void* stream);
 int64_t ca_gemm_workspace_bytes(const ca_gemm_args* args);
 int ca_gemm_row_sums_parts(const ca_gemm_args* args);
 int ca_gemm_ln_inline_supported(const ca_gemm_args* args);
```
